# mauruszach/multimodal_diffusion

Hardware: AMD Instinct MI355X
Metric: denoising steps/sec @256x256 multimodal-cond batch=32 (higher is better)
Workload: dtype f32 via 3xbf16 split operands (6-term products, f32 accumulate; fp32-level error); 1 GPU; C3: 256x256 audio->video CFG denoising step (cond+null MMDiT d512 L8 H8 + noise head + DDIM), 384+37 tokens, batch 32 per GPU, DDIM 50 steps, guidance 3.5; global_batch=32, sampler_steps=50, parallelism=dp1, launch=eager, matmul=bf16x3, attn=default, cfg_halves=one stacked 2B batch, one stream

## Files before the change

### multimodal_diffusion_amd/csrc/attn_bf16x3.hip

```cpp
#include "avd_common.h"

#include <stdlib.h>
#include <type_traits>

namespace avd {

constexpr int A3_DH = 64, A3_KT = 64, A3_NW = 4;
constexpr float A3_NEG = -1.0e30f;

typedef short s16x4 __attribute__((ext_vector_type(4)));
typedef unsigned int u32x2 __attribute__((ext_vector_type(2)));
typedef float f32x4t __attribute__((ext_vector_type(4)));

#define AVD_LDS_PTR(p) ((__attribute__((address_space(3))) void*)(p))
#define AVD_GLB_PTR(p) ((const __attribute__((address_space(1))) void*)(p))

template <int TERMS> struct A3Terms;
template <> struct A3Terms<6> { static constexpr int N = 6; static constexpr int PA[6] = {2, 0, 1, 1, 0, 0}; static constexpr int PB[6] = {0, 2, 1, 0, 1, 0}; };
template <> struct A3Terms<9> { static constexpr int N = 9; static constexpr int PA[9] = {2, 2, 1, 2, 0, 1, 1, 0, 0}; static constexpr int PB[9] = {2, 1, 2, 0, 2, 1, 0, 1, 0}; };
template <> struct A3Terms<1> { static constexpr int N = 1; static constexpr int PA[1] = {0}; static constexpr int PB[1] = {0}; };
template <> struct A3Terms<3> { static constexpr int N = 3; static constexpr int PA[3] = {0, 1, 0}; static constexpr int PB[3] = {1, 0, 0}; };

template <bool SPLIT_OUT, int TERMS>
__global__ __launch_bounds__(A3_NW * 64, 2) void attn_bf16x3_kernel(const unsigned char* __restrict__ img, float* __restrict__ out,
                                                                    int Bt, int N, int Npad, int H, int n_query, int nqb,
                                                                    float s_inv2, float v_inv, float o_scale, int out_tok) {
    constexpr int NW = A3_NW, ROWB = QKV3_ROWB;
    constexpr bool F16 = TERMS == 3;
    constexpr int NPL = s3_planes(TERMS);
    constexpr int PPW = 24 / NW;
    __shared__ __attribute__((aligned(16))) unsigned char Ks[A3_KT * ROWB];
    __shared__ __attribute__((aligned(16))) unsigned char Vs[A3_KT * ROWB];

    int qb, h, b;
    {
        const int nwg = gridDim.x, id = blockIdx.x, q = nwg >> 3, r = nwg & 7, x = id & 7;
        const int w = (x < r ? x * (q + 1) : r * (q + 1) + (x - r) * q) + (id >> 3);
        qb = w % nqb;
        h = (w / nqb) % H;
        b = w / (nqb * H);
    }
    const int tid = threadIdx.x, lane = tid & 63, wave = tid >> 6;
    const int l31 = lane & 31, hi = lane >> 5;
    const int64_t hstride = (int64_t)Npad * ROWB;
    const unsigned char* Qb = img + (((int64_t)0 * Bt + b) * H + h) * hstride;
    const unsigned char* Kb = img + (((int64_t)1 * Bt + b) * H + h) * hstride;
    const unsigned char* Vb = img + (((int64_t)2 * Bt + b) * H + h) * hstride;

    const int q_row = qb * (NW * 32) + wave * 32 + l31;
    bf16x8 qf[4][3];
    {
        const unsigned char* src = Qb + (int64_t)(q_row < N ? q_row : N - 1) * ROWB + hi * 16;
#pragma unroll
        for (int s = 0; s < 4; ++s)
#pragma unroll
            for (int p = 0; p < NPL; ++p) qf[s][p] = *reinterpret_cast<const bf16x8*>(src + p * 128 + s * 32);
    }

    auto dma = [&](const unsigned char* gsrc, unsigned char* ldst, int kt) {
        const int last_row = N - 1 - kt * A3_KT;
#pragma unroll
        for (int i = 0; i < PPW; ++i) {
            const int p = wave + NW * i;
            const int off = p * 1024 + lane * 16;
            int row = off / ROWB;
            const int within = off - row * ROWB;
            row = row < last_row ? row : last_row;
            __builtin_amdgcn_global_load_lds(AVD_GLB_PTR(gsrc + ((int64_t)kt * A3_KT + row) * ROWB + within), AVD_LDS_PTR(ldst + p * 1024), 16,
                                             0, 0);
        }
    };

    f32x16 o0, o1;
#pragma unroll
    for (int r = 0; r < 16; ++r) { o0[r] = 0.f; o1[r] = 0.f; }
    float m_run = A3_NEG, l_run = 0.f;

    const int nkt = (N + A3_KT - 1) / A3_KT;
    dma(Kb, Ks, 0);
    dma(Vb, Vs, 0);
    __builtin_amdgcn_s_waitcnt(0x0f70);
    __syncthreads();

    const int ksw = (l31 >> 1) & 7;
    const int k_rd = l31 * ROWB;
    const int i16 = lane & 15, cb = (lane >> 4) & 1;
    const int v_q = i16 >> 2, v_p = i16 & 3;

    const bool active = qb * (NW * 32) + wave * 32 < n_query;
    for (int kt = 0; kt < nkt; ++kt) {
        const bool more = (kt + 1) < nkt;
        if (!active) {
            __builtin_amdgcn_s_waitcnt(0x0f70);
            __syncthreads();
            if (more) dma(Kb, Ks, kt + 1);
            __builtin_amdgcn_s_waitcnt(0x0f70);
            __syncthreads();
            if (more) dma(Vb, Vs, kt + 1);
            continue;
        }
        f32x16 s0, s1;
#pragma unroll
// ... 71 lines not shown
                for (int p = 0; p < NPL; ++p) pf[p] = __builtin_bit_cast(bf16x8, P[p]);
                const int key0 = 32 * kb + 16 * t + 4 * hi + v_q;
                const int sw = qkv3_swizzle(2, key0);
#pragma unroll
                for (int db = 0; db < 2; ++db) {
                    const int chunk = 4 * db + 2 * cb + (v_p >> 1);
                    bf16x8 vf[3];
#pragma unroll
                    for (int p = 0; p < NPL; ++p) {
                        const s16x4 lo = __builtin_amdgcn_ds_read_tr16_b64_v4i16((__attribute__((address_space(3))) s16x4*)AVD_LDS_PTR(
                            Vs + key0 * ROWB + p * 128 + ((chunk ^ sw) << 4) + 8 * (v_p & 1)));
                        const s16x4 up = __builtin_amdgcn_ds_read_tr16_b64_v4i16((__attribute__((address_space(3))) s16x4*)AVD_LDS_PTR(
                            Vs + (key0 + 8) * ROWB + p * 128 + ((chunk ^ sw) << 4) + 8 * (v_p & 1)));
                        const u32x2 a = __builtin_bit_cast(u32x2, lo), c2 = __builtin_bit_cast(u32x2, up);
                        const u32x4 w = {a[0], a[1], c2[0], c2[1]};
                        vf[p] = __builtin_bit_cast(bf16x8, w);
                    }
#pragma unroll
                    for (int tt = 0; tt < TT::N; ++tt) {
                        if (db == 0) o0 = mma16<F16>(vf[TT::PA[tt]], pf[TT::PB[tt]], o0);
                        else o1 = mma16<F16>(vf[TT::PA[tt]], pf[TT::PB[tt]], o1);
                    }
                }
            }
        __builtin_amdgcn_s_waitcnt(0x0f70);
        __syncthreads();
        if (more) dma(Vb, Vs, kt + 1);
    }
    if (!active) return;

    const float l_tot = l_run + __shfl_xor(l_run, 32, 64);
    const float inv = F16 ? v_inv / l_tot : 1.0f / l_tot;
    const int d = H * A3_DH;
    if constexpr (SPLIT_OUT) {
        float ch[8][4];
#pragma unroll
        for (int g4 = 0; g4 < 4; ++g4)
#pragma unroll
            for (int e = 0; e < 4; ++e) {
                ch[g4][e] = o0[4 * g4 + e] * inv;
                ch[4 + g4][e] = o1[4 * g4 + e] * inv;
            }
        unsigned char* o3 = reinterpret_cast<unsigned char*>(out);
#pragma unroll
        for (int c = 0; c < 8; c += 2) {
            float v[8];
#pragma unroll
            for (int e = 0; e < 4; ++e) {
                const float send = hi ? ch[c][e] : ch[c + 1][e];
                const float recv = __shfl_xor(send, 32, 64);
                v[e] = hi ? recv : ch[c][e];
                v[4 + e] = hi ? ch[c + 1][e] : recv;
            }
            if (q_row < n_query) {
                if constexpr (F16) store_split8_h2(o3, (int64_t)b * out_tok + q_row, h * A3_DH + 8 * (c + hi), d, v, o_scale);
                else store_split8(o3, (int64_t)b * out_tok + q_row, h * A3_DH + 8 * (c + hi), d, v);
            }
        }
    } else if (q_row < n_query) {
        float* dst = out + ((int64_t)b * out_tok + q_row) * d + h * A3_DH + 4 * hi;
#pragma unroll
        for (int g4 = 0; g4 < 4; ++g4) {
            f32x4 a = {o0[4 * g4] * inv, o0[4 * g4 + 1] * inv, o0[4 * g4 + 2] * inv, o0[4 * g4 + 3] * inv};
            f32x4 c = {o1[4 * g4] * inv, o1[4 * g4 + 1] * inv, o1[4 * g4 + 2] * inv, o1[4 * g4 + 3] * inv};
            *reinterpret_cast<f32x4*>(dst + 8 * g4) = a;
            *reinterpret_cast<f32x4*>(dst + 32 + 8 * g4) = c;
        }
    }
}

int g_attn_pipe = getenv("AVD_ATTN_PIPE") ? atoi(getenv("AVD_ATTN_PIPE")) : 1;

template <bool MORE_, bool KCL_, bool VCL_, bool COPY_> struct A3Flags {
    static constexpr bool MORE = MORE_, KCL = KCL_, VCL = VCL_, COPY = COPY_;
};

template <bool SPLIT_OUT, int TERMS>
__global__ __launch_bounds__(A3_NW * 64, 2) void attn_bf16x3_pipe_kernel(const unsigned char* __restrict__ img, float* __restrict__ out,
                                                                         int Bt, int N, int Npad, int H, int n_query, int nqb,
                                                                         float s_inv2, float v_inv, float o_scale, int out_tok) {
    constexpr int NW = A3_NW, ROWB = QKV3_ROWB;
    constexpr bool F16 = TERMS == 3;
    constexpr int NPL = s3_planes(TERMS);
    constexpr int PPW = 24 / NW;
    using TT = A3Terms<TERMS>;
    __shared__ __attribute__((aligned(16))) unsigned char Ks[A3_KT * ROWB];
    __shared__ __attribute__((aligned(16))) unsigned char Vs[A3_KT * ROWB];

    int qb, h, b;
    {
        const int nwg = gridDim.x, id = blockIdx.x, q = nwg >> 3, r = nwg & 7, x = id & 7;
        const int w = (x < r ? x * (q + 1) : r * (q + 1) + (x - r) * q) + (id >> 3);
        qb = w % nqb;
        h = (w / nqb) % H;
        b = w / (nqb * H);
    }
    const int tid = threadIdx.x, lane = tid & 63;
    const int wave = __builtin_amdgcn_readfirstlane(tid >> 6);
    const int l31 = lane & 31, hi = lane >> 5;
    const int64_t hstride = (int64_t)Npad * ROWB;
    const unsigned char* Qb = img + (((int64_t)0 * Bt + b) * H + h) * hstride;
    const unsigned char* Kb = img + (((int64_t)1 * Bt + b) * H + h) * hstride;
    const unsigned char* Vb = img + (((int64_t)2 * Bt + b) * H + h) * hstride;

    const int q_row = qb * (NW * 32) + wave * 32 + l31;
    bf16x8 qf[4][3];
    {
        const unsigned char* src = Qb + (int64_t)(q_row < N ? q_row : N - 1) * ROWB + hi * 16;
#pragma unroll
        for (int s = 0; s < 4; ++s)
#pragma unroll
            for (int p = 0; p < NPL; ++p) qf[s][p] = *reinterpret_cast<const bf16x8*>(src + p * 128 + s * 32);
    }
    auto dma_clamp = [&](const unsigned char* gsrc, unsigned char* ldst, int kt) {
        const int last_row = N - 1 - kt * A3_KT;
#pragma unroll
        for (int i = 0; i < PPW; ++i) {
            const int p = wave + NW * i;
            const int off = p * 1024 + lane * 16;
            int row = off / ROWB;
            const int within = off - row * ROWB;
            row = row < last_row ? row : last_row;
            __builtin_amdgcn_global_load_lds(AVD_GLB_PTR(gsrc + ((int64_t)kt * A3_KT + row) * ROWB + within), AVD_LDS_PTR(ldst + p * 1024), 16,
                                             0, 0);
        }
    };
    const unsigned lane16 = (unsigned)lane * 16u;
    auto dma_full = [&](const unsigned char* gsrc, unsigned char* ldst, int kt) {
        const unsigned char* base = gsrc + ((int64_t)kt * (A3_KT * ROWB) + wave * 1024);
#pragma unroll
        for (int i = 0; i < PPW; ++i)
            __builtin_amdgcn_global_load_lds(AVD_GLB_PTR(base + i * (NW * 1024) + lane16), AVD_LDS_PTR(ldst + (wave + NW * i) * 1024), 16, 0, 0);
    };
    auto sync = [&]() {
        __builtin_amdgcn_s_waitcnt(0x0f70);
        __syncthreads();
    };

    const int nkt = (N + A3_KT - 1) / A3_KT;
    const bool ragged = (N & (A3_KT - 1)) != 0;
    dma_clamp(Kb, Ks, 0);
    dma_clamp(Vb, Vs, 0);
    sync();

    const bool active = qb * (NW * 32) + wave * 32 < n_query;
    if (!active) {
        sync();
        if (nkt > 1) dma_clamp(Kb, Ks, 1);
        sync();
        for (int kt = 0; kt < nkt; ++kt) {
            sync();
            if (kt + 2 < nkt) dma_clamp(Kb, Ks, kt + 2);
            if (kt + 1 < nkt) {
                sync();
                dma_clamp(Vb, Vs, kt + 1);
            }
        }
        return;
// ... 169 lines not shown
            if constexpr (F16) mt *= s_inv2;
            mt = fmaxf(mt, __shfl_xor(mt, 32, 64));
            m_new = fmaxf(m_run, mt);
            if constexpr (FL::COPY) {
                c0 = n0;
                c1 = n1;
            }
            sync();
            if constexpr (FL::VCL) dma_clamp(Vb, Vs, kt + 1);
            else dma_full(Vb, Vs, kt + 1);
        }
    };
    {
        using Main = A3Flags<true, false, false, false>;
        using MainC = A3Flags<true, false, false, true>;
        using KClamp = A3Flags<true, true, false, true>;
        using VClamp = A3Flags<true, false, true, true>;
        using Last = A3Flags<false, false, false, false>;
        int kt = 0;
        for (; kt + 4 < nkt; kt += 2) {
            tile(Main{}, kt, sa0, sa1, sb0, sb1);
            tile(Main{}, kt + 1, sb0, sb1, sa0, sa1);
        }
        if (nkt - kt == 4) { tile(MainC{}, kt, sa0, sa1, sb0, sb1); ++kt; }
        if (nkt - kt == 3) { tile(KClamp{}, kt, sa0, sa1, sb0, sb1); ++kt; }
        if (nkt - kt == 2) { tile(VClamp{}, kt, sa0, sa1, sb0, sb1); ++kt; }
        tile(Last{}, kt, sa0, sa1, sb0, sb1);
    }
#undef A3_SB

    const float l_tot = l_run + __shfl_xor(l_run, 32, 64);
    const float inv = F16 ? v_inv / l_tot : 1.0f / l_tot;
    const int d = H * A3_DH;
    if constexpr (SPLIT_OUT) {
        float ch[8][4];
#pragma unroll
        for (int g4 = 0; g4 < 4; ++g4)
#pragma unroll
            for (int e = 0; e < 4; ++e) {
                ch[g4][e] = o0[4 * g4 + e] * inv;
                ch[4 + g4][e] = o1[4 * g4 + e] * inv;
            }
        unsigned char* o3 = reinterpret_cast<unsigned char*>(out);
#pragma unroll
        for (int c = 0; c < 8; c += 2) {
            float v[8];
#pragma unroll
            for (int e = 0; e < 4; ++e) {
                const float send = hi ? ch[c][e] : ch[c + 1][e];
                const float recv = __shfl_xor(send, 32, 64);
                v[e] = hi ? recv : ch[c][e];
                v[4 + e] = hi ? ch[c + 1][e] : recv;
            }
            if (q_row < n_query) {
                if constexpr (F16) store_split8_h2(o3, (int64_t)b * out_tok + q_row, h * A3_DH + 8 * (c + hi), d, v, o_scale);
                else store_split8(o3, (int64_t)b * out_tok + q_row, h * A3_DH + 8 * (c + hi), d, v);
            }
        }
    } else if (q_row < n_query) {
        float* dst = out + ((int64_t)b * out_tok + q_row) * d + h * A3_DH + 4 * hi;
#pragma unroll
        for (int g4 = 0; g4 < 4; ++g4) {
            f32x4 a = {o0[4 * g4] * inv, o0[4 * g4 + 1] * inv, o0[4 * g4 + 2] * inv, o0[4 * g4 + 3] * inv};
            f32x4 c = {o1[4 * g4] * inv, o1[4 * g4 + 1] * inv, o1[4 * g4 + 2] * inv, o1[4 * g4 + 3] * inv};
            *reinterpret_cast<f32x4*>(dst + 8 * g4) = a;
            *reinterpret_cast<f32x4*>(dst + 32 + 8 * g4) = c;
        }
    }
}

template <bool F16>
__device__ __forceinline__ f32x4t mma16s(bf16x8 a, bf16x8 b, f32x4t c) {
    if constexpr (F16) return __builtin_amdgcn_mfma_f32_16x16x32_f16(__builtin_bit_cast(f16x8, a), __builtin_bit_cast(f16x8, b), c, 0, 0, 0);
    else return __builtin_amdgcn_mfma_f32_16x16x32_bf16(a, b, c, 0, 0, 0);
}
int g_attn_m16 = getenv("AVD_ATTN_M16") ? atoi(getenv("AVD_ATTN_M16")) : 1;

struct S16 { f32x4t t[4][2]; };

template <bool SPLIT_OUT, int TERMS>
__global__ __launch_bounds__(A3_NW * 64, 2) void attn_bf16x3_p16_kernel(const unsigned char* __restrict__ img, float* __restrict__ out,
                                                                        int Bt, int N, int Npad, int H, int n_query, int nqb,
                                                                        float s_inv2, float v_inv, float o_scale, int out_tok) {
    constexpr int NW = A3_NW, ROWB = QKV3_ROWB;
    constexpr bool F16 = TERMS == 3;
    constexpr int NPL = s3_planes(TERMS);
    constexpr int PPW = 24 / NW;
    using TT = A3Terms<TERMS>;
    __shared__ __attribute__((aligned(16))) unsigned char Ks[A3_KT * ROWB];
    __shared__ __attribute__((aligned(16))) unsigned char Vs[A3_KT * ROWB];

    int qb, h, b;
    {
        const int nwg = gridDim.x, id = blockIdx.x, q = nwg >> 3, r = nwg & 7, x = id & 7;
        const int w = (x < r ? x * (q + 1) : r * (q + 1) + (x - r) * q) + (id >> 3);
        qb = w % nqb;
        h = (w / nqb) % H;
        b = w / (nqb * H);
    }
    const int tid = threadIdx.x, lane = tid & 63;
    const int wave = __builtin_amdgcn_readfirstlane(tid >> 6);
    const int l15 = lane & 15, kq = lane >> 4;
    const int64_t hstride = (int64_t)Npad * ROWB;
    const unsigned char* Qb = img + (((int64_t)0 * Bt + b) * H + h) * hstride;
    const unsigned char* Kb = img + (((int64_t)1 * Bt + b) * H + h) * hstride;
    const unsigned char* Vb = img + (((int64_t)2 * Bt + b) * H + h) * hstride;

    const int q_row0 = qb * (NW * 32) + wave * 32 + l15;
    bf16x8 qf[2][2][3];
#pragma unroll
    for (int qt = 0; qt < 2; ++qt) {
        const int qr = q_row0 + 16 * qt;
        const unsigned char* src = Qb + (int64_t)(qr < N ? qr : N - 1) * ROWB + kq * 16;
#pragma unroll
        for (int sd = 0; sd < 2; ++sd)
#pragma unroll
            for (int p = 0; p < NPL; ++p) qf[qt][sd][p] = *reinterpret_cast<const bf16x8*>(src + p * 128 + sd * 64);
    }
    auto dma_clamp = [&](const unsigned char* gsrc, unsigned char* ldst, int kt) {
        const int last_row = N - 1 - kt * A3_KT;
#pragma unroll
        for (int i = 0; i < PPW; ++i) {
            const int p = wave + NW * i;
            const int off = p * 1024 + lane * 16;
            int row = off / ROWB;
            const int within = off - row * ROWB;
            row = row < last_row ? row : last_row;
            __builtin_amdgcn_global_load_lds(AVD_GLB_PTR(gsrc + ((int64_t)kt * A3_KT + row) * ROWB + within), AVD_LDS_PTR(ldst + p * 1024), 16,
                                             0, 0);
        }
    };
    const unsigned lane16 = (unsigned)lane * 16u;
    auto dma_full = [&](const unsigned char* gsrc, unsigned char* ldst, int kt) {
        const unsigned char* base = gsrc + ((int64_t)kt * (A3_KT * ROWB) + wave * 1024);
#pragma unroll
        for (int i = 0; i < PPW; ++i)
// ... 205 lines not shown
#pragma unroll
                    for (int w = sl * 8 / NS; w < (sl + 1) * 8 / NS; ++w) split_pair(c, 1, w >> 2, w & 3, pf[1][w >> 2]);
                }
                if (MORE && g == 1) {
                    constexpr int NS = 4 * TT::N;
#pragma unroll
                    for (int w = sl * 16 / NS; w < (sl + 1) * 16 / NS; ++w) {
                        const int i = w >> 2, qt = (w >> 1) & 1, r0 = 2 * (w & 1);
                        mt[qt] = fmaxf(mt[qt], fmaxf(n.t[i][qt][r0], n.t[i][qt][r0 + 1]));
                    }
                    asm volatile("" : "+v"(mt[0]), "+v"(mt[1]));
                }
            }
        }
        A3_SB();
        if constexpr (MORE) {
#pragma unroll
            for (int qt = 0; qt < 2; ++qt) {
                if constexpr (F16) mt[qt] *= s_inv2;
                m_new[qt] = fmaxf(m_run[qt], xmax(mt[qt]));
            }
            if constexpr (FL::COPY) c = n;
            sync();
            if constexpr (FL::VCL) dma_clamp(Vb, Vs, kt + 1);
            else dma_full(Vb, Vs, kt + 1);
        }
    };
    {
        using Main = A3Flags<true, false, false, false>;
        using MainC = A3Flags<true, false, false, true>;
        using KClamp = A3Flags<true, true, false, true>;
        using VClamp = A3Flags<true, false, true, true>;
        using Last = A3Flags<false, false, false, false>;
        int kt = 0;
        for (; kt + 4 < nkt; kt += 2) {
            tile(Main{}, kt, sa, sb);
            tile(Main{}, kt + 1, sb, sa);
        }
        if (nkt - kt == 4) { tile(MainC{}, kt, sa, sb); ++kt; }
        if (nkt - kt == 3) { tile(KClamp{}, kt, sa, sb); ++kt; }
        if (nkt - kt == 2) { tile(VClamp{}, kt, sa, sb); ++kt; }
        tile(Last{}, kt, sa, sb);
    }
#undef A3_SB

    float inv[2];
#pragma unroll
    for (int qt = 0; qt < 2; ++qt) {
        const float l_tot = xsum(l_run[qt]);
        inv[qt] = F16 ? v_inv / l_tot : 1.0f / l_tot;
    }
    const int d = H * A3_DH;
    const int q_row = q_row0 + 16 * (kq & 1);
    unsigned char* o3 = reinterpret_cast<unsigned char*>(out);
#pragma unroll
    for (int dt = 0; dt < 4; ++dt) {
        float v[8];
#pragma unroll
        for (int r = 0; r < 4; ++r) {
            const auto sw = __builtin_amdgcn_permlane16_swap(__float_as_uint(o[dt][0][r] * inv[0]), __float_as_uint(o[dt][1][r] * inv[1]), false, false);
            v[r] = __uint_as_float(sw[0]);
            v[4 + r] = __uint_as_float(sw[1]);
        }
        const int col = h * A3_DH + 16 * dt + 8 * (kq >> 1);
        if (q_row < n_query) {
            if constexpr (SPLIT_OUT) {
                if constexpr (F16) store_split8_h2(o3, (int64_t)b * out_tok + q_row, col, d, v, o_scale);
                else store_split8(o3, (int64_t)b * out_tok + q_row, col, d, v);
            } else {
                float* dst = out + ((int64_t)b * out_tok + q_row) * d + col;
                *reinterpret_cast<f32x4*>(dst) = f32x4{v[0], v[1], v[2], v[3]};
                *reinterpret_cast<f32x4*>(dst + 4) = f32x4{v[4], v[5], v[6], v[7]};
            }
        }
    }
}

int64_t qkv3_bytes(int B, int N, int H) { return (int64_t)3 * B * H * qkv3_npad(N) * QKV3_ROWB; }

template <int TERMS>
static void attn3_launch(const unsigned char* img, float* out, void* out3, int B, int N, int Npad, int H, int n_query, int nqb, hipStream_t st,
                         float img_scale, float out_scale, int out_tok) {
    const float s_inv2 = 1.0f / (img_scale * img_scale), v_inv = 1.0f / img_scale;
    if (g_attn_m16 && (TERMS == 6 || TERMS == 9 || g_attn_m16 == 2)) {
        if (out3)
            hipLaunchKernelGGL((attn_bf16x3_p16_kernel<true, TERMS>), dim3(nqb * H * B), dim3(A3_NW * 64), 0, st, img, static_cast<float*>(out3),
                               B, N, Npad, H, n_query, nqb, s_inv2, v_inv, out_scale, out_tok);
        else
            hipLaunchKernelGGL((attn_bf16x3_p16_kernel<false, TERMS>), dim3(nqb * H * B), dim3(A3_NW * 64), 0, st, img, out, B, N, Npad, H,
                               n_query, nqb, s_inv2, v_inv, out_scale, out_tok);
        return;
    }
    if (g_attn_pipe == 2 || (g_attn_pipe == 1 && (TERMS == 6 || TERMS == 9))) {
        if (out3)
            hipLaunchKernelGGL((attn_bf16x3_pipe_kernel<true, TERMS>), dim3(nqb * H * B), dim3(A3_NW * 64), 0, st, img, static_cast<float*>(out3),
                               B, N, Npad, H, n_query, nqb, s_inv2, v_inv, out_scale, out_tok);
        else
            hipLaunchKernelGGL((attn_bf16x3_pipe_kernel<false, TERMS>), dim3(nqb * H * B), dim3(A3_NW * 64), 0, st, img, out, B, N, Npad, H,
                               n_query, nqb, s_inv2, v_inv, out_scale, out_tok);
        return;
    }
    if (out3)
        hipLaunchKernelGGL((attn_bf16x3_kernel<true, TERMS>), dim3(nqb * H * B), dim3(A3_NW * 64), 0, st, img, static_cast<float*>(out3), B, N,
                           Npad, H, n_query, nqb, s_inv2, v_inv, out_scale, out_tok);
    else
        hipLaunchKernelGGL((attn_bf16x3_kernel<false, TERMS>), dim3(nqb * H * B), dim3(A3_NW * 64), 0, st, img, out, B, N, Npad, H, n_query, nqb,
                           s_inv2, v_inv, out_scale, out_tok);
}

int attn_bf16x3(const void* qkv3, float* out, void* out3, int B, int N, int H, int n_query, int terms, hipStream_t st, float img_scale,
                float out_scale, int out_tokens) {
    const int out_tok = out_tokens > 0 ? out_tokens : N;
    AVD_REQUIRE(out_tok >= n_query, AVD_EINVAL, "attn_bf16x3: out_tokens=%d < n_query=%d", out_tok, n_query);
    AVD_REQUIRE(terms == 0 || terms == 6 || terms == 9 || terms == 1 || terms == 3, AVD_EINVAL, "attn_bf16x3: terms must be 6, 9, 1 or 3, got %d", terms);
    AVD_REQUIRE(img_scale > 0.f && img_scale < __builtin_inff() && out_scale > 0.f && out_scale < __builtin_inff() &&
                    img_scale * img_scale < __builtin_inff(), AVD_EINVAL, "attn_bf16x3: image scales must be positive and finite");
    AVD_REQUIRE(qkv3 && (out || out3), AVD_EINVAL, "attn_bf16x3: null pointer");
    AVD_REQUIRE(B > 0 && N > 0 && H > 0, AVD_EINVAL, "attn_bf16x3: bad dims B=%d N=%d H=%d", B, N, H);
    AVD_REQUIRE(n_query >= 0 && n_query <= N, AVD_EINVAL, "attn_bf16x3: n_query=%d outside [0,%d]", n_query, N);
    AVD_REQUIRE(aligned16(qkv3) && aligned16(out) && aligned16(out3), AVD_EUNSUPPORTED, "attn_bf16x3: pointers must be 16-byte aligned");
    AVD_REQUIRE(!out3 || (H * A3_DH) % 16 == 0, AVD_EUNSUPPORTED, "attn_bf16x3: split3 output needs d %% 16 == 0");
    if (n_query == 0) return AVD_OK;
    const int nqb = (n_query + 32 * A3_NW - 1) / (32 * A3_NW);
    AVD_REQUIRE((int64_t)B * H * nqb < (1ll << 31), AVD_EUNSUPPORTED, "attn_bf16x3: grid too large");
    const int tag = prof_tag_id("attn_bf16x3_kernel<%d>", terms ? terms : 6);
    ProfScope prof(tag, 4.0 * (double)B * H * (double)n_query * N * A3_DH, st);
    const int Npad = qkv3_npad(N);
    const auto* img = static_cast<const unsigned char*>(qkv3);
    if (terms == 9) attn3_launch<9>(img, out, out3, B, N, Npad, H, n_query, nqb, st, 1.f, 1.f, out_tok);
    else if (terms == 1) attn3_launch<1>(img, out, out3, B, N, Npad, H, n_query, nqb, st, 1.f, 1.f, out_tok);
    else if (terms == 3) attn3_launch<3>(img, out, out3, B, N, Npad, H, n_query, nqb, st, img_scale, out_scale, out_tok);
    else attn3_launch<6>(img, out, out3, B, N, Npad, H, n_query, nqb, st, 1.f, 1.f, out_tok);
    AVD_CHECK_LAUNCH("attn_bf16x3");
    return AVD_OK;
}

}

extern "C" int64_t avd_qkv3_bytes(int B, int N, int H) {
    if (B <= 0 || N <= 0 || H <= 0) return -1;
    return avd::qkv3_bytes(B, N, H);
}
extern "C" int avd_attn_fwd_qkv_f16x2_f32(const void* qkv, float* out, void* out2, int B, int N, int H, int n_query, float qkv_scale,
                                          float out_scale, avd_stream_t stream) {
    return avd::attn_bf16x3(qkv, out, out2, B, N, H, n_query, 3, static_cast<hipStream_t>(stream), qkv_scale, out_scale);
}
extern "C" int avd_attn_fwd_qkv3_f32(const void* qkv3, float* out, void* out3, int B, int N, int H, int n_query, int terms,
                                     avd_stream_t stream) {
    return avd::attn_bf16x3(qkv3, out, out3, B, N, H, n_query, terms, static_cast<hipStream_t>(stream));
}
```

### multimodal_diffusion_amd/csrc/avd_common.h

```cpp
#pragma once
#include <hip/hip_runtime.h>
#include <stdint.h>
#include <stdio.h>
#include <stdarg.h>
#include <atomic>

#include "../../include/avdiff_hip.h"

namespace avd {

int set_error(int code, const char* fmt, ...);

#define AVD_REQUIRE(cond, code, ...)                       \
    do {                                                   \
        if (!(cond)) return avd::set_error((code), __VA_ARGS__); \
    } while (0)

#define AVD_CHECK_LAUNCH(name)                                                          \
    do {                                                                                \
        hipError_t e__ = hipGetLastError();                                             \
        if (e__ != hipSuccess)                                                          \
            return avd::set_error(AVD_ELAUNCH, "%s: %s", (name), hipGetErrorString(e__)); \
    } while (0)

struct LdsAttr {
    std::atomic<uint64_t> done{0};
    int ensure(const void* kern, int lds_bytes, const char* what);
};

static inline bool aligned16(const void* p) { return (reinterpret_cast<uintptr_t>(p) & 15u) == 0; }

typedef float f32x4 __attribute__((ext_vector_type(4)));
typedef float f32x16 __attribute__((ext_vector_type(16)));

constexpr int kWave = 64;

__device__ __forceinline__ int mfma32_row(int r, int hi) { return (r & 3) + 8 * (r >> 2) + 4 * hi; }

__device__ __forceinline__ float gelu_erf(float x) {
    const float z = x * 0.70710678118654752440f;
    const float a = fabsf(z);
    const float t = __builtin_amdgcn_rcpf(fmaf(0.3275911f, a, 1.0f));
    float p = fmaf(1.061405429f, t, -1.453152027f);
    p = fmaf(p, t, 1.421413741f);
    p = fmaf(p, t, -0.284496736f);
    p = fmaf(p, t, 0.254829592f);
    p *= t;
    const float e = __builtin_amdgcn_exp2f(-a * a * 1.4426950408889634f);
    const float er = copysignf(fmaf(-p, e, 1.0f), z);
    return 0.5f * x * (1.0f + er);
}
__device__ __forceinline__ float silu(float x) { return x / (1.0f + expf(-x)); }

template <int ACT>
__device__ __forceinline__ float apply_act(float x) {
    if constexpr (ACT == AVD_ACT_GELU) return gelu_erf(x);
    else if constexpr (ACT == AVD_ACT_SILU) return silu(x);
    else return x;
}

__device__ __forceinline__ float wave_sum(float v) {
#pragma unroll
    for (int o = 32; o > 0; o >>= 1) v += __shfl_xor(v, o, 64);
    return v;
}

struct RowMap {
    int64_t ld;
    int64_t seg;
    int64_t stride;
    __host__ __device__ __forceinline__ int64_t off(int64_t r) const {
        return seg > 0 ? (r / seg) * stride + (r % seg) * ld : r * ld;
    }
};

struct TubeGather {
    int T, H, W, t, h, w, Ht, Wt, Nt;
    int64_t per;
    __host__ __device__ __forceinline__ int64_t row_off(int64_t row) const {
        const int64_t b = row / Nt;
        const int n = (int)(row - b * Nt);
        const int nx = n % Wt, ny = (n / Wt) % Ht, nt = n / (Wt * Ht);
        return b * per + ((int64_t)(nt * t) * H + ny * h) * W + nx * w;
    }
    __host__ __device__ __forceinline__ int64_t k_off(int k) const {
        const int dx = k % w, dy = (k / w) % h, dt = (k / (w * h)) % t, c = k / (w * h * t);
        return (((int64_t)c * T + dt) * H + dy) * W + dx;
    }
};

typedef __bf16 bf16x8 __attribute__((ext_vector_type(8)));
typedef unsigned int u32x4 __attribute__((ext_vector_type(4)));

constexpr int S3_CHUNK = 128 * 96;
constexpr int S3_PLANE = 128 * 32;

typedef __bf16 bf16x2 __attribute__((ext_vector_type(2)));
typedef float f32x2 __attribute__((ext_vector_type(2)));

__device__ __forceinline__ unsigned int pk_bf16(float a, float b) {
    const f32x2 v = {a, b};
    return __builtin_bit_cast(unsigned int, __builtin_convertvector(v, bf16x2));
}
__device__ __forceinline__ float bf16_lo(unsigned int p) { return __uint_as_float(p << 16); }
__device__ __forceinline__ float bf16_hi(unsigned int p) { return __uint_as_float(p & 0xffff0000u); }

template <bool RANGE_CHECK = true>
__device__ __forceinline__ void split8(const float* v, u32x4& H, u32x4& Mi, u32x4& Lo) {
#pragma clang fp contract(off)
    bool edge = false;
    if constexpr (RANGE_CHECK) {
        float amax = fabsf(v[0]);
#pragma unroll
        for (int e = 1; e < 8; ++e) amax = fmaxf(amax, fabsf(v[e]));
        edge = __any(amax > 3.3895313892515355e38f);
    }
#pragma unroll
    for (int e = 0; e < 4; ++e) {
        const float a = v[2 * e], b = v[2 * e + 1];
        unsigned int h = pk_bf16(a, b);
        float ra = a - bf16_lo(h), rb = b - bf16_hi(h);
        if (edge) {
            if ((h & 0x7fffu) == 0x7f80u) {
                if (fabsf(a) < __builtin_inff()) { h = (h & 0xffff8000u) | 0x7f7fu; ra = a - bf16_lo(h); } else ra = 0.f;
            }
            if ((h & 0x7fff0000u) == 0x7f800000u) {
// ... 75 lines not shown
             float* C, RowMap cm, int64_t M, int N, int K, int act, hipStream_t st);
int gemm_f32_tube(const float* z, const TubeGather& tg, const float* W, const float* bias, float* C, RowMap cm, int64_t M, int N, int K,
                  hipStream_t st);

extern int g_gemm_stages;
extern int g_gemm_force_tile;
bool gemm_f32_fold_supported(int N, int K);
int gemm_f32_fold(const float* A, RowMap am, const float* W, const float* bias, const float* R, RowMap rm, float* C, RowMap cm,
                  int64_t M, int N, int K, int act, const float* ss_in, int ss_in_cols, float sqrt_d, float eps, float* ss_out,
                  hipStream_t st);
int rowss_f32(const float* x, float* ss, int64_t rows, int d, hipStream_t st);
constexpr int kGemmSplitKMax = 4;
extern int g_gemm_splitk;
int gemm_f32_splitk_slices(int64_t M, int N, int K);
int64_t gemm_f32_splitk_ws_max_floats(int64_t M, int N, int K);
int gemm_f32_splitk(const float* A, RowMap am, const float* W, const float* bias, const float* R, RowMap rm, float* C, RowMap cm, int64_t M,
                    int N, int K, int ns, float* part, float* ss_out, hipStream_t st);

int attn_f32(const float* qkv, float* out, int B, int N, int H, int Dh, float scale, int n_query, const unsigned char* key_padding_mask,
             hipStream_t st);
int rmsnorm_f32(const float* x, RowMap xm, const float* scale, float* y, RowMap ym, int64_t rows, int d, float eps,
                hipStream_t st);
int layernorm_act_f32(const float* x, const float* gamma, const float* beta, float* y, int64_t rows, int d, float eps,
                      int act, hipStream_t st);
int weight_bounds_f32(const float* x, int64_t rows, int d, float* out2, hipStream_t st);

int64_t split3_bytes(int64_t rows, int K);
int split3_f32(const float* x, int64_t ld, void* out, int64_t rows, int K, hipStream_t st, float h2_scale = 0.f);
int split3_rows_f32(const float* x, RowMap xm, void* out, int64_t rows, int K, hipStream_t st, float h2_scale = 0.f, float* ss = nullptr);
int rmsnorm_split3_f32(const float* x, const float* scale, void* out, int64_t rows, int d, float eps, hipStream_t st, float h2_scale = 0.f);
int layernorm_act_split3_f32(const float* x, const float* gamma, const float* beta, void* out, int64_t rows, int d, float eps, int act,
                             hipStream_t st, float h2_scale = 0.f);
bool gemm_bf16x3_supported(int64_t M, int N, int K);
int attn_f32_split3(const float* qkv, void* out3, int B, int N, int H, int Dh, float scale, int n_query, hipStream_t st);
extern int g_s3_stagger;
extern int g_mlp_fused;
bool mlp_bf16x3_supported(int d, int hidden, int terms);
int mlp_bf16x3(const void* X3, const void* W1n3, const float* b1, const void* W23, const float* b2, const float* ss_in, float eps,
               const float* R, float* C, void* C3, float* ss_out, int64_t M, int d, int hidden, hipStream_t st);
extern int g_attn_m16;
extern int g_attn_pipe;
extern int g_s3_m16;
extern int g_s3_w128;
extern int g_s3_rt4;
extern int g_s3_deep4;
extern int g_s3_rt;
extern int g_vae_lat;
extern int g_vae_fold;
extern int g_codec_mfma;
extern int g_cfg_rows;
extern int g_s3_sn, g_s3_super4, g_s3_super8;
extern int g_s3_tile;
extern thread_local bool t_s3_two_streams;
int gemm_bf16x3_qkv3(const void* A3, const void* W3, const float* bias, void* img, int64_t M, int tokens, int heads, int K, float qscale,
                     int terms, hipStream_t st, float ab_scale = 1.f, float c_scale = 1.f, const float* ss_in = nullptr, float eps = 0.f);
int64_t qkv3_bytes(int B, int N, int H);
int64_t attn_fp8_ws_bytes(int B, int N, int H);
int attn_fp8(const void* qkv3, void* ws, int64_t ws_bytes, float* out, void* out3, int B, int N, int H, int n_query, hipStream_t st,
             int img_terms = 6, float img_scale = 1.f, float out_scale = 1.f);
int attn_bf16x3(const void* qkv3, float* out, void* out3, int B, int N, int H, int n_query, int terms, hipStream_t st,
                float img_scale = 1.f, float out_scale = 1.f, int out_tokens = 0);
int gemm_bf16x3(const void* A3, const void* W3, const float* bias, const float* R, float* C, void* C3, int64_t M, int N, int K,
                int act, int terms, hipStream_t st, float ab_scale = 1.f, float c_scale = 1.f, const float* ss_in = nullptr, float eps = 0.f,
                float* ss_out = nullptr, const float* gamma = nullptr, int r_seg = 0, int r_stride = 0);
bool gemm_bf16x3_resmap_supported(int terms);
bool gemm_bf16x3_rownorm_supported(int N, int terms);
extern int g_s3_splitk;
int gemm_bf16x3_splitk_slices(int64_t M, int N, int K, int terms);
int64_t gemm_bf16x3_splitk_ws_floats(int64_t M, int N, int ns);
constexpr int kS3SplitKMax = 4;
int64_t gemm_bf16x3_splitk_ws_max_floats(int64_t M, int N, int K);
int gemm_bf16x3_splitk(const void* A3, const void* W3, const float* bias, const float* R, float* C, void* C3, float* ss, int64_t M, int N,
                       int K, int terms, int ns, float* part, hipStream_t st);

}
```

### multimodal_diffusion_amd/csrc/composite.hip

```cpp
#include "avd_common.h"

#include <stdlib.h>

#include <string.h>
#include <map>
#include <mutex>
#include <string>
#include <utility>
#include <vector>

namespace avd {

static thread_local char g_err[512] = "";

int set_error(int code, const char* fmt, ...) {
    va_list ap;
    va_start(ap, fmt);
    vsnprintf(g_err, sizeof(g_err), fmt, ap);
    va_end(ap);
    return code;
}

int LdsAttr::ensure(const void* kern, int lds_bytes, const char* what) {
    int dev = 0;
    hipError_t e = hipGetDevice(&dev);
    if (e != hipSuccess) return set_error(AVD_ELAUNCH, "%s: hipGetDevice: %s", what, hipGetErrorString(e));
    const uint64_t bit = dev < 64 ? (uint64_t)1 << dev : 0;
    if (bit && (done.load(std::memory_order_acquire) & bit)) return AVD_OK;
    e = hipFuncSetAttribute(kern, hipFuncAttributeMaxDynamicSharedMemorySize, lds_bytes);
    if (e != hipSuccess) return set_error(AVD_ELAUNCH, "%s: hipFuncSetAttribute: %s", what, hipGetErrorString(e));
    done.fetch_or(bit, std::memory_order_release);
    return AVD_OK;
}

bool g_prof_on = false;
namespace {
struct ProfRec { hipEvent_t a, b; int tag; double work; };
std::vector<ProfRec> g_recs;
std::vector<hipEvent_t> g_pool;
std::vector<std::string> g_tags;
hipEvent_t take_event() {
    if (!g_pool.empty()) { hipEvent_t e = g_pool.back(); g_pool.pop_back(); return e; }
    hipEvent_t e; (void)hipEventCreate(&e); return e;
}
}
int prof_tag_id(const char* fmt, ...) {
    char buf[160];
    va_list ap;
    va_start(ap, fmt);
    vsnprintf(buf, sizeof(buf), fmt, ap);
    va_end(ap);
    for (size_t i = 0; i < g_tags.size(); ++i)
        if (g_tags[i] == buf) return (int)i;
    g_tags.emplace_back(buf);
    return (int)g_tags.size() - 1;
}
void prof_mark(int tag, double work, hipStream_t st, bool begin) {
    if (begin) {
        ProfRec r{take_event(), take_event(), tag, work};
        (void)hipEventRecord(r.a, st);
        g_recs.push_back(r);
    } else if (!g_recs.empty()) {
        (void)hipEventRecord(g_recs.back().b, st);
    }
}

int temb_f32(const int64_t* t, const float* freqs, float* out, int B, int dim, float max_period, hipStream_t st);
int tube_patch_f32(const float* z, float* tok, int B, int C, int T, int H, int W, int t, int h, int w, hipStream_t st);
int audio_tokens_f32(const float* z, float* tok, int B, int Ca, int F, int len, int stride, hipStream_t st);
int assemble_f32(float* X2, const float* temb, const float* Xp, int B, int N, int d, int tdim, int Nt, int Np,
                 int target_first, hipStream_t st);
int assemble_rows_f32(float* X2, const int64_t* t_now, const float* freqs, const float* Xp, float* ss, int B, int N, int d, int tdim,
                      int Nt, int Np, int target_first, float max_period, hipStream_t st);
int cfg_unpatch_ddim_f32(const float* eps2, const float* z, const int64_t* t_now, const int64_t* t_prev,
                         const float* abar, int T_train, float guidance, float eta, const float* noise, float* z_out,
                         int B, int C, int T, int H, int W, int t, int h, int w, hipStream_t st);
int cfg_untoken_ddim_audio_f32(const float* eps2, const float* z, const int64_t* t_now, const int64_t* t_prev,
                               const float* abar, int T_train, float guidance, float eta, const float* noise,
                               float* z_out, int B, int Ca, int F, int len, int stride, hipStream_t st);

static inline int64_t align_up(int64_t x) { return (x + 255) & ~(int64_t)255; }

struct Carver {
    char* base;
    int64_t used, cap;
    bool ok = true;
    float* take(int64_t floats) {
        float* p = reinterpret_cast<float*>(base + used);
        used += align_up(floats * (int64_t)sizeof(float));
        if (used > cap) ok = false;
        return p;
    }
};

constexpr int64_t kSplitMinRows = 6144;
constexpr int64_t kSplitMinRowsM16 = 2048;
static int64_t g_s3_min_rows = [] { const char* e = getenv("AVD_S3_MIN_ROWS"); return e ? (int64_t)atoll(e) : (int64_t)-1; }();
static bool g_no_fold = getenv("AVD_NO_FOLD") != nullptr;
static int64_t split_min_rows(int terms = 3) {
    if (g_s3_min_rows >= 0) return g_s3_min_rows;
    return (terms == 0 || terms == 6) && g_s3_m16 ? kSplitMinRowsM16 : kSplitMinRows;
}
static bool core_split_capable(const avd_core_weights* w, int64_t M) {
    if (w->norm_kind != 0) return false;
    if (!gemm_bf16x3_supported(M, 3 * w->d, w->d) || !gemm_bf16x3_supported(M, w->d, w->d) ||
        !gemm_bf16x3_supported(M, w->mlp_hidden, w->d) || !gemm_bf16x3_supported(M, w->d, w->mlp_hidden))
        return false;
    for (int l = 0; l < w->n_layers; ++l) {
        const avd_block_weights& b = w->blocks[l];
        if (!b.in_proj_weight3 || !b.out_proj_weight3 || !b.fc1_weight3 || !b.fc2_weight3) return false;
    }
    return true;
}
static thread_local int64_t t_step_rows = 0;
static bool core_use_split(const avd_core_weights* w, int64_t M) {
    const int64_t Mt = t_step_rows > M ? t_step_rows : M;
    if (Mt < split_min_rows(w->split_terms) && w->split_terms != 1 && w->attn_mode != 1) return false;
    return core_split_capable(w, M);
}

static bool core_split_fold_capable(const avd_core_weights* w) {
    if (w->norm_kind != 0 || w->split_terms == 3 || w->d % 64 != 0) return false;
    for (int l = 0; l < w->n_layers; ++l)
        if (!w->blocks[l].in_proj_weight3n || !w->blocks[l].fc1_weight3n) return false;
    return true;
}
static bool core_use_split_fold(const avd_core_weights* w) { return !g_no_fold && core_split_fold_capable(w); }

static bool core_split_rownorm_capable(const avd_core_weights* w) {
    return w->norm_kind == 0 && w->split_terms == 3 && gemm_bf16x3_rownorm_supported(w->d, 3);
}
static bool core_use_split_rownorm(const avd_core_weights* w) { return !g_no_fold && core_split_rownorm_capable(w); }

static bool core_use_fold(const avd_core_weights* w) {
    if (g_no_fold || w->norm_kind != 0) return false;
    if (!gemm_f32_fold_supported(3 * w->d, w->d) || !gemm_f32_fold_supported(w->d, w->d) ||
        !gemm_f32_fold_supported(w->mlp_hidden, w->d) || !gemm_f32_fold_supported(w->d, w->mlp_hidden))
        return false;
    for (int l = 0; l < w->n_layers; ++l)
        if (!w->blocks[l].in_proj_weight_n || !w->blocks[l].fc1_weight_n) return false;
    return true;
}

static bool g_core_trim = getenv("AVD_CORE_TRIM") ? atoi(getenv("AVD_CORE_TRIM")) != 0 : true;
static int64_t core_trim_floats(const avd_core_weights* w, int B, int N) { return (int64_t)B * N * w->d; }

static int64_t core_split_wide_bytes(const avd_core_weights* w, int B, int N) {
    const int64_t qkv3 = qkv3_bytes(B, N, w->n_heads), fc1 = split3_bytes((int64_t)B * N, w->mlp_hidden);
    return qkv3 > fc1 ? qkv3 : fc1;
}

static int64_t core_ws_bytes(const avd_core_weights* w, int B, int N) {
    const int64_t M = (int64_t)B * N;
    const int wide = 3 * w->d > w->mlp_hidden ? 3 * w->d : w->mlp_hidden;
    int64_t fp32_path = align_up(M * w->d * 4) + align_up(M * wide * 4) + 2 * align_up(M * (w->d / 32 + 1) * 4) +
                        align_up(gemm_f32_splitk_ws_max_floats(M, w->d, w->mlp_hidden) * 4);
    if (!core_split_capable(w, M)) return fp32_path;
    const int64_t wide_b = core_split_wide_bytes(w, B, N);
    const int64_t f8_b = w->attn_mode == 1 ? attn_fp8_ws_bytes(B, N, w->n_heads) : 0;
    const int64_t fold_b = core_split_fold_capable(w) ? align_up(split3_bytes(M, w->d)) + align_up(M * (w->d / 64) * 4)
                         : core_split_rownorm_capable(w) ? align_up(split3_bytes(M, w->d)) : 0;
    const int64_t sk_b = core_split_fold_capable(w) ? align_up(gemm_bf16x3_splitk_ws_max_floats(M, w->d, w->mlp_hidden) * 4) : 0;
    const int64_t trim_b = core_split_fold_capable(w) ? align_up(core_trim_floats(w, B, N) * 4) : 0;
    const int64_t split_path = align_up(wide_b) + align_up(split3_bytes(M, w->d)) + align_up(f8_b) + fold_b + sk_b + trim_b;
    return split_path > fp32_path ? split_path : fp32_path;
}

static int check_core(const avd_core_weights* w) {
    AVD_REQUIRE(w && w->blocks && w->final_norm_scale, AVD_EINVAL, "core: null weight table");
    AVD_REQUIRE(w->d > 0 && w->n_layers > 0 && w->n_heads > 0 && w->mlp_hidden > 0, AVD_EINVAL, "core: bad dims");
    AVD_REQUIRE(w->d % w->n_heads == 0, AVD_EINVAL, "core: d_model %d not divisible by n_heads %d", w->d, w->n_heads);
    AVD_REQUIRE(w->attn_mode == 0 || w->attn_mode == 1, AVD_EINVAL, "core: attn_mode must be 0 (follow the matmul mode) or 1 (fp8)");
    AVD_REQUIRE(w->norm_kind == 0 || w->norm_kind == 1, AVD_EINVAL, "core: norm_kind must be 0 (RMSNorm) or 1 (LayerNorm)");
    AVD_REQUIRE(w->d / w->n_heads == 64, AVD_EUNSUPPORTED, "core: head_dim %d unsupported (64 only)", w->d / w->n_heads);
    AVD_REQUIRE(w->d % 4 == 0 && w->mlp_hidden % 4 == 0, AVD_EUNSUPPORTED, "core: widths must be multiples of 4");
    AVD_REQUIRE(w->split_terms == 0 || w->split_terms == 6 || w->split_terms == 9 || w->split_terms == 1 || w->split_terms == 3, AVD_EINVAL,
                "core: split_terms must be 0/6 (default), 9 (strict), 1 (plain bf16) or 3 (f16x2), got %d", w->split_terms);
    if (w->split_terms == 3) {
        for (int l = 0; l < w->n_layers; ++l)
            for (int i = 0; i < 8; ++i) {
                const float s = w->blocks[l].f16x2_scale[i];
                AVD_REQUIRE(s > 0.f && s < __builtin_inff(), AVD_EINVAL, "core: blocks[%d].f16x2_scale[%d] must be positive and finite", l, i);
            }
    }
    return AVD_OK;
}

static int core_norm(const avd_core_weights* w, const float* x, const float* scale, const float* bias, float* y, int64_t M, hipStream_t st) {
    const RowMap rd{w->d, 0, 0};
    if (w->norm_kind == 0) return rmsnorm_f32(x, rd, scale, y, rd, M, w->d, w->norm_eps, st);
    AVD_REQUIRE(bias, AVD_EINVAL, "core: norm_kind 1 (LayerNorm) needs the bias vectors");
    return layernorm_act_f32(x, scale, bias, y, M, w->d, w->norm_eps, AVD_ACT_NONE, st);
}

static int core_forward(const avd_core_weights* w, const float* x, float* y, int B, int N, int out_row0,
                        int n_out_rows, const unsigned char* kpm, void* ws, int64_t ws_bytes, hipStream_t st,
                        const float* ss_first = nullptr) {
    if (int rc = check_core(w)) return rc;
    AVD_REQUIRE(x && y && B > 0 && N > 0, AVD_EINVAL, "core: bad input");
    AVD_REQUIRE(out_row0 >= 0 && n_out_rows > 0 && out_row0 + n_out_rows <= N, AVD_EINVAL, "core: bad output row window");
    const int64_t M = (int64_t)B * N;
    AVD_REQUIRE(ws && ws_bytes >= core_ws_bytes(w, B, N), AVD_EWORKSPACE, "core: workspace %lld < %lld bytes",
                (long long)ws_bytes, (long long)core_ws_bytes(w, B, N));
    const int d = w->d, hid = w->mlp_hidden, H = w->n_heads;
    Carver cv{static_cast<char*>(ws), 0, ws_bytes};
    float* hbuf = cv.take(M * d);
    float* wide = cv.take(M * (3 * d > hid ? 3 * d : hid));
    const RowMap rd{d, 0, 0}, r3{3 * d, 0, 0}, rh{hid, 0, 0};
    const float scale = 1.0f / sqrtf((float)(d / H));
    const float* cur = x;
    AVD_REQUIRE(!(w->attn_mode == 1 && (kpm || w->norm_kind != 0)), AVD_EUNSUPPORTED,
                "core: attn_mode 1 (fp8 attention) cannot be combined with a key_padding_mask or norm_kind 1 (LayerNorm)");
    AVD_REQUIRE(!(w->attn_mode == 1 && !core_use_split(w, M)), AVD_EUNSUPPORTED,
                "core: attn_mode 1 (fp8 attention) reads the q|k|v image of the split-operand projections, which these weights / shapes "
                "do not take (every block needs its *_weight3 images; 3 d, d and mlp_hidden must be multiples of 256, d of 16)");
    if (!kpm && core_use_split(w, M)) {
        const int terms = w->split_terms;
        Carver cs{static_cast<char*>(ws), 0, ws_bytes};
        const int64_t wide_b = core_split_wide_bytes(w, B, N);
        float* qkv = cs.take((wide_b + 3) / 4);
        void* wide3 = qkv;
        void* hs = cs.take((split3_bytes(M, d) + 3) / 4);
        const int64_t f8_b = w->attn_mode == 1 ? attn_fp8_ws_bytes(B, N, H) : 0;
        float* f8w = cs.take((f8_b + 3) / 4);
        if (core_use_split_fold(w)) {
            void* hx = cs.take((split3_bytes(M, d) + 3) / 4);
            float* ss = cs.take(M * (d / 64));
            const int ns = gemm_bf16x3_splitk_slices(M, d, hid, terms);
            float* part = ns ? cs.take(gemm_bf16x3_splitk_ws_floats(M, d, ns)) : nullptr;
            const bool trim = g_core_trim && out_row0 == 0 && n_out_rows < N && w->attn_mode == 0 && gemm_bf16x3_resmap_supported(terms);
            float* yc = cs.take(core_trim_floats(w, B, N));
            const bool fused = g_mlp_fused && !ns && mlp_bf16x3_supported(d, hid, terms) && gemm_bf16x3_resmap_supported(terms);
            AVD_REQUIRE(cs.ok, AVD_EWORKSPACE, "core: workspace carve %lld > %lld bytes", (long long)cs.used, (long long)cs.cap);
            if (int rc = split3_rows_f32(cur, rd, hx, M, d, st, 0.f, ss)) return rc;
            for (int l = 0; l < w->n_layers; ++l) {
                const avd_block_weights& b = w->blocks[l];
                const bool last = l == w->n_layers - 1;
                const int nq = (last && out_row0 == 0) ? n_out_rows : N;
                if (last && trim) {
                    const int64_t Mc = (int64_t)B * nq;
                    if (int rc = gemm_bf16x3_qkv3(hx, b.in_proj_weight3n, b.in_proj_bias, qkv, M, N, H, d, scale * 1.4426950408889634f, terms, st,
                                                  1.f, 1.f, ss, w->norm_eps)) return rc;
                    if (int rc = attn_bf16x3(qkv, nullptr, hs, B, N, H, nq, terms, st, 1.f, 1.f, nq)) return rc;
                    if (int rc = gemm_bf16x3(hs, b.out_proj_weight3, b.out_proj_bias, cur, yc, hx, Mc, d, d, AVD_ACT_NONE, terms, st, 1.f, 1.f,
                                             nullptr, 0.f, ss, nullptr, nq, N)) return rc;
                    if (fused) {
                        if (int rc = mlp_bf16x3(hx, b.fc1_weight3n, b.fc1_bias, b.fc2_weight3, b.fc2_bias, ss, w->norm_eps, yc, yc, nullptr, nullptr, Mc,
                                                d, hid, st)) return rc;
                    } else {
                        if (int rc = gemm_bf16x3(hx, b.fc1_weight3n, b.fc1_bias, nullptr, nullptr, wide3, Mc, hid, d, AVD_ACT_GELU, terms, st, 1.f, 1.f,
                                                 ss, w->norm_eps)) return rc;
                        if (ns) {
                            if (int rc = gemm_bf16x3_splitk(wide3, b.fc2_weight3, b.fc2_bias, yc, yc, nullptr, nullptr, Mc, d, hid, terms, ns, part,
                                                            st)) return rc;
                        } else {
                            if (int rc = gemm_bf16x3(wide3, b.fc2_weight3, b.fc2_bias, yc, yc, nullptr, Mc, d, hid, AVD_ACT_NONE, terms, st)) return rc;
                        }
                    }
                    return rmsnorm_f32(yc, rd, w->final_norm_scale, y, RowMap{d, nq, (int64_t)N * d}, Mc, d, w->norm_eps, st);
                }
                if (int rc = gemm_bf16x3_qkv3(hx, b.in_proj_weight3n, b.in_proj_bias, qkv, M, N, H, d, scale * 1.4426950408889634f, terms, st,
                                              1.f, 1.f, ss, w->norm_eps)) return rc;
                if (w->attn_mode == 1) {
                    if (int rc = attn_fp8(qkv, f8w, f8_b, nullptr, hs, B, N, H, nq, st, terms, 1.f, 1.f)) return rc;
                } else {
                    if (int rc = attn_bf16x3(qkv, nullptr, hs, B, N, H, nq, terms, st, 1.f, 1.f)) return rc;
                }
                if (int rc = gemm_bf16x3(hs, b.out_proj_weight3, b.out_proj_bias, cur, y, hx, M, d, d, AVD_ACT_NONE, terms, st, 1.f, 1.f, nullptr,
                                         0.f, ss)) return rc;
                cur = y;
                if (fused) {
                    if (int rc = mlp_bf16x3(hx, b.fc1_weight3n, b.fc1_bias, b.fc2_weight3, b.fc2_bias, ss, w->norm_eps, y, y, last ? nullptr : hx,
                                            last ? nullptr : ss, M, d, hid, st)) return rc;
                    continue;
                }
                if (int rc = gemm_bf16x3(hx, b.fc1_weight3n, b.fc1_bias, nullptr, nullptr, wide3, M, hid, d, AVD_ACT_GELU, terms, st, 1.f, 1.f, ss,
                                         w->norm_eps)) return rc;
                if (ns) {
                    if (int rc = gemm_bf16x3_splitk(wide3, b.fc2_weight3, b.fc2_bias, y, y, last ? nullptr : hx, last ? nullptr : ss, M, d, hid,
                                                    terms, ns, part, st)) return rc;
                } else if (last) {
                    if (int rc = gemm_bf16x3(wide3, b.fc2_weight3, b.fc2_bias, y, y, nullptr, M, d, hid, AVD_ACT_NONE, terms, st)) return rc;
                } else {
                    if (int rc = gemm_bf16x3(wide3, b.fc2_weight3, b.fc2_bias, y, y, hx, M, d, hid, AVD_ACT_NONE, terms, st, 1.f, 1.f, nullptr, 0.f,
                                             ss)) return rc;
                }
            }
            return rmsnorm_f32(y, rd, w->final_norm_scale, y, rd, M, d, w->norm_eps, st);
        }
        const bool rown = core_use_split_rownorm(w);
        void* hn = rown ? cs.take((split3_bytes(M, d) + 3) / 4) : hs;
        AVD_REQUIRE(cs.ok, AVD_EWORKSPACE, "core: workspace carve %lld > %lld bytes", (long long)cs.used, (long long)cs.cap);
        for (int l = 0; l < w->n_layers; ++l) {
            const avd_block_weights& b = w->blocks[l];
            const bool last = l == w->n_layers - 1;
            const int nq = (last && out_row0 == 0) ? n_out_rows : N;
            const bool h2 = terms == 3;
            const float* fs = b.f16x2_scale;
            const float s_n1 = h2 ? fs[4] : 0.f, s_qkv = h2 ? fs[5] : 1.f, s_n2 = h2 ? fs[6] : 0.f, s_fc1 = h2 ? fs[7] : 1.f;
            const float w_in = h2 ? fs[0] : 1.f, w_out = h2 ? fs[1] : 1.f, w_fc1 = h2 ? fs[2] : 1.f, w_fc2 = h2 ? fs[3] : 1.f;
            if (!rown || l == 0)
                if (int rc = rmsnorm_split3_f32(cur, b.norm1_scale, hn, M, d, w->norm_eps, st, s_n1)) return rc;
            if (int rc = gemm_bf16x3_qkv3(hn, b.in_proj_weight3, b.in_proj_bias, qkv, M, N, H, d, scale * 1.4426950408889634f, terms, st,
                                          h2 ? s_n1 * w_in : 1.f, s_qkv)) return rc;
            if (w->attn_mode == 1) {
                if (int rc = attn_fp8(qkv, f8w, f8_b, nullptr, hs, B, N, H, nq, st, terms, s_qkv, s_qkv)) return rc;
            } else {
                if (int rc = attn_bf16x3(qkv, nullptr, hs, B, N, H, nq, terms, st, s_qkv, s_qkv)) return rc;
            }
            if (rown) {
                if (int rc = gemm_bf16x3(hs, b.out_proj_weight3, b.out_proj_bias, cur, y, hn, M, d, d, AVD_ACT_NONE, terms, st, s_qkv * w_out, s_n2,
                                         nullptr, w->norm_eps, nullptr, b.norm2_scale)) return rc;
                cur = y;
            } else {
                if (int rc = gemm_bf16x3(hs, b.out_proj_weight3, b.out_proj_bias, cur, y, nullptr, M, d, d, AVD_ACT_NONE, terms, st,
                                         h2 ? s_qkv * w_out : 1.f, 1.f)) return rc;
                cur = y;
                if (int rc = rmsnorm_split3_f32(y, b.norm2_scale, hn, M, d, w->norm_eps, st, s_n2)) return rc;
            }
            if (int rc = gemm_bf16x3(hn, b.fc1_weight3, b.fc1_bias, nullptr, nullptr, wide3, M, hid, d, AVD_ACT_GELU, terms, st,
                                     h2 ? s_n2 * w_fc1 : 1.f, s_fc1)) return rc;
            if (rown && !last) {
                const avd_block_weights& nb = w->blocks[l + 1];
                if (int rc = gemm_bf16x3(wide3, b.fc2_weight3, b.fc2_bias, y, y, hn, M, d, hid, AVD_ACT_NONE, terms, st, s_fc1 * w_fc2,
                                         nb.f16x2_scale[4], nullptr, w->norm_eps, nullptr, nb.norm1_scale)) return rc;
            } else {
                if (int rc = gemm_bf16x3(wide3, b.fc2_weight3, b.fc2_bias, y, y, nullptr, M, d, hid, AVD_ACT_NONE, terms, st,
                                         h2 ? s_fc1 * w_fc2 : 1.f, 1.f)) return rc;
            }
        }
        return rmsnorm_f32(y, rd, w->final_norm_scale, y, rd, M, d, w->norm_eps, st);
    }
    if (core_use_fold(w)) {
        float* ssA = cv.take(M * (d / 32 + 1));
        float* ssB = cv.take(M * (d / 32 + 1));
        const int nsf = gemm_f32_splitk_slices(M, d, hid);
        float* partf = nsf ? cv.take((int64_t)nsf * M * d) : nullptr;
        AVD_REQUIRE(cv.ok, AVD_EWORKSPACE, "core: workspace carve %lld > %lld bytes", (long long)cv.used, (long long)cv.cap);
        const float sqrt_d = (float)sqrt((double)d);
        const float* ssA_in = ss_first;
        if (!ssA_in) {
// ... 88 lines not shown
        float* t2 = cv.take(rows * w->hidden);
        if (int rc = split3_rows_f32(h, hm, imgA, rows, w->d_in, st, asc(0))) return rc;
        if (int rc = gemm_bf16x3(imgA, w->input_proj_weight3, w->input_proj_bias, nullptr, nullptr, imgB, rows, w->hidden, w->d_in, AVD_ACT_NONE,
                                 terms, st, h2 ? asc(0) * wsc(0) : 1.f, h2 ? asc(1) : 1.f)) return rc;
        void* cur = imgB;
        void* nxt = imgA;
        for (int j = 0; j < n; ++j) {
            if (int rc = gemm_bf16x3(cur, w->shared_lin_weight3[j], w->shared_lin_bias[j], nullptr, t2, nullptr, rows, w->hidden, w->hidden,
                                     AVD_ACT_NONE, terms, st, h2 ? asc(1 + j) * wsc(1 + j) : 1.f, 1.f)) return rc;
            if (int rc = layernorm_act_split3_f32(t2, w->shared_ln_weight[j], w->shared_ln_bias[j], nxt, rows, w->hidden, w->ln_eps, w->act, st,
                                                  asc(2 + j))) return rc;
            void* t = cur; cur = nxt; nxt = t;
        }
        return gemm_bf16x3(cur, w->out_proj_weight3, w->out_proj_bias, nullptr, out, nullptr, rows, w->d_out, w->hidden, AVD_ACT_NONE, terms, st,
                           h2 ? asc(1 + n) * wsc(1 + n) : 1.f, 1.f);
    }
    float* t1 = cv.take(rows * w->hidden);
    float* t2 = cv.take(rows * w->hidden);
    if (int rc = gemm_f32(h, hm, w->input_proj_weight, w->input_proj_bias, nullptr, rh, t1, rh, rows, w->hidden, w->d_in, AVD_ACT_NONE, st)) return rc;
    for (int j = 0; j < w->n_shared; ++j) {
        if (int rc = gemm_f32(t1, rh, w->shared_lin_weight[j], w->shared_lin_bias[j], nullptr, rh, t2, rh, rows, w->hidden, w->hidden, AVD_ACT_NONE, st)) return rc;
        if (int rc = layernorm_act_f32(t2, w->shared_ln_weight[j], w->shared_ln_bias[j], t1, rows, w->hidden, w->ln_eps, w->act, st)) return rc;
    }
    return gemm_f32(t1, rh, w->out_proj_weight, w->out_proj_bias, nullptr, ro, out, ro, rows, w->d_out, w->hidden, AVD_ACT_NONE, st);
}

static int check_embed(const avd_embed_desc* e) {
    AVD_REQUIRE(e, AVD_EINVAL, "embed: null descriptor");
    AVD_REQUIRE(e->B > 0 && e->d > 0 && e->tdim >= 0, AVD_EINVAL, "embed: bad widths");
    AVD_REQUIRE(e->temb_add ? e->tdim == e->d : e->tdim < e->d, AVD_EINVAL,
                "embed: timestep width %d does not fit token width %d in %s mode", e->tdim, e->d, e->temb_add ? "add" : "concat");
    AVD_REQUIRE(e->d % 4 == 0 && e->tdim % 4 == 0, AVD_EUNSUPPORTED, "embed: d and tdim must be multiples of 4");
    AVD_REQUIRE(e->Nt > 0 && e->Np >= 0, AVD_EINVAL, "embed: bad token counts");
    if (e->target_kind == 0) {
        AVD_REQUIRE(e->p0 > 0 && e->p1 > 0 && e->p2 > 0 && e->T % e->p0 == 0 && e->H % e->p1 == 0 && e->W % e->p2 == 0,
                    AVD_EINVAL, "tube sizes must divide latent dims");
        AVD_REQUIRE(e->Nt == (e->T / e->p0) * (e->H / e->p1) * (e->W / e->p2), AVD_EINVAL, "embed: token count mismatch");
    } else if (e->target_kind == 1) {
        AVD_REQUIRE(e->p0 > 0 && e->p1 > 0 && e->T >= e->p0, AVD_EINVAL, "embed: bad audio chunking");
        AVD_REQUIRE(e->Nt == (e->T - e->p0) / e->p1 + 1, AVD_EINVAL, "embed: token count mismatch");
    } else {
        return set_error(AVD_EINVAL, "embed: unknown target_kind %d", e->target_kind);
    }
    return AVD_OK;
}
static int embed_tok_dim(const avd_embed_desc* e) {
    return e->target_kind == 0 ? e->C * e->p0 * e->p1 * e->p2 : e->C * e->p0;
}
static int64_t embed_ws_floats(const avd_embed_desc* e) {
    return align_up((int64_t)e->B * e->Nt * embed_tok_dim(e) * 4) / 4 + align_up((int64_t)e->B * (e->tdim > 0 ? e->tdim : 1) * 4) / 4;
}

static int embed_cfg_pair(const avd_embed_desc* e, const float* z, const float* Wt, const float* bt,
                          const int64_t* t_now, const float* Xp, float* tok_ws, float* X2, hipStream_t st, float* ss_out = nullptr) {
    if (int rc = check_embed(e)) return rc;
    AVD_REQUIRE(z && Wt && t_now && tok_ws && X2 && (e->Np == 0 || Xp), AVD_EINVAL, "embed: null pointer");
    const int B = e->B, d = e->d, N = e->Nt + e->Np, D = embed_tok_dim(e);
    float* tok = tok_ws;
    float* temb = tok_ws + align_up((int64_t)B * e->Nt * D * 4) / 4;
    const bool fuse_patch = e->target_kind == 0 && !e->temb_add && e->p2 % 4 == 0 && e->W % 4 == 0 && D % 4 == 0 && aligned16(z);
    if (e->target_kind == 0) {
        if (!fuse_patch)
            if (int rc = tube_patch_f32(z, tok, B, e->C, e->T, e->H, e->W, e->p0, e->p1, e->p2, st)) return rc;
    } else {
        if (int rc = audio_tokens_f32(z, tok, B, e->C, e->T, e->p0, e->p1, st)) return rc;
    }
    if (e->tdim > 0 && e->temb_add)
        if (int rc = temb_f32(t_now, e->temb_freqs, temb, B, e->tdim, 10000.f, st)) return rc;
    float* c0 = X2 + (e->target_first ? 0 : (int64_t)e->Np * d);
    const RowMap cm{d, e->Nt, (int64_t)N * d};
    if (e->temb_add) {
        const RowMap rm{0, e->Nt, (int64_t)e->tdim};
        if (int rc = gemm_f32(tok, RowMap{D, 0, 0}, Wt, bt, temb, rm, c0, cm, (int64_t)B * e->Nt, d, D, AVD_ACT_NONE, st)) return rc;
        return assemble_f32(X2, temb, Xp, B, N, d, 0, e->Nt, e->Np, e->target_first, st);
    }
    if (fuse_patch) {
        const TubeGather tg{e->T, e->H, e->W, e->p0, e->p1, e->p2, e->H / e->p1, e->W / e->p2, e->Nt, (int64_t)e->C * e->T * e->H * e->W};
        if (int rc = gemm_f32_tube(z, tg, Wt, bt, c0, cm, (int64_t)B * e->Nt, d - e->tdim, D, st)) return rc;
    } else {
        if (int rc = gemm_f32(tok, RowMap{D, 0, 0}, Wt, bt, nullptr, cm, c0, cm, (int64_t)B * e->Nt, d - e->tdim, D, AVD_ACT_NONE, st)) return rc;
    }
    return assemble_rows_f32(X2, t_now, e->temb_freqs, Xp, ss_out, B, N, d, e->tdim, e->Nt, e->Np, e->target_first, 10000.f, st);
}

#define AVD_HIP(call)                                                                        \
    do {                                                                                     \
        hipError_t e__ = (call);                                                             \
        if (e__ != hipSuccess) return set_error(AVD_ELAUNCH, "%s: %s", #call, hipGetErrorString(e__)); \
    } while (0)

struct AuxState { hipStream_t aux = nullptr; hipEvent_t fork = nullptr, join = nullptr; };
static std::mutex g_aux_mu;
static std::map<std::pair<int, hipStream_t>, AuxState> g_aux_map;
static int ensure_aux(hipStream_t st, AuxState& out) {
    int dev = 0;
    AVD_HIP(hipGetDevice(&dev));
    std::lock_guard<std::mutex> lk(g_aux_mu);
    AuxState& a = g_aux_map[{dev, st}];
    if (!a.aux) {
        AVD_HIP(hipStreamCreateWithFlags(&a.aux, hipStreamNonBlocking));
        AVD_HIP(hipEventCreateWithFlags(&a.fork, hipEventDisableTiming));
        AVD_HIP(hipEventCreateWithFlags(&a.join, hipEventDisableTiming));
    }
    out = a;
    return AVD_OK;
}

struct StepPlan {
    int64_t x2, tok, core, head, eps, ss, total;
    int N, D;
    int64_t rows;
};
static int plan_step(const avd_step_desc* s, StepPlan& p) {
    AVD_REQUIRE(s && s->core && s->head, AVD_EINVAL, "step: null descriptor");
    if (int rc = check_embed(&s->embed)) return rc;
    if (int rc = check_core(s->core)) return rc;
    const avd_embed_desc& e = s->embed;
    AVD_REQUIRE(e.d == s->core->d && s->head->d_in == e.d, AVD_EINVAL, "step: width mismatch between embed/core/head");
    p.N = e.Nt + e.Np;
    p.D = embed_tok_dim(&e);
    AVD_REQUIRE(s->head->d_out == p.D, AVD_EINVAL, "step: head d_out %d != token dim %d", s->head->d_out, p.D);
    p.rows = (int64_t)2 * e.B * e.Nt;
    p.x2 = align_up((int64_t)2 * e.B * p.N * e.d * 4);
    p.tok = align_up(embed_ws_floats(&e) * 4);
    const int64_t halves = 2 * core_ws_bytes(s->core, e.B, p.N), whole = core_ws_bytes(s->core, 2 * e.B, p.N);
    p.core = halves > whole ? halves : whole;
    const int64_t head_halves = 2 * head_ws_bytes(s->head, p.rows / 2), head_whole = head_ws_bytes(s->head, p.rows);
    p.head = head_halves > head_whole ? head_halves : head_whole;
    p.eps = align_up(p.rows * p.D * 4);
    p.ss = align_up((int64_t)2 * e.B * p.N * 4);
    p.total = p.x2 + p.tok + p.core + p.head + p.ss + p.eps;
    return AVD_OK;
}

}

using namespace avd;

extern "C" int avd_abi_version(void) { return AVD_ABI_VERSION; }
extern "C" const char* avd_last_error(void) { return g_err; }

extern "C" int avd_tune_set(const char* key, int64_t value) {
    AVD_REQUIRE(key, AVD_EINVAL, "tune_set: null key");
    if (!strcmp(key, "s3_tile")) { g_s3_tile = (int)value; return AVD_OK; }
    if (!strcmp(key, "s3_m16")) { g_s3_m16 = (int)value; return AVD_OK; }
    if (!strcmp(key, "s3_rt")) { g_s3_rt = (int)value; return AVD_OK; }
    if (!strcmp(key, "s3_rt4")) {
        AVD_REQUIRE(value == 0 || (value >= 2 && value <= 8), AVD_EINVAL, "tune_set: s3_rt4 must be 0 (automatic) or 2 .. 8");
        g_s3_rt4 = (int)value;
        return AVD_OK;
    }
    if (!strcmp(key, "s3_deep4")) { g_s3_deep4 = value != 0; return AVD_OK; }
    if (!strcmp(key, "s3_w128")) { g_s3_w128 = (int)value; return AVD_OK; }
    if (!strcmp(key, "s3_splitk")) {
        AVD_REQUIRE(value >= 0 && value <= kS3SplitKMax, AVD_EINVAL, "tune_set: s3_splitk must be in [0, %d]", kS3SplitKMax);
        g_s3_splitk = (int)value;
        return AVD_OK;
    }
    if (!strcmp(key, "s3_stagger")) { g_s3_stagger = (int)value; return AVD_OK; }
    if (!strcmp(key, "cfg_rows")) { g_cfg_rows = value != 0; return AVD_OK; }
    if (!strcmp(key, "vae_lat")) { g_vae_lat = value != 0; return AVD_OK; }
    if (!strcmp(key, "vae_fold")) { g_vae_fold = value != 0; return AVD_OK; }
    if (!strcmp(key, "codec_mfma")) { g_codec_mfma = value != 0; return AVD_OK; }
    if (!strcmp(key, "s3_sn")) { g_s3_sn = (int)value; return AVD_OK; }
    if (!strcmp(key, "s3_super4")) { g_s3_super4 = (int)value; return AVD_OK; }
    if (!strcmp(key, "s3_super8")) { g_s3_super8 = (int)value; return AVD_OK; }
    if (!strcmp(key, "attn_pipe")) { g_attn_pipe = (int)value; return AVD_OK; }
    if (!strcmp(key, "attn_m16")) { g_attn_m16 = (int)value; return AVD_OK; }
    if (!strcmp(key, "core_trim")) { g_core_trim = value != 0; return AVD_OK; }
    if (!strcmp(key, "mlp_fused")) { g_mlp_fused = (int)value; return AVD_OK; }
    if (!strcmp(key, "gemm_tile")) { g_gemm_force_tile = (int)value; return AVD_OK; }
    if (!strcmp(key, "gemm_stages")) { g_gemm_stages = (int)value; return AVD_OK; }
    if (!strcmp(key, "gemm_splitk")) {
        AVD_REQUIRE(value >= 0 && value <= kGemmSplitKMax, AVD_EINVAL, "tune_set: gemm_splitk must be in [0, %d]", kGemmSplitKMax);
        g_gemm_splitk = (int)value;
        return AVD_OK;
    }
    if (!strcmp(key, "s3_min_rows")) { g_s3_min_rows = value; return AVD_OK; }
    if (!strcmp(key, "no_fold")) { g_no_fold = value != 0; return AVD_OK; }
    return set_error(AVD_EINVAL, "tune_set: unknown key '%s'", key);
}

extern "C" int avd_device_arch(char* buf, int buflen) {
    AVD_REQUIRE(buf && buflen > 0, AVD_EINVAL, "device_arch: bad buffer");
    hipDeviceProp_t prop;
    int dev = 0;
    hipError_t e = hipGetDevice(&dev);
    if (e != hipSuccess) return set_error(AVD_ELAUNCH, "hipGetDevice: %s", hipGetErrorString(e));
    e = hipGetDeviceProperties(&prop, dev);
    if (e != hipSuccess) return set_error(AVD_ELAUNCH, "hipGetDeviceProperties: %s", hipGetErrorString(e));
    strncpy(buf, prop.gcnArchName, buflen - 1);
    buf[buflen - 1] = 0;
    return AVD_OK;
}

extern "C" int64_t avd_core_workspace_bytes(const avd_core_weights* w, int B, int N) {
    if (!w || B <= 0 || N <= 0) return -1;
    return core_ws_bytes(w, B, N);
}
extern "C" int avd_core_forward_f32(const avd_core_weights* w, const float* x, float* y, int B, int N, int out_row0,
                                    int n_out_rows, const uint8_t* key_padding_mask, void* workspace, int64_t workspace_bytes,
                                    avd_stream_t stream) {
    return core_forward(w, x, y, B, N, out_row0, n_out_rows, key_padding_mask, workspace, workspace_bytes,
                        static_cast<hipStream_t>(stream));
}

extern "C" int64_t avd_head_workspace_bytes(const avd_head_weights* w, int64_t rows) {
    if (!w || rows < 0) return -1;
    return head_ws_bytes(w, rows);
}
extern "C" int avd_head_forward_f32(const avd_head_weights* w, const float* h, int64_t ldh, int64_t seg_rows,
                                    int64_t seg_stride, int64_t rows, float* out, void* workspace,
                                    int64_t workspace_bytes, avd_stream_t stream) {
    return head_forward(w, h, RowMap{ldh, seg_rows, seg_stride}, rows, out, workspace, workspace_bytes,
                        static_cast<hipStream_t>(stream));
}

extern "C" int64_t avd_embed_workspace_floats(const avd_embed_desc* e) {
    if (check_embed(e)) return -1;
    return embed_ws_floats(e);
}
extern "C" int avd_embed_cfg_pair_f32(const avd_embed_desc* desc, const float* z_target, const float* Wt,
                                      const float* bt, const int64_t* t_now, const float* Xp, float* tok_ws, float* X2,
                                      avd_stream_t stream) {
    return embed_cfg_pair(desc, z_target, Wt, bt, t_now, Xp, tok_ws, X2, static_cast<hipStream_t>(stream));
}

extern "C" int64_t avd_step_workspace_bytes(const avd_step_desc* s) {
    StepPlan p;
    if (plan_step(s, p)) return -1;
    return p.total;
}

extern "C" int avd_denoise_step_f32(const avd_step_desc* s, const float* z, const float* Xp, const int64_t* t_now,
                                    const int64_t* t_prev, const float* noise, float* z_out, void* workspace,
                                    int64_t workspace_bytes, avd_stream_t stream) {
    StepPlan p;
    if (int rc = plan_step(s, p)) return rc;
    AVD_REQUIRE(z && z_out && t_now && t_prev && s->alpha_bar && s->adapt_w, AVD_EINVAL, "step: null pointer");
    AVD_REQUIRE(z != z_out, AVD_EINVAL, "step: z_out must not alias z");
    AVD_REQUIRE(workspace && workspace_bytes >= p.total, AVD_EWORKSPACE, "step: workspace %lld < %lld bytes",
                (long long)workspace_bytes, (long long)p.total);
    hipStream_t st = static_cast<hipStream_t>(stream);
    const avd_embed_desc& e = s->embed;
    char* w = static_cast<char*>(workspace);
    float* X2 = reinterpret_cast<float*>(w);
    float* tok = reinterpret_cast<float*>(w + p.x2);
    void* core_ws = w + p.x2 + p.tok;
    void* head_ws = w + p.x2 + p.tok + p.core;
    float* ssx = reinterpret_cast<float*>(w + p.x2 + p.tok + p.core + p.head);
    float* eps2 = reinterpret_cast<float*>(w + p.x2 + p.tok + p.core + p.head + p.ss);
    const bool have_ss = !e.temb_add;

    if (int rc = embed_cfg_pair(&e, z, s->adapt_w, s->adapt_b, t_now, Xp, tok, X2, st, ssx)) return rc;
    const int row0 = e.target_first ? 0 : e.Np;
    const RowMap hm{e.d, e.Nt, (int64_t)p.N * e.d};
    if (!s->split_streams) {
        if (int rc = core_forward(s->core, X2, X2, 2 * e.B, p.N, row0, e.Nt, nullptr, core_ws, p.core, st, have_ss ? ssx : nullptr)) return rc;
        if (int rc = head_forward(s->head, X2 + (int64_t)row0 * e.d, hm, p.rows, eps2, head_ws, p.head, st)) return rc;
    } else {
        AuxState ax;
        if (int rc = ensure_aux(st, ax)) return rc;
        hipStream_t g_aux = ax.aux;
        hipEvent_t g_fork = ax.fork, g_join = ax.join;
        const int64_t half_rows = (int64_t)e.B * p.N * e.d;
        const int64_t hc = p.core / 2, hh = p.head / 2;
        AVD_HIP(hipEventRecord(g_fork, st));
        AVD_HIP(hipStreamWaitEvent(g_aux, g_fork, 0));
        struct TwoStreams {
            TwoStreams(int64_t rows, int64_t head_rows) { t_s3_two_streams = true; t_step_rows = rows; t_step_head_rows = head_rows; }
            ~TwoStreams() { t_s3_two_streams = false; t_step_rows = 0; t_step_head_rows = 0; }
        } two_streams_scope((int64_t)2 * e.B * p.N, p.rows);
        for (int half = 0; half < 2; ++half) {
            hipStream_t hs = half ? g_aux : st;
            float* xh = X2 + half * half_rows;
            if (int rc = core_forward(s->core, xh, xh, e.B, p.N, row0, e.Nt, nullptr, static_cast<char*>(core_ws) + half * hc, hc, hs,
                                      have_ss ? ssx + (int64_t)half * e.B * p.N : nullptr)) return rc;
            if (int rc = head_forward(s->head, xh + (int64_t)row0 * e.d, hm, p.rows / 2, eps2 + half * (p.rows / 2) * p.D,
                                      static_cast<char*>(head_ws) + half * hh, hh, hs)) return rc;
        }
        AVD_HIP(hipEventRecord(g_join, g_aux));
        AVD_HIP(hipStreamWaitEvent(st, g_join, 0));
    }
    if (e.target_kind == 0)
        return cfg_unpatch_ddim_f32(eps2, z, t_now, t_prev, s->alpha_bar, s->T_train, s->guidance, s->eta, noise, z_out,
                                    e.B, e.C, e.T, e.H, e.W, e.p0, e.p1, e.p2, st);
    return cfg_untoken_ddim_audio_f32(eps2, z, t_now, t_prev, s->alpha_bar, s->T_train, s->guidance, s->eta, noise, z_out,
                                      e.B, e.C, e.T, e.p0, e.p1, st);
}

extern "C" int avd_prof_enable(int on) {
    if (on) {
        for (auto& r : g_recs) { g_pool.push_back(r.a); g_pool.push_back(r.b); }
        g_recs.clear();
    }
    g_prof_on = on != 0;
    return AVD_OK;
}

extern "C" int avd_prof_num_tags(void) { return (int)g_tags.size(); }
extern "C" const char* avd_prof_tag_name(int tag) { return (tag >= 0 && tag < (int)g_tags.size()) ? g_tags[tag].c_str() : ""; }

extern "C" int avd_prof_report(int64_t* launches, double* total_ms, double* work, int ntags) {
    AVD_REQUIRE(launches && total_ms && work && ntags >= (int)g_tags.size(), AVD_EINVAL, "prof_report: need %d tags",
                (int)g_tags.size());
    for (int i = 0; i < ntags; ++i) { launches[i] = 0; total_ms[i] = 0.0; work[i] = 0.0; }
    for (auto& r : g_recs) {
        hipError_t e = hipEventSynchronize(r.b);
        if (e != hipSuccess) return set_error(AVD_ELAUNCH, "prof_report: %s", hipGetErrorString(e));
        float ms = 0.f;
        e = hipEventElapsedTime(&ms, r.a, r.b);
// ... 6 lines not shown
```

### multimodal_diffusion_amd/csrc/gemm_bf16x3.hip

```cpp
#include "avd_common.h"
#include "s3_common.h"

#include <stdlib.h>
#include <type_traits>

namespace avd {


template <bool F16>
__global__ __launch_bounds__(256) void split3_kernel(const float* __restrict__ x, RowMap xm, unsigned char* __restrict__ out,
                                                     int64_t rows, int64_t rows_pad, int K, float s, float* __restrict__ ss) {
    const int64_t i = (int64_t)blockIdx.x * 256 + threadIdx.x;
    const int per_row = K >> 3;
    if (i >= rows_pad * per_row) return;
    const int64_t r = i / per_row;
    const int k = (int)(i % per_row) * 8;
    float v[8] = {0.f, 0.f, 0.f, 0.f, 0.f, 0.f, 0.f, 0.f};
    if (r < rows) {
        const float* xr = x + xm.off(r) + k;
        *reinterpret_cast<f32x4*>(v) = *reinterpret_cast<const f32x4*>(xr);
        *reinterpret_cast<f32x4*>(v + 4) = *reinterpret_cast<const f32x4*>(xr + 4);
    }
    if constexpr (F16) store_split8_h2(out, r, k, K, v, s);
    else store_split8(out, r, k, K, v);
// ... 133 lines not shown
                    if constexpr (F16) store_split8_h2(g.C3, m, n, g.N, v, g.c_scale);
                    else store_split8(g.C3, m, n, g.N, v);
                }
            }
        } else {
            const int cr = lane >> 4, cc = (lane & 15) * 4;
            const int n = nbase + cc;
            f32x4 bv = {0.f, 0.f, 0.f, 0.f};
            if (g.bias) bv = *reinterpret_cast<const f32x4*>(g.bias + n);
            float* cptr = g.C + (m0 + cr) * g.N + n;
            const float* rptr = EPI == S3_EPI_RES ? g.R + (m0 + cr) * g.N + n : nullptr;
#pragma unroll
            for (int c0 = 0; c0 < 16; c0 += 8) {
                f32x4 rv[8];
                if constexpr (EPI == S3_EPI_RES) {
#pragma unroll
                    for (int u = 0; u < 8; ++u)
                        rv[u] = m0 + cr + (c0 + u) * 4 < g.M ? *reinterpret_cast<const f32x4*>(rptr + (int64_t)(c0 + u) * 4 * g.N)
                                                            : f32x4{0.f, 0.f, 0.f, 0.f};
                }
#pragma unroll
                for (int u = 0; u < 8; ++u) {
                    const int it = c0 + u;
                    f32x4 v = *reinterpret_cast<const f32x4*>(slab + (cr + it * 4) * CLD + cc);
                    if constexpr (F16) v *= g.ab_inv;
                    v += bv;
                    if constexpr (EPI == S3_EPI_RES) v += rv[u];
                    if (m0 + cr + it * 4 < g.M) *reinterpret_cast<f32x4*>(cptr + (int64_t)it * 4 * g.N) = v;
                }
            }
        }
    }
}

template <int EPI, bool F16>
__device__ __forceinline__ void s3_epilogue_img_t(const S3Args& g, f32x16 (&acc)[4][2], int64_t mwave0, int nbase, int lane, bool big) {
    const int l31 = lane & 31, hi = lane >> 5;
    float bv[2][2][8];
#pragma unroll
    for (int j = 0; j < 2; ++j)
#pragma unroll
        for (int cg = 0; cg < 2; ++cg) {
            const float* bp = g.bias + nbase + 32 * j + 8 * (2 * cg + hi);
            *reinterpret_cast<f32x4*>(bv[j][cg]) = *reinterpret_cast<const f32x4*>(bp);
            *reinterpret_cast<f32x4*>(bv[j][cg] + 4) = *reinterpret_cast<const f32x4*>(bp + 4);
        }
    [[maybe_unused]] float mul = 1.0f;
    [[maybe_unused]] float ssq[4] = {0.f, 0.f, 0.f, 0.f};
    [[maybe_unused]] int64_t qbase = 0;
    if constexpr (EPI == S3_EPI_QKV3) {
        const int dmodel = g.heads * 64;
        const int part = nbase / dmodel, head = (nbase % dmodel) >> 6;
        mul = part == 0 ? g.qscale : 1.0f;
        qbase = (((int64_t)part * (g.M / g.tokN)) * g.heads + head) * (int64_t)g.tokNpad * QKV3_ROWB;
    }
#pragma unroll
    for (int i = 0; i < 4; ++i) {
        const int64_t m = mwave0 + 32 * i + l31;
        float rinv = 1.0f;
        if (EPI != S3_EPI_RES_IMG && g.ss_in != nullptr && m < g.M) {
            const int nc = g.K >> 6;
            const float* sp = g.ss_in + m * nc;
            float ssum = 0.f;
            if (nc == 8) {
                const f32x4 p0 = *reinterpret_cast<const f32x4*>(sp), p1 = *reinterpret_cast<const f32x4*>(sp + 4);
                const f32x4 t = p0 + p1;
                ssum = (t[0] + t[1]) + (t[2] + t[3]);
            } else {
                for (int c = 0; c < nc; ++c) ssum += sp[c];
            }
            rinv = 1.0f / (sqrtf(ssum) / g.ss_sqrt_d + g.ss_eps);
        }
        [[maybe_unused]] unsigned char* qrow = nullptr;
        [[maybe_unused]] int qsw = 0;
        if constexpr (EPI == S3_EPI_QKV3) {
            const unsigned b = (unsigned)m / (unsigned)g.tokN, tok = (unsigned)m - b * (unsigned)g.tokN;
            const int dmodel = g.heads * 64;
            qrow = g.C3 + qbase + ((int64_t)b * g.heads * g.tokNpad + tok) * QKV3_ROWB;
            qsw = qkv3_swizzle(nbase / dmodel, (int)tok);
        }
#pragma unroll
        for (int j = 0; j < 2; ++j)
#pragma unroll
            for (int cg = 0; cg < 2; ++cg) {
                float v[8];
#pragma unroll
                for (int e = 0; e < 4; ++e) {
                    const auto sw = __builtin_amdgcn_permlane32_swap(__float_as_uint(acc[i][j][8 * cg + e]), __float_as_uint(acc[i][j][8 * cg + 4 + e]),
                                                                     false, false);
                    v[e] = __uint_as_float(sw[0]);
                    v[4 + e] = __uint_as_float(sw[1]);
                }
                if constexpr (EPI == S3_EPI_QKV3) {
#pragma unroll
                    for (int e = 0; e < 8; ++e) v[e] = fmaf(F16 ? v[e] * g.ab_inv : v[e], rinv, bv[j][cg][e]) * mul;
                    if (S3_ROW_OK(m)) {
                        const int c = 4 * j + 2 * cg + hi;
                        unsigned char* dst = qrow + ((c ^ qsw) << 4);
                        if constexpr (F16) {
                            u32x4 Hh, Lo;
                            split8_h2(v, g.c_scale, Hh, Lo);
                            *reinterpret_cast<u32x4*>(dst) = Hh;
                            *reinterpret_cast<u32x4*>(dst + 128) = Lo;
                        } else {
                            u32x4 Hh, Mi, Lo;
                            if (big) split8<true>(v, Hh, Mi, Lo);
                            else split8<false>(v, Hh, Mi, Lo);
                            *reinterpret_cast<u32x4*>(dst) = Hh;
                            *reinterpret_cast<u32x4*>(dst + 128) = Mi;
                            *reinterpret_cast<u32x4*>(dst + 256) = Lo;
                        }
                    }
                } else if constexpr (EPI == S3_EPI_RES_IMG) {
                    const int n = nbase + 32 * j + 8 * (2 * cg + hi);
                    if (m < g.M) {
                        const float* rp = g.R + m * g.N + n;
                        const f32x4 r0 = *reinterpret_cast<const f32x4*>(rp), r1 = *reinterpret_cast<const f32x4*>(rp + 4);
#pragma unroll
                        for (int e = 0; e < 8; ++e) v[e] = ((F16 ? v[e] * g.ab_inv : v[e]) + bv[j][cg][e]) + (e < 4 ? r0[e] : r1[e - 4]);
                        float* cp = g.C + m * g.N + n;
                        *reinterpret_cast<f32x4*>(cp) = f32x4{v[0], v[1], v[2], v[3]};
                        *reinterpret_cast<f32x4*>(cp + 4) = f32x4{v[4], v[5], v[6], v[7]};
                        ssq[i] += ((v[0] * v[0] + v[1] * v[1]) + (v[2] * v[2] + v[3] * v[3])) + ((v[4] * v[4] + v[5] * v[5]) + (v[6] * v[6] + v[7] * v[7]));
                        if constexpr (F16) store_split8_h2(g.C3, m, n, g.N, v, g.c_scale);
                        else if (big) store_split8<true>(g.C3, m, n, g.N, v);
                        else store_split8<false>(g.C3, m, n, g.N, v);
                    }
                } else {
                    const int n = nbase + 32 * j + 8 * (2 * cg + hi);
#pragma unroll
                    for (int e = 0; e < 8; ++e) {
                        const float t = fmaf(F16 ? v[e] * g.ab_inv : v[e], rinv, bv[j][cg][e]);
                        v[e] = EPI == S3_EPI_GELU_SPLIT ? gelu_erf(t) : t;
                    }
                    if (S3_ROW_OK(m)) {
                        if constexpr (F16) store_split8_h2(g.C3, m, n, g.N, v, g.c_scale);
                        else if (big) store_split8<true>(g.C3, m, n, g.N, v);
                        else store_split8<false>(g.C3, m, n, g.N, v);
                    }
                }
            }
    }
    if constexpr (EPI == S3_EPI_RES_IMG) {
#pragma unroll
        for (int i = 0; i < 4; ++i) {
            const float tot = ssq[i] + __shfl_xor(ssq[i], 32, 64);
            const int64_t m = mwave0 + 32 * i + l31;
            if (hi == 0 && m < g.M) g.ss_out[m * (g.N >> 6) + (nbase >> 6)] = tot;
        }
    }
}

template <int EPI, bool F16>
__device__ __forceinline__ void s3_epilogue_img(const S3Args& g, f32x16 (&acc)[4][2], int64_t mwave0, int nbase, int lane) {
    bool big = false;
    if constexpr (!F16) {
        const int l31 = lane & 31;
        float amax = 0.f;
#pragma unroll
        for (int i = 0; i < 4; ++i) {
            float a = 0.f;
#pragma unroll
            for (int j = 0; j < 2; ++j)
// ... 884 lines not shown
    AVD_REQUIRE(h2_scale >= 0.f && h2_scale < __builtin_inff(), AVD_EINVAL, "rmsnorm_split3: f16x2 image scale must be positive and finite");
#define AVD_RMS3(NC)                                                                                                                  \
    if (h2_scale > 0.f) hipLaunchKernelGGL((rmsnorm_split3_kernel<NC, true>), dim3(grid), dim3(256), 0, st, x, scale, o, rows, d, eps, isd, h2_scale); \
    else hipLaunchKernelGGL((rmsnorm_split3_kernel<NC, false>), dim3(grid), dim3(256), 0, st, x, scale, o, rows, d, eps, isd, 0.f)
    switch ((d + 511) / 512) {
        case 1: AVD_RMS3(1); break;
        case 2: AVD_RMS3(2); break;
        case 3: AVD_RMS3(3); break;
        default: AVD_RMS3(4); break;
    }
#undef AVD_RMS3
    AVD_CHECK_LAUNCH("rmsnorm_split3");
    return AVD_OK;
}

int layernorm_act_split3_f32(const float* x, const float* gamma, const float* beta, void* out, int64_t rows, int d, float eps, int act,
                             hipStream_t st, float h2_scale) {
    AVD_REQUIRE(x && gamma && beta && out, AVD_EINVAL, "layernorm_split3: null pointer");
    AVD_REQUIRE(rows > 0 && d > 0 && d % 16 == 0 && d <= 2048, AVD_EUNSUPPORTED, "layernorm_split3: d=%d must be a multiple of 16, <= 2048", d);
    AVD_REQUIRE(aligned16(x) && aligned16(out) && aligned16(gamma) && aligned16(beta), AVD_EUNSUPPORTED, "layernorm_split3: pointers must be 16-byte aligned");
    AVD_REQUIRE(h2_scale >= 0.f && h2_scale < __builtin_inff(), AVD_EINVAL, "layernorm_split3: f16x2 image scale must be positive and finite");
    static const int tag = prof_tag_id("layernorm_act_split3_kernel");
    ProfScope prof(tag, image_rw_bytes(h2_scale) * (double)rows * d, st);
    const unsigned grid = (unsigned)((rows + 3) / 4);
    unsigned char* o = static_cast<unsigned char*>(out);
#define AVD_LN3K(NC, F16, G) hipLaunchKernelGGL((layernorm_act_split3_kernel<NC, F16, G>), dim3(grid), dim3(256), 0, st, x, gamma, beta, o, rows, d, eps, act, h2_scale)
#define AVD_LN3(NC)                                                                            \
    if (h2_scale > 0.f) { if (act == AVD_ACT_GELU) AVD_LN3K(NC, true, true); else AVD_LN3K(NC, true, false); } \
    else { if (act == AVD_ACT_GELU) AVD_LN3K(NC, false, true); else AVD_LN3K(NC, false, false); }
    switch ((d + 511) / 512) {
        case 1: AVD_LN3(1); break;
        case 2: AVD_LN3(2); break;
        case 3: AVD_LN3(3); break;
        default: AVD_LN3(4); break;
    }
#undef AVD_LN3
#undef AVD_LN3K
    AVD_CHECK_LAUNCH("layernorm_split3");
    return AVD_OK;
}

bool gemm_bf16x3_supported(int64_t M, int N, int K) { return M > 0 && N > 0 && N % 256 == 0 && K > 0 && K % 16 == 0; }
bool gemm_bf16x3_rownorm_supported(int N, int terms) { return N == 512 && terms == 3; }

int g_s3_tile = getenv("AVD_S3_TILE") ? atoi(getenv("AVD_S3_TILE")) : -1;
static int s3_tile_for(int epi, int64_t M, int N) {
    if (g_s3_tile == 0 || g_s3_tile == 1) return g_s3_tile;
    if (epi == S3_EPI_GELU_SPLIT || epi == S3_EPI_QKV3 || epi == S3_EPI_SPLIT) return 1;
    return (M + 255) / 256 * (N / 256) >= 192 ? 0 : 1;
}

int g_s3_stagger = getenv("AVD_S3_STAGGER") ? atoi(getenv("AVD_S3_STAGGER")) : -1;
thread_local bool t_s3_two_streams = false;
#ifdef AVD_S3_STAMPS
unsigned long long* g_s3_dbg = nullptr;
extern "C" void lab_set_dbg(unsigned long long* p) { g_s3_dbg = p; }
#endif

static int s3_cu_count() {
    static std::atomic<int> cache[64];
    int dev = 0;
    if (hipGetDevice(&dev) != hipSuccess) return 0;
    int n = dev < 64 ? cache[dev].load(std::memory_order_acquire) : 0;
    if (!n) {
        hipDeviceProp_t prop;
        if (hipGetDeviceProperties(&prop, dev) != hipSuccess) return 0;
        n = prop.multiProcessorCount;
        if (dev < 64) cache[dev].store(n, std::memory_order_release);
    }
    return n;
}

int g_s3_sn = getenv("AVD_S3_SN") ? atoi(getenv("AVD_S3_SN")) : 0;
int g_s3_super4 = getenv("AVD_S3_SUPER4") ? atoi(getenv("AVD_S3_SUPER4")) : 0;
int g_s3_super8 = getenv("AVD_S3_SUPER8") ? atoi(getenv("AVD_S3_SUPER8")) : 0;
static void s3_supertile(bool tile, int nbn, int& sn_out, int& sm_out) {
    int sn = 8;
    while (nbn % sn) sn >>= 1;
    if (tile && nbn <= 16) sn = nbn;
    int total = tile ? 32 : 16;
    if (tile && nbn >= 8 && nbn % 4 == 0) { sn = 4; total = 64; }
    if (g_s3_sn > 0) { sn = g_s3_sn < nbn ? g_s3_sn : nbn; while (nbn % sn) --sn; }
    if ((tile ? g_s3_super4 : g_s3_super8) > 0) total = tile ? g_s3_super4 : g_s3_super8;
    sn_out = sn;
    sm_out = total / sn > 0 ? total / sn : 1;
}

template <int EPI, int TERMS, int WAVES>
static int launch_s3w(S3Args g, hipStream_t st, int nz = 1) {
    using Cf = S3Cfg<TERMS, WAVES, EPI == S3_EPI_RES_NORM>;
    constexpr bool tile = WAVES == 4;
    static LdsAttr attr;
    auto kern = gemm_bf16x3_kernel<EPI, TERMS, WAVES>;
    if (int rc = attr.ensure(reinterpret_cast<const void*>(kern), Cf::LDS, "gemm_bf16x3")) return rc;
#ifdef AVD_S3_STAMPS
    g.dbg = g_s3_dbg;
#endif
    g.nbn = g.N / Cf::BN;
    s3_supertile(tile, g.nbn, g.sn, g.sm);
    const int64_t nbm = (g.M + Cf::BM - 1) / Cf::BM;
    const int64_t nwg = nbm * g.nbn;
    AVD_REQUIRE(nwg < (1ll << 31), AVD_EUNSUPPORTED, "gemm_bf16x3 grid too large");
    g.stagger = 0;
    g.first_gen = 2 * s3_cu_count();
    if (tile && g.first_gen > 0 && nbm * g.nbn >= 2 * g.first_gen)
        g.stagger = g_s3_stagger >= 0 ? g_s3_stagger : t_s3_two_streams ? 0 : (TERMS == 3 ? 24 : TERMS == 1 ? 12 : 48) * (g.K >= 1024 ? 2 : 1);
// ... 29 lines not shown
        g.stagger = g_s3_stagger >= 0 ? g_s3_stagger : t_s3_two_streams ? 0 : 48 * (g.K >= 1024 ? 2 : 1);
    static const int tag = prof_tag_id("gemm_bf16x3_m16_kernel<%d, %d, %d, %d>", EPI, WAVES, RT, NSTK);
    ProfScope prof(tag, 2.0 * (double)g.M * g.N * g.K, st);
    hipLaunchKernelGGL(kern, dim3((unsigned)nwg), dim3(WAVES * 64), LDS, st, g);
    AVD_CHECK_LAUNCH("gemm_bf16x3 (16x16x32)");
    return AVD_OK;
}

int g_s3_w128 = getenv("AVD_S3_W128") ? atoi(getenv("AVD_S3_W128")) : 1;
template <int EPI, int RT>
static int launch_s3w128(S3Args g, hipStream_t st) {
    constexpr int BM = 32 * RT, LDS = 3 * 6 * 256 * 32;
    static LdsAttr attr;
    auto kern = gemm_bf16x3_w128_kernel<EPI, RT>;
    if (int rc = attr.ensure(reinterpret_cast<const void*>(kern), LDS, "gemm_bf16x3 (128x128 wave tile)")) return rc;
#ifdef AVD_S3_STAMPS
    g.dbg = g_s3_dbg;
#endif
    g.nbn = g.N / 256;
    s3_supertile(false, g.nbn, g.sn, g.sm);
    const int64_t nbm = (g.M + BM - 1) / BM;
    const int64_t nwg = nbm * g.nbn;
    AVD_REQUIRE(nwg < (1ll << 31), AVD_EUNSUPPORTED, "gemm_bf16x3 grid too large");
    g.stagger = 0;
    g.first_gen = 0;
    static const int tag = prof_tag_id("gemm_bf16x3_w128_kernel<%d, %d>", EPI, RT);
    ProfScope prof(tag, 2.0 * (double)g.M * g.N * g.K, st);
    hipLaunchKernelGGL(kern, dim3((unsigned)nwg), dim3(256), LDS, st, g);
    AVD_CHECK_LAUNCH("gemm_bf16x3 (128x128 wave tile)");
    return AVD_OK;
}

int g_s3_rt4 = getenv("AVD_S3_RT4") ? atoi(getenv("AVD_S3_RT4")) : 0;
static int s3_rt4_for(int64_t M, int N, int rt_min) {
    if (g_s3_rt4 >= 2 && g_s3_rt4 <= 8) return g_s3_rt4 > rt_min ? g_s3_rt4 : rt_min;
    const int64_t cu = s3_cu_count() > 0 ? s3_cu_count() : 256, nbn = N / 128;
    int best = 8;
    int64_t cost8 = 0, cbest = 0;
    for (int rt = 8; rt >= rt_min; --rt) {
        const int64_t blocks = (M + 32 * rt - 1) / (32 * rt) * nbn, cost = (blocks + cu - 1) / cu * (rt + 3);
        if (rt == 8) cost8 = cbest = cost;
        else if (cost < cbest) { cbest = cost; best = rt; }
    }
    return cbest * 100 <= cost8 * 94 ? best : 8;
}
int g_s3_deep4 = getenv("AVD_S3_DEEP4") ? atoi(getenv("AVD_S3_DEEP4")) : 1;
static bool s3_deep4_for(int64_t M, int N, int rt) {
    const int64_t cu = s3_cu_count() > 0 ? s3_cu_count() : 256;
    return g_s3_deep4 != 0 && (M + 32 * rt - 1) / (32 * rt) * (N / 128) <= cu;
}

template <int EPI, int TERMS>
static int launch_s3t(const S3Args& a, hipStream_t st) {
    if constexpr (TERMS == 6 && EPI != S3_EPI_RES_NORM) {
        if (g_s3_m16) {
            if (s3_tile_for(EPI, a.M, a.N)) {
                if constexpr (EPI == S3_EPI_BIAS || EPI == S3_EPI_SPLIT) {
                    constexpr int E2 = EPI == S3_EPI_BIAS ? (int)S3_EPI_BIAS_REG : (int)S3_EPI_SPLIT;
                    const int rt = s3_rt4_for(a.M, a.N, 2);
                    if (a.bias && a.N % 128 == 0 && s3_deep4_for(a.M, a.N, rt)) {
                        switch (rt) {
                            case 2: return launch_s3w16<E2, 4, 2, 4>(a, st);
                            case 3: return launch_s3w16<E2, 4, 3, 4>(a, st);
                            case 4: return launch_s3w16<E2, 4, 4, 4>(a, st);
                            case 5: return launch_s3w16<E2, 4, 5, 4>(a, st);
                            case 6: return launch_s3w16<E2, 4, 6, 4>(a, st);
                            case 7: return launch_s3w16<E2, 4, 7, 4>(a, st);
                            default: return launch_s3w16<E2, 4, 8, 4>(a, st);
                        }
                    }
                }
                if constexpr (EPI == S3_EPI_RES_IMG) {
                    const int rt = s3_rt4_for(a.M, a.N, 2);
                    if (s3_deep4_for(a.M, a.N, rt)) {
                        switch (rt) {
                            case 2: return launch_s3w16<EPI, 4, 2, 4>(a, st);
                            case 3: return launch_s3w16<EPI, 4, 3, 4>(a, st);
                            case 4: return launch_s3w16<EPI, 4, 4, 4>(a, st);
                            case 5: return launch_s3w16<EPI, 4, 5, 4>(a, st);
                            case 6: return launch_s3w16<EPI, 4, 6, 4>(a, st);
                            case 7: return launch_s3w16<EPI, 4, 7, 4>(a, st);
                            default: return launch_s3w16<EPI, 4, 8, 4>(a, st);
                        }
                    }
                }
                if constexpr (EPI == S3_EPI_RES_IMG) {
                    switch (s3_rt4_for(a.M, a.N, 2)) {
                        case 2: return launch_s3w16<EPI, 4, 2>(a, st);
                        case 3: return launch_s3w16<EPI, 4, 3>(a, st);
                        case 4: return launch_s3w16<EPI, 4, 4>(a, st);
                        default: break;
                    }
                }
                if constexpr (EPI == S3_EPI_GELU_SPLIT || EPI == S3_EPI_QKV3 || EPI == S3_EPI_RES_IMG) {
                    switch (s3_rt4_for(a.M, a.N, 5)) {
                        case 5: return launch_s3w16<EPI, 4, 5>(a, st);
                        case 6: return launch_s3w16<EPI, 4, 6>(a, st);
                        case 7: return launch_s3w16<EPI, 4, 7>(a, st);
                        default: break;
                    }
                }
                return launch_s3w16<EPI, 4>(a, st);
            }
            constexpr bool TR = EPI == S3_EPI_GELU_SPLIT || EPI == S3_EPI_SPLIT || EPI == S3_EPI_QKV3 || EPI == S3_EPI_RES_IMG;
            bool rt7 = false, rt6 = false;
            if constexpr (EPI == S3_EPI_RES_IMG) {
                const int64_t cu = s3_cu_count() > 0 ? s3_cu_count() : 256, nbn = a.N / 256;
                const int64_t g8 = ((a.M + 255) / 256 * nbn + cu - 1) / cu * 8, g7 = ((a.M + 223) / 224 * nbn + cu - 1) / cu * 7;
                const int64_t g6 = ((a.M + 191) / 192 * nbn + cu - 1) / cu * 6;
                rt6 = g_s3_w128 && (g_s3_rt == 6 || (g_s3_rt == 0 && g6 < g7 && g6 < g8));
                rt7 = !rt6 && (g_s3_rt == 7 || (g_s3_rt != 8 && g7 < g8));
            }
            if constexpr (TR) {
                if (g_s3_w128) {
                    if constexpr (EPI == S3_EPI_RES_IMG) {
                        if (rt6) return launch_s3w128<EPI, 6>(a, st);
                    }
                    return rt7 ? launch_s3w128<EPI, 7>(a, st) : launch_s3w128<EPI, 8>(a, st);
                }
            }
            if constexpr (EPI == S3_EPI_RES_IMG) {
                if (rt7) return launch_s3w16<EPI, 8, 7>(a, st);
            }
            return launch_s3w16<EPI, 8>(a, st);
        }
    }
    if constexpr (EPI == S3_EPI_RES_NORM) {
        if constexpr (TERMS == 3) return launch_s3w<EPI, 3, 8>(a, st);
        else AVD_REQUIRE(false, AVD_EUNSUPPORTED, "gemm_bf16x3: the residual + RMSNorm epilogue exists for f16x2 images only");
    } else {
        return s3_tile_for(EPI, a.M, a.N) ? launch_s3w<EPI, TERMS, 4>(a, st) : launch_s3w<EPI, TERMS, 8>(a, st);
    }
}

template <int EPI>
static int launch_s3(const S3Args& a, hipStream_t st) {
    switch (a.terms) {
        case 0: case 6: return launch_s3t<EPI, 6>(a, st);
        case 9: return launch_s3t<EPI, 9>(a, st);
        case 1: return launch_s3t<EPI, 1>(a, st);
        case 3: return launch_s3t<EPI, 3>(a, st);
        default: return set_error(AVD_EINVAL, "gemm_bf16x3: terms must be 6 (default), 9 (strict), 1 (plain bf16) or 3 (f16x2), got %d", a.terms);
    }
}

bool gemm_bf16x3_resmap_supported(int terms) { return (terms == 0 || terms == 6) && g_s3_m16 != 0; }

int gemm_bf16x3(const void* A3, const void* W3, const float* bias, const float* R, float* C, void* C3, int64_t M, int N, int K,
                int act, int terms, hipStream_t st, float ab_scale, float c_scale, const float* ss_in, float eps, float* ss_out,
                const float* gamma, int r_seg, int r_stride) {
    AVD_REQUIRE(r_seg == 0 || (r_seg > 0 && r_stride >= r_seg && ss_out && gemm_bf16x3_resmap_supported(terms) && M < (1ll << 31)), AVD_EUNSUPPORTED,
                "gemm_bf16x3: a residual row map needs the fp32 + image residual epilogue of the six-term 16x16x32 kernels");
    AVD_REQUIRE(A3 && W3 && (C || C3), AVD_EINVAL, "gemm_bf16x3: null pointer");
    AVD_REQUIRE(!gamma || (gemm_bf16x3_rownorm_supported(N, terms) && C && C3 && R && bias && !ss_in && !ss_out && act == AVD_ACT_NONE && aligned16(gamma)),
                AVD_EUNSUPPORTED, "gemm_bf16x3: the residual + RMSNorm epilogue needs N == 512, f16x2 images, fp32 and image outputs, bias and residual");
    AVD_REQUIRE(!ss_in || (C3 && !C && K % 64 == 0), AVD_EUNSUPPORTED, "gemm_bf16x3: a folded norm needs an image output and K %% 64 == 0");
    AVD_REQUIRE(!ss_out || (C && C3 && R && bias && N % 64 == 0 && act == AVD_ACT_NONE && terms != 3), AVD_EUNSUPPORTED,
                "gemm_bf16x3: sums of squares are written by the fp32 + image residual epilogue only (bf16 planes)");
    AVD_REQUIRE(ab_scale > 0.f && ab_scale < __builtin_inff() && c_scale > 0.f && c_scale < __builtin_inff(), AVD_EINVAL,
                "gemm_bf16x3: image scales must be positive and finite");
    AVD_REQUIRE(gemm_bf16x3_supported(M, N, K), AVD_EUNSUPPORTED, "gemm_bf16x3: need N %% 256 == 0 and K %% 16 == 0 (M=%lld N=%d K=%d)",
                (long long)M, N, K);
    AVD_REQUIRE(aligned16(A3) && aligned16(W3) && aligned16(C) && aligned16(C3) && aligned16(bias) && aligned16(R), AVD_EUNSUPPORTED,
                "gemm_bf16x3: pointers must be 16-byte aligned");
    S3Args a{static_cast<const unsigned char*>(A3), static_cast<const unsigned char*>(W3), bias, R, C,
             static_cast<unsigned char*>(C3), M, N, K, 0, 0, 0, 0, 0, 0, 0.f, 0, 0, terms, 1.0f / ab_scale, c_scale,
             ss_in, ss_out, (float)sqrt((double)K), eps, gamma, r_seg, r_stride};
    if (gamma) {
        a.ss_sqrt_d = (float)sqrt((double)N);
        return launch_s3<S3_EPI_RES_NORM>(a, st);
    }
    if (C && C3) {
        AVD_REQUIRE(ss_out, AVD_EUNSUPPORTED, "gemm_bf16x3: fp32 and image output together imply the residual + sums-of-squares epilogue");
        return launch_s3<S3_EPI_RES_IMG>(a, st);
    }
    if (C3) {
        AVD_REQUIRE((act == AVD_ACT_GELU || act == AVD_ACT_NONE) && !R && bias, AVD_EUNSUPPORTED,
                    "gemm_bf16x3: image output implies bias, act NONE or GELU, no residual");
        return act == AVD_ACT_GELU ? launch_s3<S3_EPI_GELU_SPLIT>(a, st) : launch_s3<S3_EPI_SPLIT>(a, st);
    }
    AVD_REQUIRE(act == AVD_ACT_NONE, AVD_EUNSUPPORTED, "gemm_bf16x3: fp32 output supports act NONE only");
    if (R) {
        if ((terms == 0 || terms == 6) && g_s3_m16 && bias) return launch_s3<S3_EPI_RES_IMG>(a, st);
        return launch_s3<S3_EPI_RES>(a, st);
    }
    return launch_s3<S3_EPI_BIAS>(a, st);
}

template <bool IMG>
__global__ __launch_bounds__(256) void splitk_reduce_kernel(const float* __restrict__ part, int ns, const float* __restrict__ bias,
                                                            const float* R, float* C, unsigned char* __restrict__ C3,
                                                            float* __restrict__ ss, int64_t M, int N) {
    const int64_t i = (int64_t)blockIdx.x * 256 + threadIdx.x;
    const int per_row = N >> 3;
    const int64_t m = i / per_row;
    const int n = (int)(i % per_row) * 8;
    float v[8] = {0.f, 0.f, 0.f, 0.f, 0.f, 0.f, 0.f, 0.f};
    if (m < M) {
        const int64_t o = m * N + n;
        *reinterpret_cast<f32x4*>(v) = *reinterpret_cast<const f32x4*>(part + o);
        *reinterpret_cast<f32x4*>(v + 4) = *reinterpret_cast<const f32x4*>(part + o + 4);
        for (int z = 1; z < ns; ++z) {
            const float* pz = part + (int64_t)z * M * N + o;
            const f32x4 a = *reinterpret_cast<const f32x4*>(pz), b = *reinterpret_cast<const f32x4*>(pz + 4);
#pragma unroll
            for (int e = 0; e < 4; ++e) { v[e] += a[e]; v[4 + e] += b[e]; }
        }
        const f32x4 b0 = *reinterpret_cast<const f32x4*>(bias + n), b1 = *reinterpret_cast<const f32x4*>(bias + n + 4);
        const f32x4 r0 = *reinterpret_cast<const f32x4*>(R + o), r1 = *reinterpret_cast<const f32x4*>(R + o + 4);
#pragma unroll
        for (int e = 0; e < 4; ++e) { v[e] = (v[e] + b0[e]) + r0[e]; v[4 + e] = (v[4 + e] + b1[e]) + r1[e]; }
        *reinterpret_cast<f32x4*>(C + o) = f32x4{v[0], v[1], v[2], v[3]};
        *reinterpret_cast<f32x4*>(C + o + 4) = f32x4{v[4], v[5], v[6], v[7]};
        if constexpr (IMG) store_split8<true>(C3, m, n, N, v);
    }
    if constexpr (IMG) {
        float q = ((v[0] * v[0] + v[1] * v[1]) + (v[2] * v[2] + v[3] * v[3])) + ((v[4] * v[4] + v[5] * v[5]) + (v[6] * v[6] + v[7] * v[7]));
        q += __shfl_xor(q, 1, 64);
        q += __shfl_xor(q, 2, 64);
        q += __shfl_xor(q, 4, 64);
        if ((threadIdx.x & 7) == 0 && m < M) ss[m * (N >> 6) + (n >> 6)] = q;
    }
}

int g_s3_splitk = [] { const int v = getenv("AVD_S3_SPLITK") ? atoi(getenv("AVD_S3_SPLITK")) : 4; return v < 0 ? 0 : v > kS3SplitKMax ? kS3SplitKMax : v; }();
static bool splitk_shape_ok(int64_t M, int N, int K) {
    if (N % 128 || K % 32 || K / 2 < 512) return false;
    return (M + 255) / 256 * (N / 128) * 2 <= (int64_t)s3_cu_count();
}
int gemm_bf16x3_splitk_slices(int64_t M, int N, int K, int terms) {
    if (g_s3_splitk < 2 || terms == 3 || ((terms == 0 || terms == 6) && g_s3_m16) || !splitk_shape_ok(M, N, K)) return 0;
    const int64_t cu = s3_cu_count(), blocks = (M + 255) / 256 * (N / 128);
    int ns = 1;
    while (ns * 2 <= g_s3_splitk && blocks * ns * 2 <= cu && K % (32 * ns) == 0 && K / (ns * 2) >= 512) ns *= 2;
    return ns >= 2 ? ns : 0;
}
int64_t gemm_bf16x3_splitk_ws_floats(int64_t M, int N, int ns) { return (int64_t)ns * M * N; }
int64_t gemm_bf16x3_splitk_ws_max_floats(int64_t M, int N, int K) {
    return splitk_shape_ok(M, N, K) ? gemm_bf16x3_splitk_ws_floats(M, N, kS3SplitKMax) : 0;
}

int gemm_bf16x3_splitk(const void* A3, const void* W3, const float* bias, const float* R, float* C, void* C3, float* ss, int64_t M, int N,
                       int K, int terms, int ns, float* part, hipStream_t st) {
    AVD_REQUIRE(A3 && W3 && bias && R && C && part && ns >= 2, AVD_EINVAL, "gemm_bf16x3_splitk: null pointer");
    AVD_REQUIRE((C3 != nullptr) == (ss != nullptr), AVD_EINVAL, "gemm_bf16x3_splitk: the image and the sums of squares come together");
    AVD_REQUIRE(K % (16 * ns) == 0 && N % 128 == 0 && N % 64 == 0 && gemm_bf16x3_supported(M, N, K / ns), AVD_EUNSUPPORTED,
                "gemm_bf16x3_splitk: shape (M=%lld N=%d K=%d slices=%d)", (long long)M, N, K, ns);
    AVD_REQUIRE(aligned16(A3) && aligned16(W3) && aligned16(C) && aligned16(C3) && aligned16(bias) && aligned16(R) && aligned16(part),
                AVD_EUNSUPPORTED, "gemm_bf16x3_splitk: pointers must be 16-byte aligned");
    S3Args a{static_cast<const unsigned char*>(A3), static_cast<const unsigned char*>(W3), nullptr, nullptr, part, nullptr, M, N, K / ns,
             0, 0, 0, 0, 0, 0, 0.f, 0, 0, terms, 1.0f, 1.0f, nullptr, nullptr, 1.0f, 0.f, nullptr, 0, 0};
    int rc;
    switch (terms) {
        case 1: rc = launch_s3w<S3_EPI_BIAS, 1, 4>(a, st, ns); break;
        case 9: rc = launch_s3w<S3_EPI_BIAS, 9, 4>(a, st, ns); break;
        case 0: case 6: rc = launch_s3w<S3_EPI_BIAS, 6, 4>(a, st, ns); break;
        default: AVD_REQUIRE(false, AVD_EUNSUPPORTED, "gemm_bf16x3_splitk: bf16-plane modes only (terms %d)", terms);
    }
    if (rc) return rc;
    const int64_t threads = M * (N >> 3);
    static const int tag = prof_tag_id("splitk_reduce_kernel");
    ProfScope prof(tag, (double)M * N * 4.0 * (ns + 2) + (C3 ? (double)M * N * 6.0 : 0.0), st);
    if (C3)
        hipLaunchKernelGGL(splitk_reduce_kernel<true>, dim3((unsigned)((threads + 255) / 256)), dim3(256), 0, st, part, ns, bias, R, C,
                           static_cast<unsigned char*>(C3), ss, M, N);
    else
        hipLaunchKernelGGL(splitk_reduce_kernel<false>, dim3((unsigned)((threads + 255) / 256)), dim3(256), 0, st, part, ns, bias, R, C,
                           nullptr, nullptr, M, N);
    AVD_CHECK_LAUNCH("splitk_reduce");
    return AVD_OK;
}

int gemm_bf16x3_qkv3(const void* A3, const void* W3, const float* bias, void* img, int64_t M, int tokens, int heads, int K, float qscale,
                     int terms, hipStream_t st, float ab_scale, float c_scale, const float* ss_in, float eps) {
    AVD_REQUIRE(!ss_in || K % 64 == 0, AVD_EUNSUPPORTED, "gemm_bf16x3_qkv3: a folded norm needs K %% 64 == 0");
    AVD_REQUIRE(A3 && W3 && bias && img, AVD_EINVAL, "gemm_bf16x3_qkv3: null pointer");
    AVD_REQUIRE(ab_scale > 0.f && ab_scale < __builtin_inff() && c_scale > 0.f && c_scale < __builtin_inff(), AVD_EINVAL,
                "gemm_bf16x3_qkv3: image scales must be positive and finite");
    const int N = 3 * heads * 64;
    AVD_REQUIRE(tokens > 0 && heads > 0 && M > 0 && M % tokens == 0, AVD_EINVAL, "gemm_bf16x3_qkv3: rows %lld not a multiple of tokens %d",
                (long long)M, tokens);
    AVD_REQUIRE(M < (1ll << 31) - 256, AVD_EUNSUPPORTED, "gemm_bf16x3_qkv3: more than 2^31 rows");
    AVD_REQUIRE(gemm_bf16x3_supported(M, N, K), AVD_EUNSUPPORTED, "gemm_bf16x3_qkv3: need 3*heads*64 %% 256 == 0 and K %% 16 == 0");
    AVD_REQUIRE(aligned16(A3) && aligned16(W3) && aligned16(bias) && aligned16(img), AVD_EUNSUPPORTED, "gemm_bf16x3_qkv3: alignment");
    S3Args a{static_cast<const unsigned char*>(A3), static_cast<const unsigned char*>(W3), bias, nullptr, nullptr,
             static_cast<unsigned char*>(img), M, N, K, 0, 0, 0, tokens, qkv3_npad(tokens), heads, qscale, 0, 0, terms, 1.0f / ab_scale, c_scale,
             ss_in, nullptr, (float)sqrt((double)K), eps, nullptr, 0, 0};
    return launch_s3<S3_EPI_QKV3>(a, st);
}

}

using namespace avd;

extern "C" int64_t avd_split3_bytes(int64_t rows, int K) {
    if (rows <= 0 || K <= 0 || K % 16) return -1;
    return split3_bytes(rows, K);
}
extern "C" int avd_split3_f32(const float* x, void* out, int64_t rows, int K, avd_stream_t stream) {
    return split3_f32(x, K, out, rows, K, static_cast<hipStream_t>(stream));
}
extern "C" int avd_rmsnorm_split3_f32(const float* x, const float* scale, void* out, int64_t rows, int d, float eps,
                                      avd_stream_t stream) {
    return rmsnorm_split3_f32(x, scale, out, rows, d, eps, static_cast<hipStream_t>(stream));
}
extern "C" int avd_gemm_bf16x3_f32(const void* A3, const void* W3, const float* bias, const float* residual, float* C, void* C3,
                                   int64_t M, int N, int K, int act, int terms, avd_stream_t stream) {
    return gemm_bf16x3(A3, W3, bias, residual, C, C3, M, N, K, act, terms, static_cast<hipStream_t>(stream));
}
extern "C" int avd_gemm_bf16x3_qkv3_f32(const void* A3, const void* W3, const float* bias, void* qkv3, int64_t M, int tokens, int heads,
                                        int K, float qscale, int terms, avd_stream_t stream) {
    return gemm_bf16x3_qkv3(A3, W3, bias, qkv3, M, tokens, heads, K, qscale, terms, static_cast<hipStream_t>(stream));
}

extern "C" int avd_split_f16x2_f32(const float* x, void* out, int64_t rows, int K, float scale, avd_stream_t stream) {
    AVD_REQUIRE(scale > 0.f, AVD_EINVAL, "avd_split_f16x2_f32: scale must be positive");
    return split3_f32(x, K, out, rows, K, static_cast<hipStream_t>(stream), scale);
}
extern "C" int avd_rmsnorm_split_f16x2_f32(const float* x, const float* gamma, void* out, int64_t rows, int d, float eps, float scale,
                                           avd_stream_t stream) {
    AVD_REQUIRE(scale > 0.f, AVD_EINVAL, "avd_rmsnorm_split_f16x2_f32: scale must be positive");
    return rmsnorm_split3_f32(x, gamma, out, rows, d, eps, static_cast<hipStream_t>(stream), scale);
}
extern "C" int avd_gemm_f16x2_f32(const void* A2, const void* W2, const float* bias, const float* residual, float* C, void* C2, int64_t M,
                                  int N, int K, int act, float ab_scale, float c_scale, avd_stream_t stream) {
    return gemm_bf16x3(A2, W2, bias, residual, C, C2, M, N, K, act, 3, static_cast<hipStream_t>(stream), ab_scale, c_scale);
}
extern "C" int avd_gemm_f16x2_qkv_f32(const void* A2, const void* W2, const float* bias, void* qkv, int64_t M, int tokens, int heads, int K,
                                      float qscale, float ab_scale, float qkv_scale, avd_stream_t stream) {
    return gemm_bf16x3_qkv3(A2, W2, bias, qkv, M, tokens, heads, K, qscale, 3, static_cast<hipStream_t>(stream), ab_scale, qkv_scale);
}
```

### multimodal_diffusion_amd/csrc/s3_common.h

```cpp
#pragma once
#include "avd_common.h"

namespace avd {

#define AVD_LDS_PTR(p) ((__attribute__((address_space(3))) void*)(p))
#define AVD_GLB_PTR(p) ((const __attribute__((address_space(1))) void*)(p))

enum { S3_EPI_BIAS = 0, S3_EPI_RES = 2, S3_EPI_GELU_SPLIT = 3, S3_EPI_QKV3 = 4, S3_EPI_SPLIT = 5, S3_EPI_RES_IMG = 6, S3_EPI_RES_NORM = 7,
       S3_EPI_BIAS_REG = 8 };

struct S3Args {
    const unsigned char* A;
    const unsigned char* W;
    const float* bias;
    const float* R;
    float* C;
    unsigned char* C3;
    int64_t M;
    int N, K, nbn, sm, sn;
    int tokN, tokNpad, heads;
    float qscale;
    int stagger;
    int first_gen;
    int terms;
    float ab_inv, c_scale;
    const float* ss_in;
    float* ss_out;
    float ss_sqrt_d, ss_eps;
    const float* gamma;
    int r_seg, r_stride;
#ifdef AVD_S3_STAMPS
    unsigned long long* dbg;
#endif
};

#ifdef AVD_S3_STAMPS
#define S3_T() __builtin_amdgcn_s_memtime()
#define S3_RT() __builtin_amdgcn_s_memrealtime()
#define S3_DBG(i, v) do { if (threadIdx.x == 0) g.dbg[(size_t)blockIdx.x * 16 + (i)] = (v); } while (0)
#else
#define S3_T() 0ull
#define S3_RT() 0ull
#define S3_DBG(i, v) do { } while (0)
#endif

__device__ __forceinline__ void s3_block_of(const S3Args& g, int nbm, int& bm, int& bn) {
    const int b = blockIdx.x, nwg = gridDim.x, q = nwg >> 3, r = nwg & 7, x = b & 7;
    const int wg = (x < r ? x * (q + 1) : r * (q + 1) + (x - r) * q) + (b >> 3);
    const int per_row = g.sm * g.nbn;
    const int srow = wg / per_row, rem = wg - srow * per_row;
    const int left = nbm - srow * g.sm, h = left < g.sm ? left : g.sm;
    const int per_st = h * g.sn;
    const int sc = rem / per_st, rem2 = rem - sc * per_st;
    bm = srow * g.sm + rem2 / g.sn;
    bn = sc * g.sn + rem2 % g.sn;
}

template <int N> __device__ __forceinline__ void wait_vm() {
    static_assert(N >= 0 && N < 64, "vmcnt range");
    __builtin_amdgcn_s_waitcnt(0x0f70 | (N & 15) | ((N >> 4) << 14));
}

#ifdef AVD_LAB_NOSTORE
#define S3_ROW_OK(m) ((m) < g.M && __float_as_uint(v[0]) == 0x7fc12345u)
#else
#define S3_ROW_OK(m) ((m) < g.M)
#endif

typedef float f32x4t __attribute__((ext_vector_type(4)));

__device__ __forceinline__ f32x4t mma16x16(bf16x8 a, bf16x8 b, f32x4t c) { return __builtin_amdgcn_mfma_f32_16x16x32_bf16(a, b, c, 0, 0, 0); }

template <int EPI, int RT = 8>
__device__ __forceinline__ void s3_epilogue_img16(const S3Args& g, f32x4t (&acc)[8][4], int64_t mwave0, int nbase, int lane) {
    const int l15 = lane & 15, kq = lane >> 4;
    bool big = EPI == S3_EPI_RES_IMG;
    if constexpr (EPI != S3_EPI_RES_IMG && EPI != S3_EPI_BIAS_REG) {
        float amax = 0.f;
#pragma unroll
        for (int i = 0; i < 8; ++i) {
            float a = 0.f;
#pragma unroll
            for (int j = 0; j < 4; ++j)
#pragma unroll
                for (int r = 0; r < 4; ++r) a = fmaxf(a, fabsf(acc[i][j][r]));
            if (mwave0 + 16 * i + l15 < g.M) amax = fmaxf(amax, a);
        }
        float bmax = 0.f;
#pragma unroll
        for (int e = 0; e < 64; e += 4) {
            const f32x4 b4 = *reinterpret_cast<const f32x4*>(g.bias + nbase + e);
            bmax = fmaxf(fmaxf(bmax, fmaxf(fabsf(b4[0]), fabsf(b4[1]))), fmaxf(fabsf(b4[2]), fabsf(b4[3])));
        }
        big = __any(!(amax < 1.2676506e30f) || !(bmax < 1.2676506e30f) || !(fabsf(g.qscale) < 1.0e6f));
    }
    float bv[4][8];
#pragma unroll
    for (int j = 0; j < 4; ++j) {
        const float* bp = g.bias + nbase + 16 * j + 8 * (kq >> 1);
        *reinterpret_cast<f32x4*>(bv[j]) = *reinterpret_cast<const f32x4*>(bp);
        *reinterpret_cast<f32x4*>(bv[j] + 4) = *reinterpret_cast<const f32x4*>(bp + 4);
    }
    [[maybe_unused]] float mul = 1.0f;
    [[maybe_unused]] int64_t qbase = 0;
    if constexpr (EPI == S3_EPI_QKV3) {
        const int dmodel = g.heads * 64;
        const int part = nbase / dmodel, head = (nbase % dmodel) >> 6;
        mul = part == 0 ? g.qscale : 1.0f;
        qbase = (((int64_t)part * (g.M / g.tokN)) * g.heads + head) * (int64_t)g.tokNpad * QKV3_ROWB;
    }
#pragma unroll
    for (int ip = 0; ip < 4; ++ip) {
        const int tile = 2 * ip + (kq & 1);
        const int64_t m = (RT == 8 || tile < RT) ? mwave0 + 16 * tile + l15 : g.M;
        float rinv = 1.0f;
        if (EPI != S3_EPI_RES_IMG && EPI != S3_EPI_BIAS_REG && g.ss_in != nullptr && m < g.M) {
            const int nc = g.K >> 6;
            const float* sp = g.ss_in + m * nc;
            float ssum = 0.f;
            if (nc == 8) {
                const f32x4 p0 = *reinterpret_cast<const f32x4*>(sp), p1 = *reinterpret_cast<const f32x4*>(sp + 4);
                const f32x4 t = p0 + p1;
                ssum = (t[0] + t[1]) + (t[2] + t[3]);
            } else {
                for (int c = 0; c < nc; ++c) ssum += sp[c];
            }
            rinv = 1.0f / (sqrtf(ssum) / g.ss_sqrt_d + g.ss_eps);
        }
        [[maybe_unused]] unsigned char* qrow = nullptr;
        [[maybe_unused]] int qsw = 0;
        if constexpr (EPI == S3_EPI_QKV3) {
            const unsigned b = (unsigned)m / (unsigned)g.tokN, tok = (unsigned)m - b * (unsigned)g.tokN;
            qrow = g.C3 + qbase + ((int64_t)b * g.heads * g.tokNpad + tok) * QKV3_ROWB;
            qsw = qkv3_swizzle(nbase / (g.heads * 64), (int)tok);
        }
        [[maybe_unused]] float ssq = 0.f;
        [[maybe_unused]] int64_t rrow = m;
        if constexpr (EPI == S3_EPI_RES_IMG) {
            if (g.r_seg > 0 && m < g.M) {
                const unsigned sgi = (unsigned)m / (unsigned)g.r_seg;
                rrow = (int64_t)sgi * g.r_stride + ((unsigned)m - sgi * (unsigned)g.r_seg);
            }
        }
#pragma unroll
        for (int j = 0; j < 4; ++j) {
            float v[8];
#pragma unroll
            for (int r = 0; r < 4; ++r) {
                const auto sw = __builtin_amdgcn_permlane16_swap(__float_as_uint(acc[2 * ip][j][r]), __float_as_uint(acc[2 * ip + 1][j][r]), false, false);
                v[r] = __uint_as_float(sw[0]);
                v[4 + r] = __uint_as_float(sw[1]);
            }
            const int n = nbase + 16 * j + 8 * (kq >> 1);
            if constexpr (EPI == S3_EPI_QKV3) {
#pragma unroll
                for (int e = 0; e < 8; ++e) v[e] = fmaf(v[e], rinv, bv[j][e]) * mul;
                if (S3_ROW_OK(m)) {
                    const int c = 2 * j + (kq >> 1);
                    unsigned char* dst = qrow + ((c ^ qsw) << 4);
                    u32x4 Hh, Mi, Lo;
                    if (big) split8<true>(v, Hh, Mi, Lo);
                    else split8<false>(v, Hh, Mi, Lo);
                    *reinterpret_cast<u32x4*>(dst) = Hh;
                    *reinterpret_cast<u32x4*>(dst + 128) = Mi;
                    *reinterpret_cast<u32x4*>(dst + 256) = Lo;
                }
            } else if constexpr (EPI == S3_EPI_BIAS_REG) {
                if (S3_ROW_OK(m)) {
#pragma unroll
                    for (int e = 0; e < 8; ++e) v[e] += bv[j][e];
                    float* cp = g.C + m * g.N + n;
                    *reinterpret_cast<f32x4*>(cp) = f32x4{v[0], v[1], v[2], v[3]};
                    *reinterpret_cast<f32x4*>(cp + 4) = f32x4{v[4], v[5], v[6], v[7]};
                }
            } else if constexpr (EPI == S3_EPI_RES_IMG) {
                if (S3_ROW_OK(m)) {
                    const float* rp = g.R + rrow * g.N + n;
                    const f32x4 r0 = *reinterpret_cast<const f32x4*>(rp), r1 = *reinterpret_cast<const f32x4*>(rp + 4);
#pragma unroll
                    for (int e = 0; e < 8; ++e) v[e] = (v[e] + bv[j][e]) + (e < 4 ? r0[e] : r1[e - 4]);
                    float* cp = g.C + m * g.N + n;
                    *reinterpret_cast<f32x4*>(cp) = f32x4{v[0], v[1], v[2], v[3]};
                    *reinterpret_cast<f32x4*>(cp + 4) = f32x4{v[4], v[5], v[6], v[7]};
                    ssq += ((v[0] * v[0] + v[1] * v[1]) + (v[2] * v[2] + v[3] * v[3])) + ((v[4] * v[4] + v[5] * v[5]) + (v[6] * v[6] + v[7] * v[7]));
                    if (g.C3) store_split8<true>(g.C3, m, n, g.N, v);
                }
            } else {
#pragma unroll
                for (int e = 0; e < 8; ++e) {
                    const float t = fmaf(v[e], rinv, bv[j][e]);
                    v[e] = EPI == S3_EPI_GELU_SPLIT ? gelu_erf(t) : t;
                }
                if (S3_ROW_OK(m)) {
                    if (big) store_split8<true>(g.C3, m, n, g.N, v);
                    else store_split8<false>(g.C3, m, n, g.N, v);
                }
            }
        }
        if constexpr (EPI == S3_EPI_RES_IMG) {
            const float tot = ssq + __shfl_xor(ssq, 32, 64);
            if (kq < 2 && m < g.M && g.ss_out) g.ss_out[m * (g.N >> 6) + (nbase >> 6)] = tot;
        }
    }
}

}
```

### multimodal_diffusion_amd/csrc/tokens.hip

```cpp
#include "avd_common.h"

#include <stdlib.h>

namespace avd {

__global__ void temb_kernel(const int64_t* __restrict__ t, const float* __restrict__ freqs, float* __restrict__ out,
                            int B, int dim, float neg_log_mp) {
    const int half = dim >> 1;
    const int i = blockIdx.x * blockDim.x + threadIdx.x;
    if (i >= B * dim) return;
    const int b = i / dim, c = i % dim;
    float v = 0.f;
    if (c < 2 * half) {
        const int k = c < half ? c : c - half;
        const float f = freqs ? freqs[k] : expf(neg_log_mp * (float)k / (float)half);
        const float a = (float)t[b] * f;
        v = c < half ? cosf(a) : sinf(a);
    }
    out[i] = v;
}

int temb_f32(const int64_t* t, const float* freqs, float* out, int B, int dim, float max_period, hipStream_t st) {
    AVD_REQUIRE(t && out, AVD_EINVAL, "timestep_embedding: null pointer");
    AVD_REQUIRE(B > 0 && dim > 0 && max_period > 0.f, AVD_EINVAL, "timestep_embedding: bad dims");
// ... 338 lines not shown
    AVD_REQUIRE(len > 0 && stride > 0 && F >= len, AVD_EUNSUPPORTED, "cfg_untoken_ddim_audio: bad chunking");
    AVD_REQUIRE(eta >= 0.f && (eta == 0.f || noise), AVD_EINVAL, "cfg_untoken_ddim_audio: eta > 0 needs noise");
    AVD_REQUIRE(z != z_out, AVD_EINVAL, "cfg_untoken_ddim_audio: z_out must not alias z");
    const int Na = audio_na(F, len, stride);
    const int64_t n = (int64_t)B * Ca * F;
    hipLaunchKernelGGL(cfg_untoken_ddim_audio_kernel, dim3((unsigned)((n + 255) / 256)), dim3(256), 0, st, eps2, z, t_now,
                       t_prev, abar, T_train, guidance, eta, noise, z_out, B, Ca, F, len, stride, Na);
    AVD_CHECK_LAUNCH("cfg_untoken_ddim_audio");
    return AVD_OK;
}

__global__ __launch_bounds__(256) void assemble_kernel(float* __restrict__ X2, const float* __restrict__ temb,
                                                       const float* __restrict__ Xp, int B, int N, int d, int tdim,
                                                       int Nt, int Np, int target_first, int64_t total4) {
    const int64_t i = (int64_t)blockIdx.x * 256 + threadIdx.x;
    if (i >= total4) return;
    const int d4 = d >> 2;
    const int col = (int)(i % d4) * 4;
    const int64_t row = i / d4;
    const int n = (int)(row % N);
    const int bb = (int)(row / N);
    const int half = bb >= B, b = half ? bb - B : bb;
    const int t0 = target_first ? 0 : Np;
    const bool is_t = n >= t0 && n < t0 + Nt;
    f32x4 v;
    if (is_t) {
        if (col >= d - tdim) {
            v = *reinterpret_cast<const f32x4*>(temb + (int64_t)b * tdim + (col - (d - tdim)));
        } else {
            if (!half) return;
            v = *reinterpret_cast<const f32x4*>(X2 + ((int64_t)b * N + n) * d + col);
        }
    } else {
        const int np = target_first ? n - Nt : n;
        v = half ? f32x4{0.f, 0.f, 0.f, 0.f} : *reinterpret_cast<const f32x4*>(Xp + ((int64_t)b * Np + np) * d + col);
    }
    *reinterpret_cast<f32x4*>(X2 + row * d + col) = v;
}

int assemble_f32(float* X2, const float* temb, const float* Xp, int B, int N, int d, int tdim, int Nt, int Np,
                 int target_first, hipStream_t st) {
    const int64_t total4 = (int64_t)2 * B * N * (d >> 2);
    static const int tag = prof_tag_id("assemble_kernel");
    ProfScope prof(tag, 4.0 * (2.0 * B * N * d + (double)B * Nt * (d - tdim) + (double)B * Np * d), st);
    hipLaunchKernelGGL(assemble_kernel, dim3((unsigned)((total4 + 255) / 256)), dim3(256), 0, st, X2, temb, Xp, B, N, d,
                       tdim, Nt, Np, target_first, total4);
    AVD_CHECK_LAUNCH("assemble");
    return AVD_OK;
}

__global__ __launch_bounds__(256) void assemble_rows_kernel(float* __restrict__ X2, const int64_t* __restrict__ t_now,
                                                            const float* __restrict__ freqs, const float* __restrict__ Xp,
                                                            float* __restrict__ ss, int B, int N, int d, int tdim, int Nt, int Np,
                                                            int target_first, float neg_log_mp) {
    const int lane = threadIdx.x & 63;
    const int64_t row = (int64_t)blockIdx.x * 4 + (threadIdx.x >> 6);
    if (row >= (int64_t)2 * B * N) return;
    const int n = (int)(row % N);
    const int bb = (int)(row / N);
    const int half = bb >= B, b = half ? bb - B : bb;
    const int t0 = target_first ? 0 : Np;
    const bool is_t = n >= t0 && n < t0 + Nt;
    const int da = d - tdim, th = tdim >> 1;
    const float tf = is_t ? (float)t_now[b] : 0.f;
    float acc = 0.f;
    for (int col = lane * 4; col < d; col += 256) {
        f32x4 v;
        bool store = true;
        if (is_t) {
            if (col >= da) {
#pragma unroll
                for (int e = 0; e < 4; ++e) {
                    const int c = col - da + e;
                    float x = 0.f;
                    if (c < 2 * th) {
                        const int k = c < th ? c : c - th;
                        const float f = freqs ? freqs[k] : expf(neg_log_mp * (float)k / (float)th);
                        const float a = tf * f;
                        x = c < th ? cosf(a) : sinf(a);
                    }
                    v[e] = x;
                }
            } else {
                v = *reinterpret_cast<const f32x4*>(X2 + ((int64_t)b * N + n) * d + col);
                store = half != 0;
            }
        } else {
            const int np = target_first ? n - Nt : n;
            v = half ? f32x4{0.f, 0.f, 0.f, 0.f} : *reinterpret_cast<const f32x4*>(Xp + ((int64_t)b * Np + np) * d + col);
        }
        if (store) *reinterpret_cast<f32x4*>(X2 + row * d + col) = v;
        acc += v[0] * v[0] + v[1] * v[1] + v[2] * v[2] + v[3] * v[3];
    }
    acc = wave_sum(acc);
    if (ss && lane == 0) ss[row] = acc;
}

int assemble_rows_f32(float* X2, const int64_t* t_now, const float* freqs, const float* Xp, float* ss, int B, int N, int d, int tdim,
                      int Nt, int Np, int target_first, float max_period, hipStream_t st) {
    const int64_t rows = (int64_t)2 * B * N;
    static const int tag = prof_tag_id("assemble_rows_kernel");
    ProfScope prof(tag, 4.0 * (2.0 * B * N * d + (double)B * Nt * (d - tdim) + (double)B * Np * d), st);
    hipLaunchKernelGGL(assemble_rows_kernel, dim3((unsigned)((rows + 3) / 4)), dim3(256), 0, st, X2, t_now, freqs, Xp, ss, B, N, d, tdim,
                       Nt, Np, target_first, -(float)log((double)max_period));
    AVD_CHECK_LAUNCH("assemble_rows");
    return AVD_OK;
}

__global__ void sched_advance_kernel(const int64_t* __restrict__ sched, int n_sched, int32_t* cursor,
                                     int64_t* __restrict__ t_now, int64_t* __restrict__ t_prev, int B) {
    __shared__ int cur;
    if (threadIdx.x == 0) cur = *cursor;
    __syncthreads();
    int i = cur;
    if (i < 0) i = 0;
    if (i > n_sched - 2) i = n_sched - 2;
    const int64_t a = sched[i], p = sched[i + 1];
    for (int b = threadIdx.x; b < B; b += blockDim.x) {
        t_now[b] = a;
        t_prev[b] = p;
    }
    __syncthreads();
    if (threadIdx.x == 0) *cursor = cur + 1;
}

}

using namespace avd;

extern "C" int avd_timestep_embedding_f32(const int64_t* t, const float* freqs, float* out, int B, int dim,
                                          float max_period, avd_stream_t stream) {
    return temb_f32(t, freqs, out, B, dim, max_period, static_cast<hipStream_t>(stream));
}
extern "C" int avd_tube_patch_f32(const float* z, float* tok, int B, int C, int T, int H, int W, int t, int h, int w,
                                  avd_stream_t stream) {
    AVD_REQUIRE(aligned16(z) && aligned16(tok), AVD_EUNSUPPORTED, "tube_patch: pointers must be 16-byte aligned");
    return tube_patch_f32(z, tok, B, C, T, H, W, t, h, w, static_cast<hipStream_t>(stream));
}
extern "C" int avd_tube_unpatch_f32(const float* tok, float* z, int B, int C, int T, int H, int W, int t, int h, int w,
                                    avd_stream_t stream) {
    AVD_REQUIRE(aligned16(z) && aligned16(tok), AVD_EUNSUPPORTED, "tube_unpatch: pointers must be 16-byte aligned");
    return tube_unpatch_f32(tok, z, B, C, T, H, W, t, h, w, static_cast<hipStream_t>(stream));
}
extern "C" int avd_audio_tokens_f32(const float* z, float* tok, int B, int Ca, int F, int len, int stride,
                                    avd_stream_t stream) {
    return audio_tokens_f32(z, tok, B, Ca, F, len, stride, static_cast<hipStream_t>(stream));
}
extern "C" int avd_audio_untokens_f32(const float* tok, const float* window, float* z, int B, int Ca, int F, int len, int stride,
                                      avd_stream_t stream) {
    return audio_untokens_f32(tok, window, z, B, Ca, F, len, stride, static_cast<hipStream_t>(stream));
}
extern "C" int avd_ddim_step_f32(const float* x_t, const float* eps_hat, const int64_t* t_now, const int64_t* t_prev,
                                 const float* alpha_bar, int T_train, float eta, const float* noise, float* x_prev,
                                 int B, int64_t per_sample, avd_stream_t stream) {
    return ddim_step_f32(x_t, eps_hat, t_now, t_prev, alpha_bar, T_train, eta, noise, x_prev, B, per_sample,
                         static_cast<hipStream_t>(stream));
}
// ... 25 lines not shown
```

Baseline: 117.6 steps/s.

## Collapse identical null-prompt rows in the CFG unconditional half

In the null (unconditional) CFG half every prompt token row holds the same zero embedding. The change therefore keeps only one representative row per sample, packing the null half into N-Np+1 rows. The QKV GEMM epilogue then refills the collapsed span in the attention image, and attention output rows are remapped, with collapsed duplicates skipped. The intent is to cut GEMM, norm and assemble work on the redundant null-prompt rows (about 37 of 421 tokens in half the batch). The cost is extra indexing logic, a span-fill kernel, and correctness resting on those rows staying identical through the layers.

```diff
diff --git a/multimodal_diffusion_amd/csrc/attn_bf16x3.hip b/multimodal_diffusion_amd/csrc/attn_bf16x3.hip
--- a/multimodal_diffusion_amd/csrc/attn_bf16x3.hip
+++ b/multimodal_diffusion_amd/csrc/attn_bf16x3.hip
@@ -21,10 +21,18 @@
 template <> struct A3Terms<1> { static constexpr int N = 1; static constexpr int PA[1] = {0}; static constexpr int PB[1] = {0}; };
 template <> struct A3Terms<3> { static constexpr int N = 3; static constexpr int PA[3] = {0, 1, 0}; static constexpr int PB[3] = {1, 0, 0}; };
 
+__device__ __forceinline__ int64_t a3_out_row(int b, int q, int out_tok, RowCollapse cl, int Bt) {
+    if (!cl.on() || b < cl.b0) return (int64_t)b * out_tok + q;
+    const int64_t base = (int64_t)cl.b0 * out_tok;
+    if (q == cl.p0) return base + (b - cl.b0);
+    if (q > cl.p0 && q < cl.p0 + cl.np) return -1;
+    return base + (Bt - cl.b0) + (int64_t)(b - cl.b0) * (out_tok - cl.np) + (q < cl.p0 ? q : q - cl.np);
+}
+
 template <bool SPLIT_OUT, int TERMS>
 __global__ __launch_bounds__(A3_NW * 64, 2) void attn_bf16x3_kernel(const unsigned char* __restrict__ img, float* __restrict__ out,
                                                                     int Bt, int N, int Npad, int H, int n_query, int nqb,
-                                                                    float s_inv2, float v_inv, float o_scale, int out_tok) {
+                                                                    float s_inv2, float v_inv, float o_scale, int out_tok, RowCollapse cl) {
     constexpr int NW = A3_NW, ROWB = QKV3_ROWB;
     constexpr bool F16 = TERMS == 3;
     constexpr int NPL = s3_planes(TERMS);
@@ -48,6 +56,7 @@
     const unsigned char* Vb = img + (((int64_t)2 * Bt + b) * H + h) * hstride;
 
     const int q_row = qb * (NW * 32) + wave * 32 + l31;
+    const int64_t orow = a3_out_row(b, q_row, out_tok, cl, Bt);
     bf16x8 qf[4][3];
     {
         const unsigned char* src = Qb + (int64_t)(q_row < N ? q_row : N - 1) * ROWB + hi * 16;
@@ -225,13 +234,13 @@
                 v[e] = hi ? recv : ch[c][e];
                 v[4 + e] = hi ? ch[c + 1][e] : recv;
             }
-            if (q_row < n_query) {
-                if constexpr (F16) store_split8_h2(o3, (int64_t)b * out_tok + q_row, h * A3_DH + 8 * (c + hi), d, v, o_scale);
-                else store_split8(o3, (int64_t)b * out_tok + q_row, h * A3_DH + 8 * (c + hi), d, v);
-            }
-        }
-    } else if (q_row < n_query) {
-        float* dst = out + ((int64_t)b * out_tok + q_row) * d + h * A3_DH + 4 * hi;
+            if (q_row < n_query && orow >= 0) {
+                if constexpr (F16) store_split8_h2(o3, orow, h * A3_DH + 8 * (c + hi), d, v, o_scale);
+                else store_split8(o3, orow, h * A3_DH + 8 * (c + hi), d, v);
+            }
+        }
+    } else if (q_row < n_query && orow >= 0) {
+        float* dst = out + orow * d + h * A3_DH + 4 * hi;
 #pragma unroll
         for (int g4 = 0; g4 < 4; ++g4) {
             f32x4 a = {o0[4 * g4] * inv, o0[4 * g4 + 1] * inv, o0[4 * g4 + 2] * inv, o0[4 * g4 + 3] * inv};
@@ -251,7 +260,7 @@
 template <bool SPLIT_OUT, int TERMS>
 __global__ __launch_bounds__(A3_NW * 64, 2) void attn_bf16x3_pipe_kernel(const unsigned char* __restrict__ img, float* __restrict__ out,
                                                                          int Bt, int N, int Npad, int H, int n_query, int nqb,
-                                                                         float s_inv2, float v_inv, float o_scale, int out_tok) {
+                                                                         float s_inv2, float v_inv, float o_scale, int out_tok, RowCollapse cl) {
     constexpr int NW = A3_NW, ROWB = QKV3_ROWB;
     constexpr bool F16 = TERMS == 3;
     constexpr int NPL = s3_planes(TERMS);
@@ -277,6 +286,7 @@
     const unsigned char* Vb = img + (((int64_t)2 * Bt + b) * H + h) * hstride;
 
     const int q_row = qb * (NW * 32) + wave * 32 + l31;
+    const int64_t orow = a3_out_row(b, q_row, out_tok, cl, Bt);
     bf16x8 qf[4][3];
     {
         const unsigned char* src = Qb + (int64_t)(q_row < N ? q_row : N - 1) * ROWB + hi * 16;
@@ -552,13 +562,13 @@
                 v[e] = hi ? recv : ch[c][e];
                 v[4 + e] = hi ? ch[c + 1][e] : recv;
             }
-            if (q_row < n_query) {
-                if constexpr (F16) store_split8_h2(o3, (int64_t)b * out_tok + q_row, h * A3_DH + 8 * (c + hi), d, v, o_scale);
-                else store_split8(o3, (int64_t)b * out_tok + q_row, h * A3_DH + 8 * (c + hi), d, v);
-            }
-        }
-    } else if (q_row < n_query) {
-        float* dst = out + ((int64_t)b * out_tok + q_row) * d + h * A3_DH + 4 * hi;
+            if (q_row < n_query && orow >= 0) {
+                if constexpr (F16) store_split8_h2(o3, orow, h * A3_DH + 8 * (c + hi), d, v, o_scale);
+                else store_split8(o3, orow, h * A3_DH + 8 * (c + hi), d, v);
+            }
+        }
+    } else if (q_row < n_query && orow >= 0) {
+        float* dst = out + orow * d + h * A3_DH + 4 * hi;
 #pragma unroll
         for (int g4 = 0; g4 < 4; ++g4) {
             f32x4 a = {o0[4 * g4] * inv, o0[4 * g4 + 1] * inv, o0[4 * g4 + 2] * inv, o0[4 * g4 + 3] * inv};
@@ -581,7 +591,7 @@
 template <bool SPLIT_OUT, int TERMS>
 __global__ __launch_bounds__(A3_NW * 64, 2) void attn_bf16x3_p16_kernel(const unsigned char* __restrict__ img, float* __restrict__ out,
                                                                         int Bt, int N, int Npad, int H, int n_query, int nqb,
-                                                                        float s_inv2, float v_inv, float o_scale, int out_tok) {
+                                                                        float s_inv2, float v_inv, float o_scale, int out_tok, RowCollapse cl) {
     constexpr int NW = A3_NW, ROWB = QKV3_ROWB;
     constexpr bool F16 = TERMS == 3;
     constexpr int NPL = s3_planes(TERMS);
@@ -893,6 +903,7 @@
     }
     const int d = H * A3_DH;
     const int q_row = q_row0 + 16 * (kq & 1);
+    const int64_t orow = a3_out_row(b, q_row, out_tok, cl, Bt);
     unsigned char* o3 = reinterpret_cast<unsigned char*>(out);
 #pragma unroll
     for (int dt = 0; dt < 4; ++dt) {
@@ -904,12 +915,12 @@
             v[4 + r] = __uint_as_float(sw[1]);
         }
         const int col = h * A3_DH + 16 * dt + 8 * (kq >> 1);
-        if (q_row < n_query) {
+        if (q_row < n_query && orow >= 0) {
             if constexpr (SPLIT_OUT) {
-                if constexpr (F16) store_split8_h2(o3, (int64_t)b * out_tok + q_row, col, d, v, o_scale);
-                else store_split8(o3, (int64_t)b * out_tok + q_row, col, d, v);
+                if constexpr (F16) store_split8_h2(o3, orow, col, d, v, o_scale);
+                else store_split8(o3, orow, col, d, v);
             } else {
-                float* dst = out + ((int64_t)b * out_tok + q_row) * d + col;
+                float* dst = out + orow * d + col;
                 *reinterpret_cast<f32x4*>(dst) = f32x4{v[0], v[1], v[2], v[3]};
                 *reinterpret_cast<f32x4*>(dst + 4) = f32x4{v[4], v[5], v[6], v[7]};
             }
@@ -921,37 +932,39 @@
 
 template <int TERMS>
 static void attn3_launch(const unsigned char* img, float* out, void* out3, int B, int N, int Npad, int H, int n_query, int nqb, hipStream_t st,
-                         float img_scale, float out_scale, int out_tok) {
+                         float img_scale, float out_scale, int out_tok, RowCollapse cl) {
     const float s_inv2 = 1.0f / (img_scale * img_scale), v_inv = 1.0f / img_scale;
     if (g_attn_m16 && (TERMS == 6 || TERMS == 9 || g_attn_m16 == 2)) {
         if (out3)
             hipLaunchKernelGGL((attn_bf16x3_p16_kernel<true, TERMS>), dim3(nqb * H * B), dim3(A3_NW * 64), 0, st, img, static_cast<float*>(out3),
-                               B, N, Npad, H, n_query, nqb, s_inv2, v_inv, out_scale, out_tok);
+                               B, N, Npad, H, n_query, nqb, s_inv2, v_inv, out_scale, out_tok, cl);
         else
             hipLaunchKernelGGL((attn_bf16x3_p16_kernel<false, TERMS>), dim3(nqb * H * B), dim3(A3_NW * 64), 0, st, img, out, B, N, Npad, H,
-                               n_query, nqb, s_inv2, v_inv, out_scale, out_tok);
+                               n_query, nqb, s_inv2, v_inv, out_scale, out_tok, cl);
         return;
     }
     if (g_attn_pipe == 2 || (g_attn_pipe == 1 && (TERMS == 6 || TERMS == 9))) {
         if (out3)
             hipLaunchKernelGGL((attn_bf16x3_pipe_kernel<true, TERMS>), dim3(nqb * H * B), dim3(A3_NW * 64), 0, st, img, static_cast<float*>(out3),
-                               B, N, Npad, H, n_query, nqb, s_inv2, v_inv, out_scale, out_tok);
+                               B, N, Npad, H, n_query, nqb, s_inv2, v_inv, out_scale, out_tok, cl);
         else
             hipLaunchKernelGGL((attn_bf16x3_pipe_kernel<false, TERMS>), dim3(nqb * H * B), dim3(A3_NW * 64), 0, st, img, out, B, N, Npad, H,
-                               n_query, nqb, s_inv2, v_inv, out_scale, out_tok);
+                               n_query, nqb, s_inv2, v_inv, out_scale, out_tok, cl);
         return;
     }
     if (out3)
         hipLaunchKernelGGL((attn_bf16x3_kernel<true, TERMS>), dim3(nqb * H * B), dim3(A3_NW * 64), 0, st, img, static_cast<float*>(out3), B, N,
-                           Npad, H, n_query, nqb, s_inv2, v_inv, out_scale, out_tok);
+                           Npad, H, n_query, nqb, s_inv2, v_inv, out_scale, out_tok, cl);
     else
         hipLaunchKernelGGL((attn_bf16x3_kernel<false, TERMS>), dim3(nqb * H * B), dim3(A3_NW * 64), 0, st, img, out, B, N, Npad, H, n_query, nqb,
-                           s_inv2, v_inv, out_scale, out_tok);
+                           s_inv2, v_inv, out_scale, out_tok, cl);
 }
 
 int attn_bf16x3(const void* qkv3, float* out, void* out3, int B, int N, int H, int n_query, int terms, hipStream_t st, float img_scale,
-                float out_scale, int out_tokens) {
+                float out_scale, int out_tokens, RowCollapse cl) {
     const int out_tok = out_tokens > 0 ? out_tokens : N;
+    AVD_REQUIRE(!cl.on() || (out_tok == N && cl.b0 >= 0 && cl.b0 < B && cl.p0 >= 0 && cl.p0 + cl.np <= N), AVD_EINVAL,
+                "attn_bf16x3: collapsed output rows need out_tokens == N and a span inside the sample");
     AVD_REQUIRE(out_tok >= n_query, AVD_EINVAL, "attn_bf16x3: out_tokens=%d < n_query=%d", out_tok, n_query);
     AVD_REQUIRE(terms == 0 || terms == 6 || terms == 9 || terms == 1 || terms == 3, AVD_EINVAL, "attn_bf16x3: terms must be 6, 9, 1 or 3, got %d", terms);
     AVD_REQUIRE(img_scale > 0.f && img_scale < __builtin_inff() && out_scale > 0.f && out_scale < __builtin_inff() &&
@@ -968,10 +981,10 @@
     ProfScope prof(tag, 4.0 * (double)B * H * (double)n_query * N * A3_DH, st);
     const int Npad = qkv3_npad(N);
     const auto* img = static_cast<const unsigned char*>(qkv3);
-    if (terms == 9) attn3_launch<9>(img, out, out3, B, N, Npad, H, n_query, nqb, st, 1.f, 1.f, out_tok);
-    else if (terms == 1) attn3_launch<1>(img, out, out3, B, N, Npad, H, n_query, nqb, st, 1.f, 1.f, out_tok);
-    else if (terms == 3) attn3_launch<3>(img, out, out3, B, N, Npad, H, n_query, nqb, st, img_scale, out_scale, out_tok);
-    else attn3_launch<6>(img, out, out3, B, N, Npad, H, n_query, nqb, st, 1.f, 1.f, out_tok);
+    if (terms == 9) attn3_launch<9>(img, out, out3, B, N, Npad, H, n_query, nqb, st, 1.f, 1.f, out_tok, cl);
+    else if (terms == 1) attn3_launch<1>(img, out, out3, B, N, Npad, H, n_query, nqb, st, 1.f, 1.f, out_tok, cl);
+    else if (terms == 3) attn3_launch<3>(img, out, out3, B, N, Npad, H, n_query, nqb, st, img_scale, out_scale, out_tok, cl);
+    else attn3_launch<6>(img, out, out3, B, N, Npad, H, n_query, nqb, st, 1.f, 1.f, out_tok, cl);
     AVD_CHECK_LAUNCH("attn_bf16x3");
     return AVD_OK;
 }
diff --git a/multimodal_diffusion_amd/csrc/avd_common.h b/multimodal_diffusion_amd/csrc/avd_common.h
--- a/multimodal_diffusion_amd/csrc/avd_common.h
+++ b/multimodal_diffusion_amd/csrc/avd_common.h
@@ -72,6 +72,11 @@
     __host__ __device__ __forceinline__ int64_t off(int64_t r) const {
         return seg > 0 ? (r / seg) * stride + (r % seg) * ld : r * ld;
     }
+};
+
+struct RowCollapse {
+    int b0 = 0, p0 = 0, np = 0;
+    __host__ __device__ __forceinline__ bool on() const { return np > 1; }
 };
 
 struct TubeGather {
@@ -253,17 +258,20 @@
 extern int g_s3_sn, g_s3_super4, g_s3_super8;
 extern int g_s3_tile;
 extern thread_local bool t_s3_two_streams;
+extern thread_local int64_t t_s3_plan_rows;
 int gemm_bf16x3_qkv3(const void* A3, const void* W3, const float* bias, void* img, int64_t M, int tokens, int heads, int K, float qscale,
-                     int terms, hipStream_t st, float ab_scale = 1.f, float c_scale = 1.f, const float* ss_in = nullptr, float eps = 0.f);
+                     int terms, hipStream_t st, float ab_scale = 1.f, float c_scale = 1.f, const float* ss_in = nullptr, float eps = 0.f,
+                     RowCollapse cl = {}, int samples = 0, bool share = false);
 int64_t qkv3_bytes(int B, int N, int H);
 int64_t attn_fp8_ws_bytes(int B, int N, int H);
 int attn_fp8(const void* qkv3, void* ws, int64_t ws_bytes, float* out, void* out3, int B, int N, int H, int n_query, hipStream_t st,
              int img_terms = 6, float img_scale = 1.f, float out_scale = 1.f);
 int attn_bf16x3(const void* qkv3, float* out, void* out3, int B, int N, int H, int n_query, int terms, hipStream_t st,
-                float img_scale = 1.f, float out_scale = 1.f, int out_tokens = 0);
+                float img_scale = 1.f, float out_scale = 1.f, int out_tokens = 0, RowCollapse cl = {});
 int gemm_bf16x3(const void* A3, const void* W3, const float* bias, const float* R, float* C, void* C3, int64_t M, int N, int K,
                 int act, int terms, hipStream_t st, float ab_scale = 1.f, float c_scale = 1.f, const float* ss_in = nullptr, float eps = 0.f,
-                float* ss_out = nullptr, const float* gamma = nullptr, int r_seg = 0, int r_stride = 0);
+                float* ss_out = nullptr, const float* gamma = nullptr, int r_seg = 0, int r_stride = 0, int r_split = 0, int r_stride2 = 0,
+                int r_skip2 = 0);
 bool gemm_bf16x3_resmap_supported(int terms);
 bool gemm_bf16x3_rownorm_supported(int N, int terms);
 extern int g_s3_splitk;
diff --git a/multimodal_diffusion_amd/csrc/composite.hip b/multimodal_diffusion_amd/csrc/composite.hip
--- a/multimodal_diffusion_amd/csrc/composite.hip
+++ b/multimodal_diffusion_amd/csrc/composite.hip
@@ -71,7 +71,7 @@
 int assemble_f32(float* X2, const float* temb, const float* Xp, int B, int N, int d, int tdim, int Nt, int Np,
                  int target_first, hipStream_t st);
 int assemble_rows_f32(float* X2, const int64_t* t_now, const float* freqs, const float* Xp, float* ss, int B, int N, int d, int tdim,
-                      int Nt, int Np, int target_first, float max_period, hipStream_t st);
+                      int Nt, int Np, int target_first, float max_period, hipStream_t st, int collapse);
 int cfg_unpatch_ddim_f32(const float* eps2, const float* z, const int64_t* t_now, const int64_t* t_prev,
                          const float* abar, int T_train, float guidance, float eta, const float* noise, float* z_out,
                          int B, int C, int T, int H, int W, int t, int h, int w, hipStream_t st);
@@ -144,6 +144,8 @@
 
 static bool g_core_trim = getenv("AVD_CORE_TRIM") ? atoi(getenv("AVD_CORE_TRIM")) != 0 : true;
 static int64_t core_trim_floats(const avd_core_weights* w, int B, int N) { return (int64_t)B * N * w->d; }
+
+static bool g_null_dedup = getenv("AVD_NULL_DEDUP") ? atoi(getenv("AVD_NULL_DEDUP")) != 0 : true;
 
 static int64_t core_split_wide_bytes(const avd_core_weights* w, int B, int N) {
     const int64_t qkv3 = qkv3_bytes(B, N, w->n_heads), fc1 = split3_bytes((int64_t)B * N, w->mlp_hidden);
@@ -193,13 +195,26 @@
     return layernorm_act_f32(x, scale, bias, y, M, w->d, w->norm_eps, AVD_ACT_NONE, st);
 }
 
+static bool core_trim_ok(const avd_core_weights* w, int N, int out_row0, int n_out_rows) {
+    return g_core_trim && out_row0 == 0 && n_out_rows < N && w->attn_mode == 0 && gemm_bf16x3_resmap_supported(w->split_terms);
+}
+static bool core_forward_collapse_ok(const avd_core_weights* w, int B, int N, int out_row0, int n_out_rows, RowCollapse cl) {
+    return !check_core(w) && cl.on() && cl.b0 > 0 && cl.b0 < B && cl.p0 >= 0 && cl.p0 + cl.np <= N && n_out_rows <= cl.p0 &&
+           core_use_split(w, (int64_t)B * N) && core_use_split_fold(w) && core_trim_ok(w, N, out_row0, n_out_rows);
+}
+
 static int core_forward(const avd_core_weights* w, const float* x, float* y, int B, int N, int out_row0,
                         int n_out_rows, const unsigned char* kpm, void* ws, int64_t ws_bytes, hipStream_t st,
-                        const float* ss_first = nullptr) {
+                        const float* ss_first = nullptr, RowCollapse cl = {}, bool share0 = false) {
     if (int rc = check_core(w)) return rc;
     AVD_REQUIRE(x && y && B > 0 && N > 0, AVD_EINVAL, "core: bad input");
     AVD_REQUIRE(out_row0 >= 0 && n_out_rows > 0 && out_row0 + n_out_rows <= N, AVD_EINVAL, "core: bad output row window");
     const int64_t M = (int64_t)B * N;
+    AVD_REQUIRE(!cl.on() || (!kpm && core_forward_collapse_ok(w, B, N, out_row0, n_out_rows, cl)), AVD_EUNSUPPORTED,
+                "core: a collapsed null half needs the folded split path with the last-block trim and the span after the output window");
+    const int64_t Mr = cl.on() ? M - (int64_t)(B - cl.b0) * (cl.np - 1) : M;
+    AVD_REQUIRE(!share0 || (cl.on() && B == 2 * cl.b0), AVD_EINVAL, "core: share0 needs a collapsed CFG pair (B == 2 cl.b0)");
+    const int64_t M0 = share0 ? (int64_t)cl.b0 * N + cl.b0 : Mr;
     AVD_REQUIRE(ws && ws_bytes >= core_ws_bytes(w, B, N), AVD_EWORKSPACE, "core: workspace %lld < %lld bytes",
                 (long long)ws_bytes, (long long)core_ws_bytes(w, B, N));
     const int d = w->d, hid = w->mlp_hidden, H = w->n_heads;
@@ -228,22 +243,28 @@
             float* ss = cs.take(M * (d / 64));
             const int ns = gemm_bf16x3_splitk_slices(M, d, hid, terms);
             float* part = ns ? cs.take(gemm_bf16x3_splitk_ws_floats(M, d, ns)) : nullptr;
-            const bool trim = g_core_trim && out_row0 == 0 && n_out_rows < N && w->attn_mode == 0 && gemm_bf16x3_resmap_supported(terms);
+            const bool trim = core_trim_ok(w, N, out_row0, n_out_rows);
             float* yc = cs.take(core_trim_floats(w, B, N));
             const bool fused = g_mlp_fused && !ns && mlp_bf16x3_supported(d, hid, terms) && gemm_bf16x3_resmap_supported(terms);
             AVD_REQUIRE(cs.ok, AVD_EWORKSPACE, "core: workspace carve %lld > %lld bytes", (long long)cs.used, (long long)cs.cap);
-            if (int rc = split3_rows_f32(cur, rd, hx, M, d, st, 0.f, ss)) return rc;
+            struct PlanRows {
+                explicit PlanRows(int64_t r) { t_s3_plan_rows = r; }
+                ~PlanRows() { t_s3_plan_rows = 0; }
+            } plan(cl.on() ? M : 0);
+            if (int rc = split3_rows_f32(cur, rd, hx, M0, d, st, 0.f, ss)) return rc;
+            const int r_split = cl.on() ? cl.b0 : 0, r_stride2 = cl.on() ? N - cl.np : 0, r_skip2 = cl.on() ? B - cl.b0 : 0;
             for (int l = 0; l < w->n_layers; ++l) {
                 const avd_block_weights& b = w->blocks[l];
                 const bool last = l == w->n_layers - 1;
                 const int nq = (last && out_row0 == 0) ? n_out_rows : N;
                 if (last && trim) {
                     const int64_t Mc = (int64_t)B * nq;
-                    if (int rc = gemm_bf16x3_qkv3(hx, b.in_proj_weight3n, b.in_proj_bias, qkv, M, N, H, d, scale * 1.4426950408889634f, terms, st,
-                                                  1.f, 1.f, ss, w->norm_eps)) return rc;
+                    if (int rc = gemm_bf16x3_qkv3(hx, b.in_proj_weight3n, b.in_proj_bias, qkv, l == 0 ? M0 : Mr, N, H, d, scale * 1.4426950408889634f,
+                                                  terms, st, 1.f, 1.f, ss, w->norm_eps, cl, B, l == 0 && share0)) return rc;
                     if (int rc = attn_bf16x3(qkv, nullptr, hs, B, N, H, nq, terms, st, 1.f, 1.f, nq)) return rc;
+                    t_s3_plan_rows = 0;
                     if (int rc = gemm_bf16x3(hs, b.out_proj_weight3, b.out_proj_bias, cur, yc, hx, Mc, d, d, AVD_ACT_NONE, terms, st, 1.f, 1.f,
-                                             nullptr, 0.f, ss, nullptr, nq, N)) return rc;
+                                             nullptr, 0.f, ss, nullptr, nq, N, r_split, r_stride2, r_skip2)) return rc;
                     if (fused) {
                         if (int rc = mlp_bf16x3(hx, b.fc1_weight3n, b.fc1_bias, b.fc2_weight3, b.fc2_bias, ss, w->norm_eps, yc, yc, nullptr, nullptr, Mc,
                                                 d, hid, st)) return rc;
@@ -259,34 +280,34 @@
                     }
                     return rmsnorm_f32(yc, rd, w->final_norm_scale, y, RowMap{d, nq, (int64_t)N * d}, Mc, d, w->norm_eps, st);
                 }
-                if (int rc = gemm_bf16x3_qkv3(hx, b.in_proj_weight3n, b.in_proj_bias, qkv, M, N, H, d, scale * 1.4426950408889634f, terms, st,
-                                              1.f, 1.f, ss, w->norm_eps)) return rc;
+                if (int rc = gemm_bf16x3_qkv3(hx, b.in_proj_weight3n, b.in_proj_bias, qkv, l == 0 ? M0 : Mr, N, H, d, scale * 1.4426950408889634f,
+                                              terms, st, 1.f, 1.f, ss, w->norm_eps, cl, B, l == 0 && share0)) return rc;
                 if (w->attn_mode == 1) {
                     if (int rc = attn_fp8(qkv, f8w, f8_b, nullptr, hs, B, N, H, nq, st, terms, 1.f, 1.f)) return rc;
                 } else {
-                    if (int rc = attn_bf16x3(qkv, nullptr, hs, B, N, H, nq, terms, st, 1.f, 1.f)) return rc;
+                    if (int rc = attn_bf16x3(qkv, nullptr, hs, B, N, H, nq, terms, st, 1.f, 1.f, 0, cl)) return rc;
                 }
-                if (int rc = gemm_bf16x3(hs, b.out_proj_weight3, b.out_proj_bias, cur, y, hx, M, d, d, AVD_ACT_NONE, terms, st, 1.f, 1.f, nullptr,
+                if (int rc = gemm_bf16x3(hs, b.out_proj_weight3, b.out_proj_bias, cur, y, hx, Mr, d, d, AVD_ACT_NONE, terms, st, 1.f, 1.f, nullptr,
                                          0.f, ss)) return rc;
                 cur = y;
                 if (fused) {
                     if (int rc = mlp_bf16x3(hx, b.fc1_weight3n, b.fc1_bias, b.fc2_weight3, b.fc2_bias, ss, w->norm_eps, y, y, last ? nullptr : hx,
-                                            last ? nullptr : ss, M, d, hid, st)) return rc;
+                                            last ? nullptr : ss, Mr, d, hid, st)) return rc;
                     continue;
                 }
-                if (int rc = gemm_bf16x3(hx, b.fc1_weight3n, b.fc1_bias, nullptr, nullptr, wide3, M, hid, d, AVD_ACT_GELU, terms, st, 1.f, 1.f, ss,
+                if (int rc = gemm_bf16x3(hx, b.fc1_weight3n, b.fc1_bias, nullptr, nullptr, wide3, Mr, hid, d, AVD_ACT_GELU, terms, st, 1.f, 1.f, ss,
                                          w->norm_eps)) return rc;
                 if (ns) {
-                    if (int rc = gemm_bf16x3_splitk(wide3, b.fc2_weight3, b.fc2_bias, y, y, last ? nullptr : hx, last ? nullptr : ss, M, d, hid,
+                    if (int rc = gemm_bf16x3_splitk(wide3, b.fc2_weight3, b.fc2_bias, y, y, last ? nullptr : hx, last ? nullptr : ss, Mr, d, hid,
                                                     terms, ns, part, st)) return rc;
                 } else if (last) {
-                    if (int rc = gemm_bf16x3(wide3, b.fc2_weight3, b.fc2_bias, y, y, nullptr, M, d, hid, AVD_ACT_NONE, terms, st)) return rc;
+                    if (int rc = gemm_bf16x3(wide3, b.fc2_weight3, b.fc2_bias, y, y, nullptr, Mr, d, hid, AVD_ACT_NONE, terms, st)) return rc;
                 } else {
-                    if (int rc = gemm_bf16x3(wide3, b.fc2_weight3, b.fc2_bias, y, y, hx, M, d, hid, AVD_ACT_NONE, terms, st, 1.f, 1.f, nullptr, 0.f,
+                    if (int rc = gemm_bf16x3(wide3, b.fc2_weight3, b.fc2_bias, y, y, hx, Mr, d, hid, AVD_ACT_NONE, terms, st, 1.f, 1.f, nullptr, 0.f,
                                              ss)) return rc;
                 }
             }
-            return rmsnorm_f32(y, rd, w->final_norm_scale, y, rd, M, d, w->norm_eps, st);
+            return rmsnorm_f32(y, rd, w->final_norm_scale, y, rd, Mr, d, w->norm_eps, st);
         }
         const bool rown = core_use_split_rownorm(w);
         void* hn = rown ? cs.take((split3_bytes(M, d) + 3) / 4) : hs;
@@ -481,7 +502,8 @@
 }
 
 static int embed_cfg_pair(const avd_embed_desc* e, const float* z, const float* Wt, const float* bt,
-                          const int64_t* t_now, const float* Xp, float* tok_ws, float* X2, hipStream_t st, float* ss_out = nullptr) {
+                          const int64_t* t_now, const float* Xp, float* tok_ws, float* X2, hipStream_t st, float* ss_out = nullptr,
+                          int collapse = 0) {
     if (int rc = check_embed(e)) return rc;
     AVD_REQUIRE(z && Wt && t_now && tok_ws && X2 && (e->Np == 0 || Xp), AVD_EINVAL, "embed: null pointer");
     const int B = e->B, d = e->d, N = e->Nt + e->Np, D = embed_tok_dim(e);
@@ -498,6 +520,7 @@
         if (int rc = temb_f32(t_now, e->temb_freqs, temb, B, e->tdim, 10000.f, st)) return rc;
     float* c0 = X2 + (e->target_first ? 0 : (int64_t)e->Np * d);
     const RowMap cm{d, e->Nt, (int64_t)N * d};
+    AVD_REQUIRE(!(collapse && e->temb_add), AVD_EUNSUPPORTED, "embed: the collapsed null half needs the concat embedding");
     if (e->temb_add) {
         const RowMap rm{0, e->Nt, (int64_t)e->tdim};
         if (int rc = gemm_f32(tok, RowMap{D, 0, 0}, Wt, bt, temb, rm, c0, cm, (int64_t)B * e->Nt, d, D, AVD_ACT_NONE, st)) return rc;
@@ -509,7 +532,7 @@
     } else {
         if (int rc = gemm_f32(tok, RowMap{D, 0, 0}, Wt, bt, nullptr, cm, c0, cm, (int64_t)B * e->Nt, d - e->tdim, D, AVD_ACT_NONE, st)) return rc;
     }
-    return assemble_rows_f32(X2, t_now, e->temb_freqs, Xp, ss_out, B, N, d, e->tdim, e->Nt, e->Np, e->target_first, 10000.f, st);
+    return assemble_rows_f32(X2, t_now, e->temb_freqs, Xp, ss_out, B, N, d, e->tdim, e->Nt, e->Np, e->target_first, 10000.f, st, collapse);
 }
 
 #define AVD_HIP(call)                                                                        \
@@ -607,6 +630,7 @@
     }
     if (!strcmp(key, "s3_min_rows")) { g_s3_min_rows = value; return AVD_OK; }
     if (!strcmp(key, "no_fold")) { g_no_fold = value != 0; return AVD_OK; }
+    if (!strcmp(key, "null_dedup")) { g_null_dedup = value != 0; return AVD_OK; }
     return set_error(AVD_EINVAL, "tune_set: unknown key '%s'", key);
 }
 
@@ -681,11 +705,15 @@
     float* eps2 = reinterpret_cast<float*>(w + p.x2 + p.tok + p.core + p.head + p.ss);
     const bool have_ss = !e.temb_add;
 
-    if (int rc = embed_cfg_pair(&e, z, s->adapt_w, s->adapt_b, t_now, Xp, tok, X2, st, ssx)) return rc;
     const int row0 = e.target_first ? 0 : e.Np;
+    const RowCollapse cl{e.B, e.target_first ? e.Nt : 0, e.Np};
+    const bool dedup = g_null_dedup && !s->split_streams && !e.temb_add && cl.on() &&
+                       core_forward_collapse_ok(s->core, 2 * e.B, p.N, row0, e.Nt, cl);
+    if (int rc = embed_cfg_pair(&e, z, s->adapt_w, s->adapt_b, t_now, Xp, tok, X2, st, ssx, dedup)) return rc;
     const RowMap hm{e.d, e.Nt, (int64_t)p.N * e.d};
     if (!s->split_streams) {
-        if (int rc = core_forward(s->core, X2, X2, 2 * e.B, p.N, row0, e.Nt, nullptr, core_ws, p.core, st, have_ss ? ssx : nullptr)) return rc;
+        if (int rc = core_forward(s->core, X2, X2, 2 * e.B, p.N, row0, e.Nt, nullptr, core_ws, p.core, st, have_ss ? ssx : nullptr,
+                                  dedup ? cl : RowCollapse{}, dedup)) return rc;
         if (int rc = head_forward(s->head, X2 + (int64_t)row0 * e.d, hm, p.rows, eps2, head_ws, p.head, st)) return rc;
     } else {
         AuxState ax;
diff --git a/multimodal_diffusion_amd/csrc/gemm_bf16x3.hip b/multimodal_diffusion_amd/csrc/gemm_bf16x3.hip
--- a/multimodal_diffusion_amd/csrc/gemm_bf16x3.hip
+++ b/multimodal_diffusion_amd/csrc/gemm_bf16x3.hip
@@ -209,7 +209,7 @@
         const int dmodel = g.heads * 64;
         const int part = nbase / dmodel, head = (nbase % dmodel) >> 6;
         mul = part == 0 ? g.qscale : 1.0f;
-        qbase = (((int64_t)part * (g.M / g.tokN)) * g.heads + head) * (int64_t)g.tokNpad * QKV3_ROWB;
+        qbase = (((int64_t)part * qkv3_samples(g)) * g.heads + head) * (int64_t)g.tokNpad * QKV3_ROWB;
     }
 #pragma unroll
     for (int i = 0; i < 4; ++i) {
@@ -230,8 +230,11 @@
         }
         [[maybe_unused]] unsigned char* qrow = nullptr;
         [[maybe_unused]] int qsw = 0;
+        [[maybe_unused]] int64_t qdup = -1;
         if constexpr (EPI == S3_EPI_QKV3) {
-            const unsigned b = (unsigned)m / (unsigned)g.tokN, tok = (unsigned)m - b * (unsigned)g.tokN;
+            unsigned b, tok;
+            qkv3_row_of(g, m, b, tok);
+            qdup = qkv3_share_off(g, b, tok);
             const int dmodel = g.heads * 64;
             qrow = g.C3 + qbase + ((int64_t)b * g.heads * g.tokNpad + tok) * QKV3_ROWB;
             qsw = qkv3_swizzle(nbase / dmodel, (int)tok);
@@ -259,6 +262,10 @@
                             split8_h2(v, g.c_scale, Hh, Lo);
                             *reinterpret_cast<u32x4*>(dst) = Hh;
                             *reinterpret_cast<u32x4*>(dst + 128) = Lo;
+                            if (qdup >= 0) {
+                                *reinterpret_cast<u32x4*>(dst + qdup) = Hh;
+                                *reinterpret_cast<u32x4*>(dst + qdup + 128) = Lo;
+                            }
                         } else {
                             u32x4 Hh, Mi, Lo;
                             if (big) split8<true>(v, Hh, Mi, Lo);
@@ -266,6 +273,11 @@
                             *reinterpret_cast<u32x4*>(dst) = Hh;
                             *reinterpret_cast<u32x4*>(dst + 128) = Mi;
                             *reinterpret_cast<u32x4*>(dst + 256) = Lo;
+                            if (qdup >= 0) {
+                                *reinterpret_cast<u32x4*>(dst + qdup) = Hh;
+                                *reinterpret_cast<u32x4*>(dst + qdup + 128) = Mi;
+                                *reinterpret_cast<u32x4*>(dst + qdup + 256) = Lo;
+                            }
                         }
                     }
                 } else if constexpr (EPI == S3_EPI_RES_IMG) {
@@ -1256,6 +1268,7 @@
 
 int g_s3_stagger = getenv("AVD_S3_STAGGER") ? atoi(getenv("AVD_S3_STAGGER")) : -1;
 thread_local bool t_s3_two_streams = false;
+thread_local int64_t t_s3_plan_rows = 0;
 #ifdef AVD_S3_STAMPS
 unsigned long long* g_s3_dbg = nullptr;
 extern "C" void lab_set_dbg(unsigned long long* p) { g_s3_dbg = p; }
@@ -1391,13 +1404,14 @@
 
 template <int EPI, int TERMS>
 static int launch_s3t(const S3Args& a, hipStream_t st) {
+    const int64_t Mp = t_s3_plan_rows > 0 ? t_s3_plan_rows : a.M;
     if constexpr (TERMS == 6 && EPI != S3_EPI_RES_NORM) {
         if (g_s3_m16) {
-            if (s3_tile_for(EPI, a.M, a.N)) {
+            if (s3_tile_for(EPI, Mp, a.N)) {
                 if constexpr (EPI == S3_EPI_BIAS || EPI == S3_EPI_SPLIT) {
                     constexpr int E2 = EPI == S3_EPI_BIAS ? (int)S3_EPI_BIAS_REG : (int)S3_EPI_SPLIT;
-                    const int rt = s3_rt4_for(a.M, a.N, 2);
-                    if (a.bias && a.N % 128 == 0 && s3_deep4_for(a.M, a.N, rt)) {
+                    const int rt = s3_rt4_for(Mp, a.N, 2);
+                    if (a.bias && a.N % 128 == 0 && s3_deep4_for(Mp, a.N, rt)) {
                         switch (rt) {
                             case 2: return launch_s3w16<E2, 4, 2, 4>(a, st);
                             case 3: return launch_s3w16<E2, 4, 3, 4>(a, st);
@@ -1410,8 +1424,8 @@
                     }
                 }
                 if constexpr (EPI == S3_EPI_RES_IMG) {
-                    const int rt = s3_rt4_for(a.M, a.N, 2);
-                    if (s3_deep4_for(a.M, a.N, rt)) {
+                    const int rt = s3_rt4_for(Mp, a.N, 2);
+                    if (s3_deep4_for(Mp, a.N, rt)) {
                         switch (rt) {
                             case 2: return launch_s3w16<EPI, 4, 2, 4>(a, st);
                             case 3: return launch_s3w16<EPI, 4, 3, 4>(a, st);
@@ -1424,7 +1438,7 @@
                     }
                 }
                 if constexpr (EPI == S3_EPI_RES_IMG) {
-                    switch (s3_rt4_for(a.M, a.N, 2)) {
+                    switch (s3_rt4_for(Mp, a.N, 2)) {
                         case 2: return launch_s3w16<EPI, 4, 2>(a, st);
                         case 3: return launch_s3w16<EPI, 4, 3>(a, st);
                         case 4: return launch_s3w16<EPI, 4, 4>(a, st);
@@ -1432,7 +1446,7 @@
                     }
                 }
                 if constexpr (EPI == S3_EPI_GELU_SPLIT || EPI == S3_EPI_QKV3 || EPI == S3_EPI_RES_IMG) {
-                    switch (s3_rt4_for(a.M, a.N, 5)) {
+                    switch (s3_rt4_for(Mp, a.N, 5)) {
                         case 5: return launch_s3w16<EPI, 4, 5>(a, st);
                         case 6: return launch_s3w16<EPI, 4, 6>(a, st);
                         case 7: return launch_s3w16<EPI, 4, 7>(a, st);
@@ -1445,8 +1459,8 @@
             bool rt7 = false, rt6 = false;
             if constexpr (EPI == S3_EPI_RES_IMG) {
                 const int64_t cu = s3_cu_count() > 0 ? s3_cu_count() : 256, nbn = a.N / 256;
-                const int64_t g8 = ((a.M + 255) / 256 * nbn + cu - 1) / cu * 8, g7 = ((a.M + 223) / 224 * nbn + cu - 1) / cu * 7;
-                const int64_t g6 = ((a.M + 191) / 192 * nbn + cu - 1) / cu * 6;
+                const int64_t g8 = ((Mp + 255) / 256 * nbn + cu - 1) / cu * 8, g7 = ((Mp + 223) / 224 * nbn + cu - 1) / cu * 7;
+                const int64_t g6 = ((Mp + 191) / 192 * nbn + cu - 1) / cu * 6;
                 rt6 = g_s3_w128 && (g_s3_rt == 6 || (g_s3_rt == 0 && g6 < g7 && g6 < g8));
                 rt7 = !rt6 && (g_s3_rt == 7 || (g_s3_rt != 8 && g7 < g8));
             }
@@ -1468,7 +1482,7 @@
         if constexpr (TERMS == 3) return launch_s3w<EPI, 3, 8>(a, st);
         else AVD_REQUIRE(false, AVD_EUNSUPPORTED, "gemm_bf16x3: the residual + RMSNorm epilogue exists for f16x2 images only");
     } else {
-        return s3_tile_for(EPI, a.M, a.N) ? launch_s3w<EPI, TERMS, 4>(a, st) : launch_s3w<EPI, TERMS, 8>(a, st);
+        return s3_tile_for(EPI, Mp, a.N) ? launch_s3w<EPI, TERMS, 4>(a, st) : launch_s3w<EPI, TERMS, 8>(a, st);
     }
 }
 
@@ -1487,9 +1501,11 @@
 
 int gemm_bf16x3(const void* A3, const void* W3, const float* bias, const float* R, float* C, void* C3, int64_t M, int N, int K,
                 int act, int terms, hipStream_t st, float ab_scale, float c_scale, const float* ss_in, float eps, float* ss_out,
-                const float* gamma, int r_seg, int r_stride) {
+                const float* gamma, int r_seg, int r_stride, int r_split, int r_stride2, int r_skip2) {
     AVD_REQUIRE(r_seg == 0 || (r_seg > 0 && r_stride >= r_seg && ss_out && gemm_bf16x3_resmap_supported(terms) && M < (1ll << 31)), AVD_EUNSUPPORTED,
                 "gemm_bf16x3: a residual row map needs the fp32 + image residual epilogue of the six-term 16x16x32 kernels");
+    AVD_REQUIRE(r_split == 0 || (r_seg > 0 && r_split > 0 && r_stride2 >= r_seg && r_skip2 >= 0), AVD_EINVAL,
+                "gemm_bf16x3: bad two-stride residual row map");
     AVD_REQUIRE(A3 && W3 && (C || C3), AVD_EINVAL, "gemm_bf16x3: null pointer");
     AVD_REQUIRE(!gamma || (gemm_bf16x3_rownorm_supported(N, terms) && C && C3 && R && bias && !ss_in && !ss_out && act == AVD_ACT_NONE && aligned16(gamma)),
                 AVD_EUNSUPPORTED, "gemm_bf16x3: the residual + RMSNorm epilogue needs N == 512, f16x2 images, fp32 and image outputs, bias and residual");
@@ -1504,7 +1520,7 @@
                 "gemm_bf16x3: pointers must be 16-byte aligned");
     S3Args a{static_cast<const unsigned char*>(A3), static_cast<const unsigned char*>(W3), bias, R, C,
              static_cast<unsigned char*>(C3), M, N, K, 0, 0, 0, 0, 0, 0, 0.f, 0, 0, terms, 1.0f / ab_scale, c_scale,
-             ss_in, ss_out, (float)sqrt((double)K), eps, gamma, r_seg, r_stride};
+             ss_in, ss_out, (float)sqrt((double)K), eps, gamma, r_seg, r_stride, r_split, r_stride2, r_skip2};
     if (gamma) {
         a.ss_sqrt_d = (float)sqrt((double)N);
         return launch_s3<S3_EPI_RES_NORM>(a, st);
@@ -1610,14 +1626,40 @@
     return AVD_OK;
 }
 
+__global__ __launch_bounds__(256) void qkv3_span_fill_kernel(unsigned char* __restrict__ img, int samples, int heads, int npad, RowCollapse cl,
+                                                             int64_t chunks) {
+    const int64_t i = (int64_t)blockIdx.x * 256 + threadIdx.x;
+    if (i >= chunks) return;
+    constexpr int CPR = QKV3_ROWB / 16;
+    const int k = (int)(i % CPR);
+    int64_t t = i / CPR;
+    const int r = 1 + (int)(t % (cl.np - 1));
+    t /= cl.np - 1;
+    const int h = (int)(t % heads);
+    t /= heads;
+    const int nb = samples - cl.b0;
+    const int b = cl.b0 + (int)(t % nb), part = 1 + (int)(t / nb);
+    const int plane = k >> 3, c = k & 7;
+    unsigned char* base = img + (((int64_t)part * samples + b) * heads + h) * (int64_t)npad * QKV3_ROWB + plane * 128;
+    const u32x4 v = *reinterpret_cast<const u32x4*>(base + (int64_t)cl.p0 * QKV3_ROWB + ((c ^ qkv3_swizzle(part, cl.p0)) << 4));
+    *reinterpret_cast<u32x4*>(base + (int64_t)(cl.p0 + r) * QKV3_ROWB + ((c ^ qkv3_swizzle(part, cl.p0 + r)) << 4)) = v;
+}
+
 int gemm_bf16x3_qkv3(const void* A3, const void* W3, const float* bias, void* img, int64_t M, int tokens, int heads, int K, float qscale,
-                     int terms, hipStream_t st, float ab_scale, float c_scale, const float* ss_in, float eps) {
+                     int terms, hipStream_t st, float ab_scale, float c_scale, const float* ss_in, float eps, RowCollapse cl, int samples,
+                     bool share) {
     AVD_REQUIRE(!ss_in || K % 64 == 0, AVD_EUNSUPPORTED, "gemm_bf16x3_qkv3: a folded norm needs K %% 64 == 0");
+    if (cl.on()) {
+        AVD_REQUIRE(samples > cl.b0 && cl.b0 > 0 && cl.p0 >= 0 && cl.p0 + cl.np <= tokens && (!share || samples == 2 * cl.b0) &&
+                        M == (int64_t)cl.b0 * tokens + (int64_t)(samples - cl.b0) * (share ? 1 : tokens - cl.np + 1),
+                    AVD_EINVAL, "gemm_bf16x3_qkv3: collapsed rows %lld do not match %d samples (%d full) of %d tokens, span %d + %d", (long long)M,
+                    samples, cl.b0, tokens, cl.p0, cl.np);
+    }
     AVD_REQUIRE(A3 && W3 && bias && img, AVD_EINVAL, "gemm_bf16x3_qkv3: null pointer");
     AVD_REQUIRE(ab_scale > 0.f && ab_scale < __builtin_inff() && c_scale > 0.f && c_scale < __builtin_inff(), AVD_EINVAL,
                 "gemm_bf16x3_qkv3: image scales must be positive and finite");
     const int N = 3 * heads * 64;
-    AVD_REQUIRE(tokens > 0 && heads > 0 && M > 0 && M % tokens == 0, AVD_EINVAL, "gemm_bf16x3_qkv3: rows %lld not a multiple of tokens %d",
+    AVD_REQUIRE(tokens > 0 && heads > 0 && M > 0 && (cl.on() || M % tokens == 0), AVD_EINVAL, "gemm_bf16x3_qkv3: rows %lld not a multiple of tokens %d",
                 (long long)M, tokens);
     AVD_REQUIRE(M < (1ll << 31) - 256, AVD_EUNSUPPORTED, "gemm_bf16x3_qkv3: more than 2^31 rows");
     AVD_REQUIRE(gemm_bf16x3_supported(M, N, K), AVD_EUNSUPPORTED, "gemm_bf16x3_qkv3: need 3*heads*64 %% 256 == 0 and K %% 16 == 0");
@@ -1625,7 +1667,18 @@
     S3Args a{static_cast<const unsigned char*>(A3), static_cast<const unsigned char*>(W3), bias, nullptr, nullptr,
              static_cast<unsigned char*>(img), M, N, K, 0, 0, 0, tokens, qkv3_npad(tokens), heads, qscale, 0, 0, terms, 1.0f / ab_scale, c_scale,
              ss_in, nullptr, (float)sqrt((double)K), eps, nullptr, 0, 0};
-    return launch_s3<S3_EPI_QKV3>(a, st);
+    if (!cl.on()) return launch_s3<S3_EPI_QKV3>(a, st);
+    a.q_samples = samples;
+    a.q_share = share ? 1 : 0;
+    a.cl = cl;
+    if (int rc = launch_s3<S3_EPI_QKV3>(a, st)) return rc;
+    const int64_t chunks = (int64_t)2 * (samples - cl.b0) * heads * (cl.np - 1) * (QKV3_ROWB / 16);
+    static const int tag = prof_tag_id("qkv3_span_fill_kernel");
+    ProfScope prof(tag, 2.0 * 16 * chunks, st);
+    hipLaunchKernelGGL(qkv3_span_fill_kernel, dim3((unsigned)((chunks + 255) / 256)), dim3(256), 0, st, static_cast<unsigned char*>(img), samples,
+                       heads, qkv3_npad(tokens), cl, chunks);
+    AVD_CHECK_LAUNCH("qkv3_span_fill");
+    return AVD_OK;
 }
 
 }
diff --git a/multimodal_diffusion_amd/csrc/s3_common.h b/multimodal_diffusion_amd/csrc/s3_common.h
--- a/multimodal_diffusion_amd/csrc/s3_common.h
+++ b/multimodal_diffusion_amd/csrc/s3_common.h
@@ -29,6 +29,9 @@
     float ss_sqrt_d, ss_eps;
     const float* gamma;
     int r_seg, r_stride;
+    int r_split = 0, r_stride2 = 0, r_skip2 = 0;
+    int q_samples = 0, q_share = 0;
+    RowCollapse cl;
 #ifdef AVD_S3_STAMPS
     unsigned long long* dbg;
 #endif
@@ -43,6 +46,29 @@
 #define S3_RT() 0ull
 #define S3_DBG(i, v) do { } while (0)
 #endif
+
+__device__ __forceinline__ void qkv3_row_of(const S3Args& g, int64_t m, unsigned& b, unsigned& tok) {
+    const unsigned full = g.cl.on() ? (unsigned)g.cl.b0 * (unsigned)g.tokN : 0xffffffffu;
+    if ((unsigned)m < full) {
+        b = (unsigned)m / (unsigned)g.tokN;
+        tok = (unsigned)m - b * (unsigned)g.tokN;
+        return;
+    }
+    const unsigned nb = (unsigned)(g.q_samples - g.cl.b0), j = (unsigned)m - full;
+    if (j < nb) {
+        b = (unsigned)g.cl.b0 + j;
+        tok = (unsigned)g.cl.p0;
+        return;
+    }
+    const unsigned nr = (unsigned)(g.tokN - g.cl.np), bj = (j - nb) / nr, c = (j - nb) - bj * nr;
+    b = (unsigned)g.cl.b0 + bj;
+    tok = c < (unsigned)g.cl.p0 ? c : c + (unsigned)g.cl.np;
+}
+__device__ __forceinline__ int64_t qkv3_share_off(const S3Args& g, unsigned b, unsigned tok) {
+    if (!g.q_share || b >= (unsigned)g.cl.b0 || (tok >= (unsigned)g.cl.p0 && tok < (unsigned)(g.cl.p0 + g.cl.np))) return -1;
+    return (int64_t)g.cl.b0 * g.heads * g.tokNpad * QKV3_ROWB;
+}
+__device__ __forceinline__ int64_t qkv3_samples(const S3Args& g) { return g.q_samples > 0 ? g.q_samples : g.M / g.tokN; }
 
 __device__ __forceinline__ void s3_block_of(const S3Args& g, int nbm, int& bm, int& bn) {
     const int b = blockIdx.x, nwg = gridDim.x, q = nwg >> 3, r = nwg & 7, x = b & 7;
@@ -107,7 +133,7 @@
         const int dmodel = g.heads * 64;
         const int part = nbase / dmodel, head = (nbase % dmodel) >> 6;
         mul = part == 0 ? g.qscale : 1.0f;
-        qbase = (((int64_t)part * (g.M / g.tokN)) * g.heads + head) * (int64_t)g.tokNpad * QKV3_ROWB;
+        qbase = (((int64_t)part * qkv3_samples(g)) * g.heads + head) * (int64_t)g.tokNpad * QKV3_ROWB;
     }
 #pragma unroll
     for (int ip = 0; ip < 4; ++ip) {
@@ -129,8 +155,11 @@
         }
         [[maybe_unused]] unsigned char* qrow = nullptr;
         [[maybe_unused]] int qsw = 0;
+        [[maybe_unused]] int64_t qdup = -1;
         if constexpr (EPI == S3_EPI_QKV3) {
-            const unsigned b = (unsigned)m / (unsigned)g.tokN, tok = (unsigned)m - b * (unsigned)g.tokN;
+            unsigned b, tok;
+            qkv3_row_of(g, m, b, tok);
+            qdup = qkv3_share_off(g, b, tok);
             qrow = g.C3 + qbase + ((int64_t)b * g.heads * g.tokNpad + tok) * QKV3_ROWB;
             qsw = qkv3_swizzle(nbase / (g.heads * 64), (int)tok);
         }
@@ -138,8 +167,10 @@
         [[maybe_unused]] int64_t rrow = m;
         if constexpr (EPI == S3_EPI_RES_IMG) {
             if (g.r_seg > 0 && m < g.M) {
-                const unsigned sgi = (unsigned)m / (unsigned)g.r_seg;
-                rrow = (int64_t)sgi * g.r_stride + ((unsigned)m - sgi * (unsigned)g.r_seg);
+                const unsigned sgi = (unsigned)m / (unsigned)g.r_seg, rem = (unsigned)m - sgi * (unsigned)g.r_seg;
+                rrow = g.r_split > 0 && sgi >= (unsigned)g.r_split
+                     ? (int64_t)g.r_split * g.r_stride + g.r_skip2 + (int64_t)(sgi - (unsigned)g.r_split) * g.r_stride2 + rem
+                     : (int64_t)sgi * g.r_stride + rem;
             }
         }
 #pragma unroll
@@ -164,6 +195,11 @@
                     *reinterpret_cast<u32x4*>(dst) = Hh;
                     *reinterpret_cast<u32x4*>(dst + 128) = Mi;
                     *reinterpret_cast<u32x4*>(dst + 256) = Lo;
+                    if (qdup >= 0) {
+                        *reinterpret_cast<u32x4*>(dst + qdup) = Hh;
+                        *reinterpret_cast<u32x4*>(dst + qdup + 128) = Mi;
+                        *reinterpret_cast<u32x4*>(dst + qdup + 256) = Lo;
+                    }
                 }
             } else if constexpr (EPI == S3_EPI_BIAS_REG) {
                 if (S3_ROW_OK(m)) {
diff --git a/multimodal_diffusion_amd/csrc/tokens.hip b/multimodal_diffusion_amd/csrc/tokens.hip
--- a/multimodal_diffusion_amd/csrc/tokens.hip
+++ b/multimodal_diffusion_amd/csrc/tokens.hip
@@ -414,14 +414,27 @@
 __global__ __launch_bounds__(256) void assemble_rows_kernel(float* __restrict__ X2, const int64_t* __restrict__ t_now,
                                                             const float* __restrict__ freqs, const float* __restrict__ Xp,
                                                             float* __restrict__ ss, int B, int N, int d, int tdim, int Nt, int Np,
-                                                            int target_first, float neg_log_mp) {
+                                                            int target_first, float neg_log_mp, int collapse) {
     const int lane = threadIdx.x & 63;
     const int64_t row = (int64_t)blockIdx.x * 4 + (threadIdx.x >> 6);
-    if (row >= (int64_t)2 * B * N) return;
-    const int n = (int)(row % N);
-    const int bb = (int)(row / N);
-    const int half = bb >= B, b = half ? bb - B : bb;
+    const int Nn = collapse ? N - Np + 1 : N;
+    if (row >= (int64_t)B * (N + Nn)) return;
+    const int half = row >= (int64_t)B * N;
+    const int64_t r = half ? row - (int64_t)B * N : row;
     const int t0 = target_first ? 0 : Np;
+    const int p0 = target_first ? Nt : 0;
+    int b, n;
+    if (!half || !collapse) {
+        b = (int)(r / N);
+        n = (int)(r % N);
+    } else if (r < B) {
+        b = (int)r;
+        n = p0;
+    } else {
+        b = (int)((r - B) / (N - Np));
+        const int c = (int)((r - B) % (N - Np));
+        n = c < p0 ? c : c + Np;
+    }
     const bool is_t = n >= t0 && n < t0 + Nt;
     const int da = d - tdim, th = tdim >> 1;
     const float tf = is_t ? (float)t_now[b] : 0.f;
@@ -459,12 +472,13 @@
 }
 
 int assemble_rows_f32(float* X2, const int64_t* t_now, const float* freqs, const float* Xp, float* ss, int B, int N, int d, int tdim,
-                      int Nt, int Np, int target_first, float max_period, hipStream_t st) {
-    const int64_t rows = (int64_t)2 * B * N;
+                      int Nt, int Np, int target_first, float max_period, hipStream_t st, int collapse) {
+    AVD_REQUIRE(!collapse || Np > 1, AVD_EINVAL, "assemble_rows: a collapsed null half needs at least two prompt rows");
+    const int64_t rows = (int64_t)B * N + (int64_t)B * (collapse ? N - Np + 1 : N);
     static const int tag = prof_tag_id("assemble_rows_kernel");
-    ProfScope prof(tag, 4.0 * (2.0 * B * N * d + (double)B * Nt * (d - tdim) + (double)B * Np * d), st);
+    ProfScope prof(tag, 4.0 * ((double)rows * d + (double)B * Nt * (d - tdim) + (double)B * Np * d), st);
     hipLaunchKernelGGL(assemble_rows_kernel, dim3((unsigned)((rows + 3) / 4)), dim3(256), 0, st, X2, t_now, freqs, Xp, ss, B, N, d, tdim,
-                       Nt, Np, target_first, -(float)log((double)max_period));
+                       Nt, Np, target_first, -(float)log((double)max_period), collapse);
     AVD_CHECK_LAUNCH("assemble_rows");
     return AVD_OK;
 }
```

After: 120.1 steps/s (median of 6 runs). +2.1%, better.
